# FedericoV/SysBio_Modeling

Hardware: AMD Instinct MI355X
Metric: ensemble ODE-steps/sec (20-state model + fwd sens) (higher is better)
Workload: dtype f64; 1 GPU; configs[2]: cascade20 (20 states, 40 params) + full forward sensitivities = 820 ODEs, 4096 vectors/GPU, DOPRI45, 16 output times; gather + integrate + residual/Jacobian assembly; vectors_per_gpu=4096, n_equations=820, integrator=dopri45, failed_vectors=0

## Files before the change

sysbio_modeling_amd/csrc/models/cascade20.hpp:

```cpp
#pragma once

__constant__ short SBM_RL_CLASS[20] = {0, 1, 1, 1, 1, 1, 1, 1, 1, 1, 1, 1, 1, 1, 1, 1, 1, 1, 1, 1};
__constant__ short SBM_RL_YS[40] = {19, 1, 2, 3, 4, 5, 6, 7, 8, 9, 10, 11, 12, 13, 14, 15, 16, 17, 18, 19, 0, 0, 1, 2, 3, 4, 5, 6, 7, 8, 9, 10, 11, 12, 13, 14, 15, 16, 17, 18};
__constant__ short SBM_RL_PS[40] = {0, 21, 22, 23, 24, 25, 26, 27, 28, 29, 30, 31, 32, 33, 34, 35, 36, 37, 38, 39, 20, 1, 2, 3, 4, 5, 6, 7, 8, 9, 10, 11, 12, 13, 14, 15, 16, 17, 18, 19};
__constant__ short SBM_RL_JYOUT[40] = {0, 2, 4, 6, 8, 10, 12, 14, 16, 18, 20, 22, 24, 26, 28, 30, 32, 34, 36, 38, 1, 3, 5, 7, 9, 11, 13, 15, 17, 19, 21, 23, 25, 27, 29, 31, 33, 35, 37, 39};
__constant__ short SBM_RL_APOS[40] = {0, 65, 130, 195, 260, 325, 390, 455, 520, 585, 650, 715, 780, 845, 910, 975, 1040, 1105, 1170, 1235, 20, 85, 150, 215, 280, 345, 410, 475, 540, 605, 670, 735, 800, 865, 930, 995, 1060, 1125, 1190, 1255};
__constant__ short SBM_RL_JPCOL[40] = {0, 1, 2, 3, 4, 5, 6, 7, 8, 9, 10, 11, 12, 13, 14, 15, 16, 17, 18, 19, 20, 21, 22, 23, 24, 25, 26, 27, 28, 29, 30, 31, 32, 33, 34, 35, 36, 37, 38, 39};
__constant__ short SBM_RL_JYCOL[40] = {0, 0, 1, 2, 3, 4, 5, 6, 7, 8, 9, 10, 11, 12, 13, 14, 15, 16, 17, 18, 19, 1, 2, 3, 4, 5, 6, 7, 8, 9, 10, 11, 12, 13, 14, 15, 16, 17, 18, 19};

__constant__ short SBM_RG0_JYPOS[40] = {0, 3, 5, 7, 9, 11, 13, 15, 17, 19, 21, 23, 25, 27, 29, 31, 33, 35, 37, 39, 1, 2, 4, 6, 8, 10, 12, 14, 16, 18, 20, 22, 24, 26, 28, 30, 32, 34, 36, 38};
__constant__ short SBM_RG0_HSRC[3] = {19, 6, 13};

__constant__ short SBM_RG1_JYPOS[40] = {0, 3, 5, 7, 9, 11, 13, 15, 17, 19, 21, 23, 25, 27, 29, 31, 33, 35, 37, 39, 1, 2, 4, 6, 8, 10, 12, 14, 16, 18, 20, 22, 24, 26, 28, 30, 32, 34, 36, 38};
__constant__ short SBM_RG1_HSRC[7] = {19, 2, 5, 8, 11, 14, 17};

__constant__ short SBM_RG2_JYPOS[40] = {0, 3, 5, 7, 9, 11, 13, 15, 17, 19, 21, 23, 25, 27, 29, 31, 33, 35, 37, 39, 1, 2, 4, 6, 8, 10, 12, 14, 16, 18, 20, 22, 24, 26, 28, 30, 32, 34, 36, 38};
__constant__ short SBM_RG2_HSRC[3] = {19, 6, 13};

__constant__ short SBM_IM_RSTART[1] = {0};
__constant__ short SBM_IM_DIAGSLOT[1] = {-1};
__constant__ short SBM_IM_MFPOS[1] = {0};
__constant__ short SBM_IM_R0[1] = {0};
__constant__ short SBM_IM_JPQ[1] = {0};

struct SbmModel {
  static constexpr int NV = 20;
  static constexpr int NP = 40;
  static constexpr int NK = 40;
  static constexpr int NNZ_JY = 40;
  static constexpr int NNZ_JP = 40;
  static constexpr int NJY = 40;
  static constexpr int NJP = 40;
  static constexpr const char* NAME = "cascade20";

  template <class PA>
  __device__ __forceinline__ static void eval_f(double t, const double (&y)[NV], const PA& p,
                                                double (&f)[NV]) {
    (void)t;
    f[0] = -p[20]*y[0] + p[0]*SBM_RCP(y[19] + 1.0);
    f[1] = -p[21]*y[1] + p[1]*y[0]*SBM_RCP(y[0] + 1.0);
    f[2] = -p[22]*y[2] + p[2]*y[1]*SBM_RCP(y[1] + 1.0);
    f[3] = -p[23]*y[3] + p[3]*y[2]*SBM_RCP(y[2] + 1.0);
    f[4] = -p[24]*y[4] + p[4]*y[3]*SBM_RCP(y[3] + 1.0);
    f[5] = -p[25]*y[5] + p[5]*y[4]*SBM_RCP(y[4] + 1.0);
    f[6] = -p[26]*y[6] + p[6]*y[5]*SBM_RCP(y[5] + 1.0);
    f[7] = -p[27]*y[7] + p[7]*y[6]*SBM_RCP(y[6] + 1.0);
    f[8] = -p[28]*y[8] + p[8]*y[7]*SBM_RCP(y[7] + 1.0);
    f[9] = -p[29]*y[9] + p[9]*y[8]*SBM_RCP(y[8] + 1.0);
    f[10] = -p[30]*y[10] + p[10]*y[9]*SBM_RCP(y[9] + 1.0);
    f[11] = -p[31]*y[11] + p[11]*y[10]*SBM_RCP(y[10] + 1.0);
    f[12] = -p[32]*y[12] + p[12]*y[11]*SBM_RCP(y[11] + 1.0);
    f[13] = -p[33]*y[13] + p[13]*y[12]*SBM_RCP(y[12] + 1.0);
    f[14] = -p[34]*y[14] + p[14]*y[13]*SBM_RCP(y[13] + 1.0);
    f[15] = -p[35]*y[15] + p[15]*y[14]*SBM_RCP(y[14] + 1.0);
    f[16] = -p[36]*y[16] + p[16]*y[15]*SBM_RCP(y[15] + 1.0);
    f[17] = -p[37]*y[17] + p[17]*y[16]*SBM_RCP(y[16] + 1.0);
    f[18] = -p[38]*y[18] + p[18]*y[17]*SBM_RCP(y[17] + 1.0);
    f[19] = -p[39]*y[19] + p[19]*y[18]*SBM_RCP(y[18] + 1.0);
  }

  template <class PA>
  __device__ __forceinline__ static void eval_jac(double t, const double (&y)[NV], const PA& p,
                                                  double (&f)[NV], double (&jy)[NJY], double (&jp)[NJP]) {
    (void)t;
    const double x_0 = SBM_RCP(y[19] + 1.0);
    const double x_1 = SBM_RCP(y[0] + 1.0);
    const double x_2 = SBM_RCP(y[1] + 1.0);
    const double x_3 = SBM_RCP(y[2] + 1.0);
    const double x_4 = SBM_RCP(y[3] + 1.0);
    const double x_5 = SBM_RCP(y[4] + 1.0);
    const double x_6 = SBM_RCP(y[5] + 1.0);
    const double x_7 = SBM_RCP(y[6] + 1.0);
    const double x_8 = SBM_RCP(y[7] + 1.0);
    const double x_9 = SBM_RCP(y[8] + 1.0);
    const double x_10 = SBM_RCP(y[9] + 1.0);
    const double x_11 = SBM_RCP(y[10] + 1.0);
    const double x_12 = SBM_RCP(y[11] + 1.0);
    const double x_13 = SBM_RCP(y[12] + 1.0);
    const double x_14 = SBM_RCP(y[13] + 1.0);
    const double x_15 = SBM_RCP(y[14] + 1.0);
    const double x_16 = SBM_RCP(y[15] + 1.0);
    const double x_17 = SBM_RCP(y[16] + 1.0);
    const double x_18 = SBM_RCP(y[17] + 1.0);
    const double x_19 = SBM_RCP(y[18] + 1.0);
    f[0] = -p[20]*y[0] + p[0]*x_0;
    f[1] = -p[21]*y[1] + p[1]*y[0]*x_1;
    f[2] = -p[22]*y[2] + p[2]*y[1]*x_2;
    f[3] = -p[23]*y[3] + p[3]*y[2]*x_3;
    f[4] = -p[24]*y[4] + p[4]*y[3]*x_4;
    f[5] = -p[25]*y[5] + p[5]*y[4]*x_5;
    f[6] = -p[26]*y[6] + p[6]*y[5]*x_6;
    f[7] = -p[27]*y[7] + p[7]*y[6]*x_7;
    f[8] = -p[28]*y[8] + p[8]*y[7]*x_8;
    f[9] = -p[29]*y[9] + p[9]*y[8]*x_9;
    f[10] = -p[30]*y[10] + p[10]*y[9]*x_10;
    f[11] = -p[31]*y[11] + p[11]*y[10]*x_11;
    f[12] = -p[32]*y[12] + p[12]*y[11]*x_12;
    f[13] = -p[33]*y[13] + p[13]*y[12]*x_13;
    f[14] = -p[34]*y[14] + p[14]*y[13]*x_14;
    f[15] = -p[35]*y[15] + p[15]*y[14]*x_15;
    f[16] = -p[36]*y[16] + p[16]*y[15]*x_16;
    f[17] = -p[37]*y[17] + p[17]*y[16]*x_17;
    f[18] = -p[38]*y[18] + p[18]*y[17]*x_18;
    f[19] = -p[39]*y[19] + p[19]*y[18]*x_19;
    jy[0] = -p[20];
    jy[1] = -p[0]*(x_0*x_0);
    jy[2] = p[1]*(x_1*x_1);
    jy[3] = -p[21];
    jy[4] = p[2]*(x_2*x_2);
    jy[5] = -p[22];
    jy[6] = p[3]*(x_3*x_3);
    jy[7] = -p[23];
    jy[8] = p[4]*(x_4*x_4);
    jy[9] = -p[24];
    jy[10] = p[5]*(x_5*x_5);
    jy[11] = -p[25];
    jy[12] = p[6]*(x_6*x_6);
    jy[13] = -p[26];
    jy[14] = p[7]*(x_7*x_7);
    jy[15] = -p[27];
    jy[16] = p[8]*(x_8*x_8);
    jy[17] = -p[28];
    jy[18] = p[9]*(x_9*x_9);
    jy[19] = -p[29];
    jy[20] = p[10]*(x_10*x_10);
    jy[21] = -p[30];
    jy[22] = p[11]*(x_11*x_11);
    jy[23] = -p[31];
    jy[24] = p[12]*(x_12*x_12);
    jy[25] = -p[32];
    jy[26] = p[13]*(x_13*x_13);
    jy[27] = -p[33];
    jy[28] = p[14]*(x_14*x_14);
    jy[29] = -p[34];
    jy[30] = p[15]*(x_15*x_15);
    jy[31] = -p[35];
    jy[32] = p[16]*(x_16*x_16);
    jy[33] = -p[36];
    jy[34] = p[17]*(x_17*x_17);
    jy[35] = -p[37];
    jy[36] = p[18]*(x_18*x_18);
    jy[37] = -p[38];
    jy[38] = p[19]*(x_19*x_19);
    jy[39] = -p[39];
    jp[0] = x_0;
    jp[1] = -y[0];
    jp[2] = y[0]*x_1;
    jp[3] = -y[1];
    jp[4] = y[1]*x_2;
    jp[5] = -y[2];
    jp[6] = y[2]*x_3;
    jp[7] = -y[3];
    jp[8] = y[3]*x_4;
    jp[9] = -y[4];
    jp[10] = y[4]*x_5;
    jp[11] = -y[5];
    jp[12] = y[5]*x_6;
    jp[13] = -y[6];
    jp[14] = y[6]*x_7;
    jp[15] = -y[7];
    jp[16] = y[7]*x_8;
    jp[17] = -y[8];
    jp[18] = y[8]*x_9;
    jp[19] = -y[9];
    jp[20] = y[9]*x_10;
    jp[21] = -y[10];
    jp[22] = y[10]*x_11;
    jp[23] = -y[11];
    jp[24] = y[11]*x_12;
    jp[25] = -y[12];
    jp[26] = y[12]*x_13;
    jp[27] = -y[13];
    jp[28] = y[13]*x_14;
    jp[29] = -y[14];
    jp[30] = y[14]*x_15;
    jp[31] = -y[15];
    jp[32] = y[15]*x_16;
    jp[33] = -y[16];
    jp[34] = y[16]*x_17;
    jp[35] = -y[17];
    jp[36] = y[17]*x_18;
    jp[37] = -y[18];
    jp[38] = y[18]*x_19;
    jp[39] = -y[19];
  }

  __device__ __forceinline__ static void apply_col(const double (&jy)[NJY], const double (&jp)[NJP],
                                                   int scol, const double (&z)[NV], double (&dz)[NV]) {
    dz[0] = fma(jy[1], z[19], fma(jy[0], z[0], SBM_PICK(scol, 0, jp[0], SBM_PICK(scol, 20, jp[1], 0.0))));
    dz[1] = fma(jy[3], z[1], fma(jy[2], z[0], SBM_PICK(scol, 1, jp[2], SBM_PICK(scol, 21, jp[3], 0.0))));
    dz[2] = fma(jy[5], z[2], fma(jy[4], z[1], SBM_PICK(scol, 2, jp[4], SBM_PICK(scol, 22, jp[5], 0.0))));
    dz[3] = fma(jy[7], z[3], fma(jy[6], z[2], SBM_PICK(scol, 3, jp[6], SBM_PICK(scol, 23, jp[7], 0.0))));
    dz[4] = fma(jy[9], z[4], fma(jy[8], z[3], SBM_PICK(scol, 4, jp[8], SBM_PICK(scol, 24, jp[9], 0.0))));
    dz[5] = fma(jy[11], z[5], fma(jy[10], z[4], SBM_PICK(scol, 5, jp[10], SBM_PICK(scol, 25, jp[11], 0.0))));
    dz[6] = fma(jy[13], z[6], fma(jy[12], z[5], SBM_PICK(scol, 6, jp[12], SBM_PICK(scol, 26, jp[13], 0.0))));
    dz[7] = fma(jy[15], z[7], fma(jy[14], z[6], SBM_PICK(scol, 7, jp[14], SBM_PICK(scol, 27, jp[15], 0.0))));
    dz[8] = fma(jy[17], z[8], fma(jy[16], z[7], SBM_PICK(scol, 8, jp[16], SBM_PICK(scol, 28, jp[17], 0.0))));
    dz[9] = fma(jy[19], z[9], fma(jy[18], z[8], SBM_PICK(scol, 9, jp[18], SBM_PICK(scol, 29, jp[19], 0.0))));
    dz[10] = fma(jy[21], z[10], fma(jy[20], z[9], SBM_PICK(scol, 10, jp[20], SBM_PICK(scol, 30, jp[21], 0.0))));
    dz[11] = fma(jy[23], z[11], fma(jy[22], z[10], SBM_PICK(scol, 11, jp[22], SBM_PICK(scol, 31, jp[23], 0.0))));
    dz[12] = fma(jy[25], z[12], fma(jy[24], z[11], SBM_PICK(scol, 12, jp[24], SBM_PICK(scol, 32, jp[25], 0.0))));
    dz[13] = fma(jy[27], z[13], fma(jy[26], z[12], SBM_PICK(scol, 13, jp[26], SBM_PICK(scol, 33, jp[27], 0.0))));
    dz[14] = fma(jy[29], z[14], fma(jy[28], z[13], SBM_PICK(scol, 14, jp[28], SBM_PICK(scol, 34, jp[29], 0.0))));
    dz[15] = fma(jy[31], z[15], fma(jy[30], z[14], SBM_PICK(scol, 15, jp[30], SBM_PICK(scol, 35, jp[31], 0.0))));
    dz[16] = fma(jy[33], z[16], fma(jy[32], z[15], SBM_PICK(scol, 16, jp[32], SBM_PICK(scol, 36, jp[33], 0.0))));
    dz[17] = fma(jy[35], z[17], fma(jy[34], z[16], SBM_PICK(scol, 17, jp[34], SBM_PICK(scol, 37, jp[35], 0.0))));
    dz[18] = fma(jy[37], z[18], fma(jy[36], z[17], SBM_PICK(scol, 18, jp[36], SBM_PICK(scol, 38, jp[37], 0.0))));
    dz[19] = fma(jy[39], z[19], fma(jy[38], z[18], SBM_PICK(scol, 19, jp[38], SBM_PICK(scol, 39, jp[39], 0.0))));
  }

  template <class PA>
  __device__ __forceinline__ static void eval_col(double t, const double (&y)[NV], const PA& p, int scol,
                                                  const double (&z)[NV], double (&dz)[NV]) {
    (void)t;
    const bool state_lane = scol < 0;
    const double x_0 = SBM_RCP(y[19] + 1.0);
    dz[0] = SBM_SEL(state_lane, -p[20]*y[0] + p[0]*x_0, fma(-p[0]*(x_0*x_0), z[19], fma(-p[20], z[0], SBM_PICK(scol, 0, x_0, SBM_PICK(scol, 20, -y[0], 0.0)))));
    const double x_1 = SBM_RCP(y[0] + 1.0);
    dz[1] = SBM_SEL(state_lane, -p[21]*y[1] + p[1]*y[0]*x_1, fma(-p[21], z[1], fma(p[1]*(x_1*x_1), z[0], SBM_PICK(scol, 1, y[0]*x_1, SBM_PICK(scol, 21, -y[1], 0.0)))));
    const double x_2 = SBM_RCP(y[1] + 1.0);
    dz[2] = SBM_SEL(state_lane, -p[22]*y[2] + p[2]*y[1]*x_2, fma(-p[22], z[2], fma(p[2]*(x_2*x_2), z[1], SBM_PICK(scol, 2, y[1]*x_2, SBM_PICK(scol, 22, -y[2], 0.0)))));
    const double x_3 = SBM_RCP(y[2] + 1.0);
    dz[3] = SBM_SEL(state_lane, -p[23]*y[3] + p[3]*y[2]*x_3, fma(-p[23], z[3], fma(p[3]*(x_3*x_3), z[2], SBM_PICK(scol, 3, y[2]*x_3, SBM_PICK(scol, 23, -y[3], 0.0)))));
    const double x_4 = SBM_RCP(y[3] + 1.0);
    dz[4] = SBM_SEL(state_lane, -p[24]*y[4] + p[4]*y[3]*x_4, fma(-p[24], z[4], fma(p[4]*(x_4*x_4), z[3], SBM_PICK(scol, 4, y[3]*x_4, SBM_PICK(scol, 24, -y[4], 0.0)))));
    const double x_5 = SBM_RCP(y[4] + 1.0);
    dz[5] = SBM_SEL(state_lane, -p[25]*y[5] + p[5]*y[4]*x_5, fma(-p[25], z[5], fma(p[5]*(x_5*x_5), z[4], SBM_PICK(scol, 5, y[4]*x_5, SBM_PICK(scol, 25, -y[5], 0.0)))));
    const double x_6 = SBM_RCP(y[5] + 1.0);
    dz[6] = SBM_SEL(state_lane, -p[26]*y[6] + p[6]*y[5]*x_6, fma(-p[26], z[6], fma(p[6]*(x_6*x_6), z[5], SBM_PICK(scol, 6, y[5]*x_6, SBM_PICK(scol, 26, -y[6], 0.0)))));
    const double x_7 = SBM_RCP(y[6] + 1.0);
    dz[7] = SBM_SEL(state_lane, -p[27]*y[7] + p[7]*y[6]*x_7, fma(-p[27], z[7], fma(p[7]*(x_7*x_7), z[6], SBM_PICK(scol, 7, y[6]*x_7, SBM_PICK(scol, 27, -y[7], 0.0)))));
    const double x_8 = SBM_RCP(y[7] + 1.0);
    dz[8] = SBM_SEL(state_lane, -p[28]*y[8] + p[8]*y[7]*x_8, fma(-p[28], z[8], fma(p[8]*(x_8*x_8), z[7], SBM_PICK(scol, 8, y[7]*x_8, SBM_PICK(scol, 28, -y[8], 0.0)))));
    const double x_9 = SBM_RCP(y[8] + 1.0);
    dz[9] = SBM_SEL(state_lane, -p[29]*y[9] + p[9]*y[8]*x_9, fma(-p[29], z[9], fma(p[9]*(x_9*x_9), z[8], SBM_PICK(scol, 9, y[8]*x_9, SBM_PICK(scol, 29, -y[9], 0.0)))));
    const double x_10 = SBM_RCP(y[9] + 1.0);
    dz[10] = SBM_SEL(state_lane, -p[30]*y[10] + p[10]*y[9]*x_10, fma(-p[30], z[10], fma(p[10]*(x_10*x_10), z[9], SBM_PICK(scol, 10, y[9]*x_10, SBM_PICK(scol, 30, -y[10], 0.0)))));
    const double x_11 = SBM_RCP(y[10] + 1.0);
    dz[11] = SBM_SEL(state_lane, -p[31]*y[11] + p[11]*y[10]*x_11, fma(-p[31], z[11], fma(p[11]*(x_11*x_11), z[10], SBM_PICK(scol, 11, y[10]*x_11, SBM_PICK(scol, 31, -y[11], 0.0)))));
    const double x_12 = SBM_RCP(y[11] + 1.0);
    dz[12] = SBM_SEL(state_lane, -p[32]*y[12] + p[12]*y[11]*x_12, fma(-p[32], z[12], fma(p[12]*(x_12*x_12), z[11], SBM_PICK(scol, 12, y[11]*x_12, SBM_PICK(scol, 32, -y[12], 0.0)))));
    const double x_13 = SBM_RCP(y[12] + 1.0);
    dz[13] = SBM_SEL(state_lane, -p[33]*y[13] + p[13]*y[12]*x_13, fma(-p[33], z[13], fma(p[13]*(x_13*x_13), z[12], SBM_PICK(scol, 13, y[12]*x_13, SBM_PICK(scol, 33, -y[13], 0.0)))));
    const double x_14 = SBM_RCP(y[13] + 1.0);
    dz[14] = SBM_SEL(state_lane, -p[34]*y[14] + p[14]*y[13]*x_14, fma(-p[34], z[14], fma(p[14]*(x_14*x_14), z[13], SBM_PICK(scol, 14, y[13]*x_14, SBM_PICK(scol, 34, -y[14], 0.0)))));
    const double x_15 = SBM_RCP(y[14] + 1.0);
    dz[15] = SBM_SEL(state_lane, -p[35]*y[15] + p[15]*y[14]*x_15, fma(-p[35], z[15], fma(p[15]*(x_15*x_15), z[14], SBM_PICK(scol, 15, y[14]*x_15, SBM_PICK(scol, 35, -y[15], 0.0)))));
    const double x_16 = SBM_RCP(y[15] + 1.0);
    dz[16] = SBM_SEL(state_lane, -p[36]*y[16] + p[16]*y[15]*x_16, fma(-p[36], z[16], fma(p[16]*(x_16*x_16), z[15], SBM_PICK(scol, 16, y[15]*x_16, SBM_PICK(scol, 36, -y[16], 0.0)))));
    const double x_17 = SBM_RCP(y[16] + 1.0);
    dz[17] = SBM_SEL(state_lane, -p[37]*y[17] + p[17]*y[16]*x_17, fma(-p[37], z[17], fma(p[17]*(x_17*x_17), z[16], SBM_PICK(scol, 17, y[16]*x_17, SBM_PICK(scol, 37, -y[17], 0.0)))));
    const double x_18 = SBM_RCP(y[17] + 1.0);
    dz[18] = SBM_SEL(state_lane, -p[38]*y[18] + p[18]*y[17]*x_18, fma(-p[38], z[18], fma(p[18]*(x_18*x_18), z[17], SBM_PICK(scol, 18, y[17]*x_18, SBM_PICK(scol, 38, -y[18], 0.0)))));
    const double x_19 = SBM_RCP(y[18] + 1.0);
    dz[19] = SBM_SEL(state_lane, -p[39]*y[19] + p[19]*y[18]*x_19, fma(-p[39], z[19], fma(p[19]*(x_19*x_19), z[18], SBM_PICK(scol, 19, y[18]*x_19, SBM_PICK(scol, 39, -y[19], 0.0)))));
  }

  static constexpr int RL_NCLASS = 2;
  static constexpr int RL_MAXYS = 2, RL_MAXPS = 2, RL_MAXJY = 2, RL_MAXJP = 2;
  static constexpr int RL_LARGEST_CLASS = 19;
  __device__ __forceinline__ static int rl_class(int row) { return SBM_RL_CLASS[row]; }
  __device__ __forceinline__ static int rl_ys(int slot, int row) { return SBM_RL_YS[slot * NV + row]; }
  __device__ __forceinline__ static int rl_ps(int slot, int row) { return SBM_RL_PS[slot * NV + row]; }
  __device__ __forceinline__ static int rl_jyout(int slot, int row) { return SBM_RL_JYOUT[slot * NV + row]; }
  __device__ __forceinline__ static int rl_apos(int slot, int row) { return SBM_RL_APOS[slot * NV + row]; }
  __device__ __forceinline__ static int rl_jpcol(int slot, int row) { return SBM_RL_JPCOL[slot * NV + row]; }
  __device__ __forceinline__ static int rl_jycol(int slot, int row) { return SBM_RL_JYCOL[slot * NV + row]; }
  __device__ __forceinline__ static void class_dispatch(int cls, double t, const double (&ys)[RL_MAXYS],
                                                        const double (&ps)[RL_MAXPS], double& f,
                                                        double (&jy)[RL_MAXJY], double (&jp)[RL_MAXJP]) {
    (void)t; (void)ys; (void)ps;
    const bool is0 = (cls == 0);
    const double h0 = SBM_RCP(SBM_SEL(is0, ys[0], ys[1]) + 1.0);
    const double c0_x0 = h0;
    const double c1_x0 = h0;
    f = SBM_SEL(is0, ps[0]*c0_x0 - ps[1]*ys[1], -ps[0]*ys[0] + ps[1]*ys[1]*c1_x0);
    jy[0] = SBM_SEL(is0, -ps[1], ps[1]*(c1_x0*c1_x0));
    jy[1] = SBM_SEL(is0, -ps[0]*(c0_x0*c0_x0), -ps[0]);
    jp[0] = SBM_SEL(is0, c0_x0, ys[1]*c1_x0);
    jp[1] = SBM_SEL(is0, -ys[1], -ys[0]);
  }

  static constexpr int RL_NSTATIC = 20;
  __device__ __forceinline__ static void rl_static(const double (&jy)[RL_MAXJY], double (&sj)[20]) {
    (void)jy;
    sj[0] = SBM_LANE_BCAST(jy[0], 0);
    sj[1] = SBM_LANE_BCAST(jy[1], 1);
    sj[2] = SBM_LANE_BCAST(jy[1], 2);
    sj[3] = SBM_LANE_BCAST(jy[1], 3);
    sj[4] = SBM_LANE_BCAST(jy[1], 4);
    sj[5] = SBM_LANE_BCAST(jy[1], 5);
    sj[6] = SBM_LANE_BCAST(jy[1], 6);
    sj[7] = SBM_LANE_BCAST(jy[1], 7);
    sj[8] = SBM_LANE_BCAST(jy[1], 8);
    sj[9] = SBM_LANE_BCAST(jy[1], 9);
    sj[10] = SBM_LANE_BCAST(jy[1], 10);
    sj[11] = SBM_LANE_BCAST(jy[1], 11);
    sj[12] = SBM_LANE_BCAST(jy[1], 12);
    sj[13] = SBM_LANE_BCAST(jy[1], 13);
    sj[14] = SBM_LANE_BCAST(jy[1], 14);
    sj[15] = SBM_LANE_BCAST(jy[1], 15);
    sj[16] = SBM_LANE_BCAST(jy[1], 16);
    sj[17] = SBM_LANE_BCAST(jy[1], 17);
    sj[18] = SBM_LANE_BCAST(jy[1], 18);
    sj[19] = SBM_LANE_BCAST(jy[1], 19);
  }

  template <int NZ>
  __device__ __forceinline__ static void apply_rowlane(const double (&jy)[RL_MAXJY], const double (&sj)[20],
                                                       const double (&acol)[NV], const double (&z)[NZ],
                                                       double (&dz)[NZ]) {
    (void)jy; (void)sj;
    dz[0] = fma(SBM_LANE_BCAST(jy[1], 0), z[19], fma(sj[0], z[0], acol[0]));
    dz[1] = fma(sj[1], z[1], fma(SBM_LANE_BCAST(jy[0], 1), z[0], acol[1]));
    dz[2] = fma(sj[2], z[2], fma(SBM_LANE_BCAST(jy[0], 2), z[1], acol[2]));
    dz[3] = fma(sj[3], z[3], fma(SBM_LANE_BCAST(jy[0], 3), z[2], acol[3]));
    dz[4] = fma(sj[4], z[4], fma(SBM_LANE_BCAST(jy[0], 4), z[3], acol[4]));
    dz[5] = fma(sj[5], z[5], fma(SBM_LANE_BCAST(jy[0], 5), z[4], acol[5]));
    dz[6] = fma(sj[6], z[6], fma(SBM_LANE_BCAST(jy[0], 6), z[5], acol[6]));
    dz[7] = fma(sj[7], z[7], fma(SBM_LANE_BCAST(jy[0], 7), z[6], acol[7]));
    dz[8] = fma(sj[8], z[8], fma(SBM_LANE_BCAST(jy[0], 8), z[7], acol[8]));
    dz[9] = fma(sj[9], z[9], fma(SBM_LANE_BCAST(jy[0], 9), z[8], acol[9]));
    dz[10] = fma(sj[10], z[10], fma(SBM_LANE_BCAST(jy[0], 10), z[9], acol[10]));
    dz[11] = fma(sj[11], z[11], fma(SBM_LANE_BCAST(jy[0], 11), z[10], acol[11]));
    dz[12] = fma(sj[12], z[12], fma(SBM_LANE_BCAST(jy[0], 12), z[11], acol[12]));
    dz[13] = fma(sj[13], z[13], fma(SBM_LANE_BCAST(jy[0], 13), z[12], acol[13]));
    dz[14] = fma(sj[14], z[14], fma(SBM_LANE_BCAST(jy[0], 14), z[13], acol[14]));
    dz[15] = fma(sj[15], z[15], fma(SBM_LANE_BCAST(jy[0], 15), z[14], acol[15]));
    dz[16] = fma(sj[16], z[16], fma(SBM_LANE_BCAST(jy[0], 16), z[15], acol[16]));
    dz[17] = fma(sj[17], z[17], fma(SBM_LANE_BCAST(jy[0], 17), z[16], acol[17]));
    dz[18] = fma(sj[18], z[18], fma(SBM_LANE_BCAST(jy[0], 18), z[17], acol[18]));
    dz[19] = fma(sj[19], z[19], fma(SBM_LANE_BCAST(jy[0], 19), z[18], acol[19]));
  }

  template <int NZ>
  __device__ __forceinline__ static void apply_lds(const double* jyl, const double (&acol)[NV],
                                                   const double (&z)[NZ], double (&dz)[NZ]) {
    (void)jyl;
    dz[0] = fma(jyl[1], z[19], fma(jyl[0], z[0], acol[0]));
    dz[1] = fma(jyl[3], z[1], fma(jyl[2], z[0], acol[1]));
    dz[2] = fma(jyl[5], z[2], fma(jyl[4], z[1], acol[2]));
    dz[3] = fma(jyl[7], z[3], fma(jyl[6], z[2], acol[3]));
    dz[4] = fma(jyl[9], z[4], fma(jyl[8], z[3], acol[4]));
    dz[5] = fma(jyl[11], z[5], fma(jyl[10], z[4], acol[5]));
    dz[6] = fma(jyl[13], z[6], fma(jyl[12], z[5], acol[6]));
    dz[7] = fma(jyl[15], z[7], fma(jyl[14], z[6], acol[7]));
    dz[8] = fma(jyl[17], z[8], fma(jyl[16], z[7], acol[8]));
    dz[9] = fma(jyl[19], z[9], fma(jyl[18], z[8], acol[9]));
    dz[10] = fma(jyl[21], z[10], fma(jyl[20], z[9], acol[10]));
    dz[11] = fma(jyl[23], z[11], fma(jyl[22], z[10], acol[11]));
    dz[12] = fma(jyl[25], z[12], fma(jyl[24], z[11], acol[12]));
    dz[13] = fma(jyl[27], z[13], fma(jyl[26], z[12], acol[13]));
    dz[14] = fma(jyl[29], z[14], fma(jyl[28], z[13], acol[14]));
    dz[15] = fma(jyl[31], z[15], fma(jyl[30], z[14], acol[15]));
    dz[16] = fma(jyl[33], z[16], fma(jyl[32], z[15], acol[16]));
    dz[17] = fma(jyl[35], z[17], fma(jyl[34], z[16], acol[17]));
    dz[18] = fma(jyl[37], z[18], fma(jyl[36], z[17], acol[18]));
    dz[19] = fma(jyl[39], z[19], fma(jyl[38], z[18], acol[19]));
  }

  struct RG0 {
  static constexpr bool RG_OK = true;
  static constexpr int RG_G = 3, RG_C = 20, RG_CPL = 2, RG_RPG = 7, RG_JYS = 2, RG_NHALO = 1;
  static constexpr int RG_NCH = 1;
  static constexpr int RG_LS = 128;
  __device__ __forceinline__ static int rg_pos(int row, int col) {
    return (row % RG_RPG) * RG_LS + RG_CPL * ((row / RG_RPG) * RG_C + col % RG_C) + col / RG_C;
  }
  __device__ __forceinline__ static int rg_jypos(int slot, int row) { return SBM_RG0_JYPOS[slot * NV + row]; }
  __device__ __forceinline__ static int rg_hsrc(int term, int group) { return SBM_RG0_HSRC[term * RG_G + group]; }
  template <int NZ>
  __device__ __forceinline__ static void publish_rowgroup(double* h_lane, const double (&z)[NZ]) {
    (void)h_lane; (void)z;
    h_lane[640] = z[5];
    h_lane[641] = z[12];
    h_lane[768] = z[6];
    h_lane[769] = z[13];
  }
  __device__ __forceinline__ static void load_rowgroup(const double* a_lane, const double* jy_lane,
                                                       double (&acol)[14], double (&coef)[14]) {
    coef[0] = jy_lane[0];
    coef[1] = jy_lane[1];
    coef[2] = jy_lane[2];
    coef[3] = jy_lane[3];
    coef[4] = jy_lane[4];
    coef[5] = jy_lane[5];
    coef[6] = jy_lane[6];
    coef[7] = jy_lane[7];
    coef[8] = jy_lane[8];
    coef[9] = jy_lane[9];
    coef[10] = jy_lane[10];
    coef[11] = jy_lane[11];
    coef[12] = jy_lane[12];
    coef[13] = jy_lane[13];
    acol[0] = a_lane[0];
    acol[7] = a_lane[1];
    acol[1] = a_lane[128];
    acol[8] = a_lane[129];
    acol[2] = a_lane[256];
    acol[9] = a_lane[257];
    acol[3] = a_lane[384];
    acol[10] = a_lane[385];
    acol[4] = a_lane[512];
    acol[11] = a_lane[513];
    acol[5] = a_lane[640];
    acol[12] = a_lane[641];
    acol[6] = a_lane[768];
    acol[13] = a_lane[769];
  }
  template <int NZ>
  __device__ __forceinline__ static void apply_rowgroup(const double (&acol)[14], const double (&coef)[14],
                                                        const double* h_all, const int (&hoff)[1],
                                                        const double (&z)[NZ], double (&dz)[NZ]) {
    (void)h_all; (void)hoff;
    const double h0_1_0 = h_all[hoff[0] + 0];
    const double h0_1_1 = h_all[hoff[0] + 1];
    dz[1] = fma(coef[3], z[0], fma(coef[2], z[1], acol[1]));
    dz[2] = fma(coef[5], z[1], fma(coef[4], z[2], acol[2]));
    dz[3] = fma(coef[7], z[2], fma(coef[6], z[3], acol[3]));
    dz[4] = fma(coef[9], z[3], fma(coef[8], z[4], acol[4]));
    dz[5] = fma(coef[11], z[4], fma(coef[10], z[5], acol[5]));
    dz[6] = fma(coef[13], z[5], fma(coef[12], z[6], acol[6]));
    dz[0] = fma(coef[1], h0_1_0, fma(coef[0], z[0], acol[0]));
    dz[8] = fma(coef[3], z[7], fma(coef[2], z[8], acol[8]));
    dz[9] = fma(coef[5], z[8], fma(coef[4], z[9], acol[9]));
    dz[10] = fma(coef[7], z[9], fma(coef[6], z[10], acol[10]));
    dz[11] = fma(coef[9], z[10], fma(coef[8], z[11], acol[11]));
    dz[12] = fma(coef[11], z[11], fma(coef[10], z[12], acol[12]));
    dz[13] = fma(coef[13], z[12], fma(coef[12], z[13], acol[13]));
    dz[7] = fma(coef[1], h0_1_1, fma(coef[0], z[7], acol[7]));
  }
  };
  struct RG1 {
  static constexpr bool RG_OK = true;
  static constexpr int RG_G = 7, RG_C = 8, RG_CPL = 1, RG_RPG = 3, RG_JYS = 2, RG_NHALO = 1;
  static constexpr int RG_NCH = 5;
  static constexpr int RG_LS = 64;
  __device__ __forceinline__ static int rg_pos(int row, int col) {
    return (row % RG_RPG) * RG_LS + RG_CPL * ((row / RG_RPG) * RG_C + col % RG_C) + col / RG_C;
  }
  __device__ __forceinline__ static int rg_jypos(int slot, int row) { return SBM_RG1_JYPOS[slot * NV + row]; }
  __device__ __forceinline__ static int rg_hsrc(int term, int group) { return SBM_RG1_HSRC[term * RG_G + group]; }
  template <int NZ>
  __device__ __forceinline__ static void publish_rowgroup(double* h_lane, const double (&z)[NZ]) {
    (void)h_lane; (void)z;
    h_lane[64] = z[1];
    h_lane[128] = z[2];
  }
  __device__ __forceinline__ static void load_rowgroup(const double* a_lane, const double* jy_lane,
                                                       double (&acol)[3], double (&coef)[6]) {
    coef[0] = jy_lane[0];
    coef[1] = jy_lane[1];
    coef[2] = jy_lane[2];
    coef[3] = jy_lane[3];
    coef[4] = jy_lane[4];
    coef[5] = jy_lane[5];
    acol[0] = a_lane[0];
    acol[1] = a_lane[64];
    acol[2] = a_lane[128];
  }
  template <int NZ>
  __device__ __forceinline__ static void apply_rowgroup(const double (&acol)[3], const double (&coef)[6],
                                                        const double* h_all, const int (&hoff)[1],
                                                        const double (&z)[NZ], double (&dz)[NZ]) {
    (void)h_all; (void)hoff;
    const double h0_1_0 = h_all[hoff[0] + 0];
    dz[1] = fma(coef[3], z[0], fma(coef[2], z[1], acol[1]));
    dz[2] = fma(coef[5], z[1], fma(coef[4], z[2], acol[2]));
    dz[0] = fma(coef[1], h0_1_0, fma(coef[0], z[0], acol[0]));
  }
  };
  struct RG2 {
  static constexpr bool RG_OK = true;
  static constexpr int RG_G = 3, RG_C = 20, RG_CPL = 1, RG_RPG = 7, RG_JYS = 2, RG_NHALO = 1;
  static constexpr int RG_NCH = 2;
  static constexpr int RG_LS = 64;
  __device__ __forceinline__ static int rg_pos(int row, int col) {
    return (row % RG_RPG) * RG_LS + RG_CPL * ((row / RG_RPG) * RG_C + col % RG_C) + col / RG_C;
  }
  __device__ __forceinline__ static int rg_jypos(int slot, int row) { return SBM_RG2_JYPOS[slot * NV + row]; }
  __device__ __forceinline__ static int rg_hsrc(int term, int group) { return SBM_RG2_HSRC[term * RG_G + group]; }
  template <int NZ>
  __device__ __forceinline__ static void publish_rowgroup(double* h_lane, const double (&z)[NZ]) {
    (void)h_lane; (void)z;
    h_lane[320] = z[5];
    h_lane[384] = z[6];
  }
  __device__ __forceinline__ static void load_rowgroup(const double* a_lane, const double* jy_lane,
                                                       double (&acol)[7], double (&coef)[14]) {
    coef[0] = jy_lane[0];
    coef[1] = jy_lane[1];
    coef[2] = jy_lane[2];
    coef[3] = jy_lane[3];
    coef[4] = jy_lane[4];
    coef[5] = jy_lane[5];
    coef[6] = jy_lane[6];
    coef[7] = jy_lane[7];
    coef[8] = jy_lane[8];
    coef[9] = jy_lane[9];
    coef[10] = jy_lane[10];
    coef[11] = jy_lane[11];
    coef[12] = jy_lane[12];
    coef[13] = jy_lane[13];
    acol[0] = a_lane[0];
    acol[1] = a_lane[64];
    acol[2] = a_lane[128];
    acol[3] = a_lane[192];
    acol[4] = a_lane[256];
    acol[5] = a_lane[320];
    acol[6] = a_lane[384];
  }
// ... 218 lines not shown
```

sysbio_modeling_amd/csrc/models/michaelis_menten.hpp:

```cpp
#pragma once

__constant__ short SBM_RL_CLASS[2] = {0, 1};
__constant__ short SBM_RL_YS[4] = {0, 1, 0, 0};
__constant__ short SBM_RL_PS[8] = {2, 4, 3, 0, 0, 1, 1, 0};
__constant__ short SBM_RL_JYOUT[4] = {0, 1, 3, 2};
__constant__ short SBM_RL_APOS[8] = {0, 64, 1, 65, 2, 68, 3, 128};
__constant__ short SBM_RL_JPCOL[8] = {0, 0, 1, 1, 2, 4, 3, -1};
__constant__ short SBM_RL_JYCOL[4] = {0, 0, -1, 1};

__constant__ short SBM_RG0_JYPOS[4] = {0, 3, 4, 2};
__constant__ short SBM_RG0_HSRC[2] = {2, 0};

__constant__ short SBM_IM_RSTART[2] = {0, 2};
__constant__ short SBM_IM_DIAGSLOT[2] = {0, 1};
__constant__ short SBM_IM_MFPOS[4] = {4, 3, 4, 4};
__constant__ short SBM_IM_R0[1] = {0};
__constant__ short SBM_IM_JPQ[1] = {0};

struct SbmModel {
  static constexpr int NV = 2;
  static constexpr int NP = 5;
  static constexpr int NK = 5;
  static constexpr int NNZ_JY = 3;
  static constexpr int NNZ_JP = 7;
  static constexpr int NJY = 3;
  static constexpr int NJP = 7;
  static constexpr const char* NAME = "michaelis_menten";

  template <class PA>
  __device__ __forceinline__ static void eval_f(double t, const double (&y)[NV], const PA& p,
                                                double (&f)[NV]) {
    (void)t;
    const double x_0 = y[0]*p[0]*SBM_RCP(y[0] + p[1]);
    f[0] = -y[0]*p[3] + p[2] - x_0;
    f[1] = -y[1]*p[4] + x_0;
  }

  template <class PA>
  __device__ __forceinline__ static void eval_jac(double t, const double (&y)[NV], const PA& p,
                                                  double (&f)[NV], double (&jy)[NJY], double (&jp)[NJP]) {
    (void)t;
    const double x_0 = SBM_RCP(y[0] + p[1]);
    const double x_1 = y[0]*x_0;
    const double x_2 = p[0]*x_1;
    const double x_3 = p[0]*(x_0*x_0);
    const double x_4 = p[1]*x_3;
    const double x_5 = y[0]*x_3;
    f[0] = -y[0]*p[3] + p[2] - x_2;
    f[1] = -y[1]*p[4] + x_2;
    jy[0] = -p[3] - x_4;
    jy[1] = x_4;
    jy[2] = -p[4];
    jp[0] = -x_1;
    jp[1] = x_5;
    jp[2] = 1.0;
    jp[3] = -y[0];
    jp[4] = x_1;
    jp[5] = -x_5;
    jp[6] = -y[1];
  }

  __device__ __forceinline__ static void apply_col(const double (&jy)[NJY], const double (&jp)[NJP],
                                                   int scol, const double (&z)[NV], double (&dz)[NV]) {
    dz[0] = fma(jy[0], z[0], SBM_PICK(scol, 0, jp[0], SBM_PICK(scol, 1, jp[1], SBM_PICK(scol, 2, jp[2], SBM_PICK(scol, 3, jp[3], 0.0)))));
    dz[1] = fma(jy[2], z[1], fma(jy[1], z[0], SBM_PICK(scol, 0, jp[4], SBM_PICK(scol, 1, jp[5], SBM_PICK(scol, 4, jp[6], 0.0)))));
  }

  template <class PA>
  __device__ __forceinline__ static void eval_col(double t, const double (&y)[NV], const PA& p, int scol,
                                                  const double (&z)[NV], double (&dz)[NV]) {
    (void)t;
    const bool state_lane = scol < 0;
    const double x_0 = SBM_RCP(y[0] + p[1]);
    const double x_1 = y[0]*x_0;
    const double x_2 = p[0]*x_1;
    const double x_3 = p[0]*(x_0*x_0);
    const double x_4 = p[1]*x_3;
    const double x_5 = y[0]*x_3;
    dz[0] = SBM_SEL(state_lane, -y[0]*p[3] + p[2] - x_2, fma(-p[3] - x_4, z[0], SBM_PICK(scol, 0, -x_1, SBM_PICK(scol, 1, x_5, SBM_PICK(scol, 2, 1.0, SBM_PICK(scol, 3, -y[0], 0.0))))));
    dz[1] = SBM_SEL(state_lane, -y[1]*p[4] + x_2, fma(-p[4], z[1], fma(x_4, z[0], SBM_PICK(scol, 0, x_1, SBM_PICK(scol, 1, -x_5, SBM_PICK(scol, 4, -y[1], 0.0))))));
  }

  static constexpr int RL_NCLASS = 2;
  static constexpr int RL_MAXYS = 2, RL_MAXPS = 4, RL_MAXJY = 2, RL_MAXJP = 4;
  static constexpr int RL_LARGEST_CLASS = 1;
  __device__ __forceinline__ static int rl_class(int row) { return SBM_RL_CLASS[row]; }
  __device__ __forceinline__ static int rl_ys(int slot, int row) { return SBM_RL_YS[slot * NV + row]; }
  __device__ __forceinline__ static int rl_ps(int slot, int row) { return SBM_RL_PS[slot * NV + row]; }
  __device__ __forceinline__ static int rl_jyout(int slot, int row) { return SBM_RL_JYOUT[slot * NV + row]; }
  __device__ __forceinline__ static int rl_apos(int slot, int row) { return SBM_RL_APOS[slot * NV + row]; }
  __device__ __forceinline__ static int rl_jpcol(int slot, int row) { return SBM_RL_JPCOL[slot * NV + row]; }
  __device__ __forceinline__ static int rl_jycol(int slot, int row) { return SBM_RL_JYCOL[slot * NV + row]; }
  __device__ __forceinline__ static void class_dispatch(int cls, double t, const double (&ys)[RL_MAXYS],
                                                        const double (&ps)[RL_MAXPS], double& f,
                                                        double (&jy)[RL_MAXJY], double (&jp)[RL_MAXJP]) {
    (void)t; (void)ys; (void)ps;
    const bool is0 = (cls == 0);
    const double h0 = SBM_RCP(SBM_SEL(is0, ps[3], ps[2]) + SBM_SEL(is0, ys[0], ys[1]));
    const double c0_x0 = h0;
    const double c0_x1 = ys[0]*c0_x0;
    const double c0_x2 = ps[2]*(c0_x0*c0_x0);
    const double c1_x0 = h0;
    const double c1_x1 = ps[1]*(c1_x0*c1_x0);
    f = SBM_SEL(is0, ps[0] - ps[1]*ys[0] - ps[2]*c0_x1, -ps[0]*ys[0] + ps[1]*ys[1]*c1_x0);
    jy[0] = SBM_SEL(is0, -ps[1] - ps[3]*c0_x2, ps[2]*c1_x1);
    jy[1] = SBM_SEL(is0, 0.0, -ps[0]);
    jp[0] = SBM_SEL(is0, -c0_x1, ys[1]*c1_x0);
    jp[1] = SBM_SEL(is0, ys[0]*c0_x2, -ys[1]*c1_x1);
    jp[2] = SBM_SEL(is0, 1.0, -ys[0]);
    jp[3] = SBM_SEL(is0, -ys[0], 0.0);
  }

  static constexpr int RL_NSTATIC = 1;
  __device__ __forceinline__ static void rl_static(const double (&jy)[RL_MAXJY], double (&sj)[1]) {
    (void)jy;
    sj[0] = SBM_LANE_BCAST(jy[1], 1);
  }

  template <int NZ>
  __device__ __forceinline__ static void apply_rowlane(const double (&jy)[RL_MAXJY], const double (&sj)[1],
                                                       const double (&acol)[NV], const double (&z)[NZ],
                                                       double (&dz)[NZ]) {
    (void)jy; (void)sj;
    dz[0] = fma(SBM_LANE_BCAST(jy[0], 0), z[0], acol[0]);
    dz[1] = fma(sj[0], z[1], fma(SBM_LANE_BCAST(jy[0], 1), z[0], acol[1]));
  }

  template <int NZ>
  __device__ __forceinline__ static void apply_lds(const double* jyl, const double (&acol)[NV],
                                                   const double (&z)[NZ], double (&dz)[NZ]) {
    (void)jyl;
    dz[0] = fma(jyl[0], z[0], acol[0]);
    dz[1] = fma(jyl[3], z[1], fma(jyl[2], z[0], acol[1]));
  }

  struct RG0 {
  static constexpr bool RG_OK = true;
  static constexpr int RG_G = 2, RG_C = 5, RG_CPL = 1, RG_RPG = 1, RG_JYS = 2, RG_NHALO = 1;
  static constexpr int RG_NCH = 1;
  static constexpr int RG_LS = 64;
  __device__ __forceinline__ static int rg_pos(int row, int col) {
    return (row % RG_RPG) * RG_LS + RG_CPL * ((row / RG_RPG) * RG_C + col % RG_C) + col / RG_C;
  }
  __device__ __forceinline__ static int rg_jypos(int slot, int row) { return SBM_RG0_JYPOS[slot * NV + row]; }
  __device__ __forceinline__ static int rg_hsrc(int term, int group) { return SBM_RG0_HSRC[term * RG_G + group]; }
  template <int NZ>
  __device__ __forceinline__ static void publish_rowgroup(double* h_lane, const double (&z)[NZ]) {
    (void)h_lane; (void)z;
    h_lane[0] = z[0];
  }
  __device__ __forceinline__ static void load_rowgroup(const double* a_lane, const double* jy_lane,
                                                       double (&acol)[1], double (&coef)[2]) {
    coef[0] = jy_lane[0];
    coef[1] = jy_lane[1];
    acol[0] = a_lane[0];
  }
  template <int NZ>
  __device__ __forceinline__ static void apply_rowgroup(const double (&acol)[1], const double (&coef)[2],
                                                        const double* h_all, const int (&hoff)[1],
                                                        const double (&z)[NZ], double (&dz)[NZ]) {
    (void)h_all; (void)hoff;
    const double h0_1_0 = h_all[hoff[0] + 0];
    dz[0] = fma(coef[1], h0_1_0, fma(coef[0], z[0], acol[0]));
  }
  };
  using RG1 = RG0;
  using RG2 = RG0;

  static constexpr int IM_NM = 3;
  __device__ __forceinline__ static void im_build(double gamma, const double* jy, double (&m)[IM_NM]) {
    (void)gamma; (void)jy;
    m[0] = fma(-gamma, jy[0], 1.0);
    m[1] = -gamma * jy[1];
    m[2] = fma(-gamma, jy[2], 1.0);
  }
  __device__ __forceinline__ static void im_factor(double (&m)[IM_NM]) {
    m[0] = SBM_RCP(m[0]);
    m[1] *= m[0];
    m[2] = SBM_RCP(m[2]);
  }
  __device__ __forceinline__ static void im_solve(const double (&m)[IM_NM], double (&b)[NV]) {
    b[1] = fma(-m[1], b[0], b[1]);
    b[1] *= m[2];
    b[0] *= m[0];
  }
  static constexpr bool IM_TRI = true;
  __device__ __forceinline__ static void im_solve_tri(const double* mf, double (&b)[NV]) {
    b[0] = mf[0] * b[0];
    b[1] = fma(mf[3], b[0], mf[2] * b[1]);
  }
  template <int RPL>
  __device__ __forceinline__ static void im_solve_tri_pick(const double* mf, const double* g, int lane, double (&d)[RPL]) {
    const double x_0 = mf[0] * g[0];
    d[0] = SBM_SEL(lane == 0, x_0, d[0]);
    const double x_1 = fma(mf[3], x_0, mf[2] * g[1]);
    d[0] = SBM_SEL(lane == 1, x_1, d[0]);
  }
  static constexpr bool IM_SENS_TRI = true;
  static constexpr int IM_JP = RL_MAXJP > 0 ? RL_MAXJP : 1;
  __device__ __forceinline__ static void im_sens_tri(const double* mf, const double* ja, double hh, int col, double (&z)[NV]) {
    (void)col;
    double t0[4], a0[2 * IM_JP];
    _Pragma("unroll") for (int e = 0; e < 4; ++e) t0[e] = mf[0 + e];
    _Pragma("unroll") for (int e = 0; e < 2 * RL_MAXJP; ++e) a0[e] = ja[0 * RL_MAXJP + e];
    SBM_LDS_FENCE();
    z[0] = fma(hh, SBM_PICK_COL(col, 0, a0[0 * RL_MAXJP + 0], SBM_PICK_COL(col, 1, a0[0 * RL_MAXJP + 1], SBM_PICK_COL(col, 2, a0[0 * RL_MAXJP + 2], SBM_PICK_COL(col, 3, a0[0 * RL_MAXJP + 3], 0.0)))), z[0]);
    z[0] = t0[0] * z[0];
    z[1] = fma(hh, SBM_PICK_COL(col, 0, a0[1 * RL_MAXJP + 0], SBM_PICK_COL(col, 1, a0[1 * RL_MAXJP + 1], SBM_PICK_COL(col, 4, a0[1 * RL_MAXJP + 2], 0.0))), z[1]);
    z[1] = fma(t0[3], z[0], t0[2] * z[1]);
  }
  static constexpr int IM_MF = 4;
  static constexpr bool IM_CHAIN = true;
  static constexpr bool IM_ROT = false;
  static_assert(!IM_ROT || sizeof(SBM_IM_R0) / sizeof(short) >= NK, "one rotated-column entry per column");
  static_assert(!IM_ROT || sizeof(SBM_IM_JPQ) / sizeof(short) >= NK, "one rotated-column entry per column");
  __device__ __forceinline__ static int im_r0(int col) { return SBM_IM_R0[IM_ROT ? col : 0]; }
  __device__ __forceinline__ static int im_jpq(int col) { return SBM_IM_JPQ[IM_ROT ? col : 0]; }
  static constexpr bool IM_DIST = false;
  static constexpr int IM_LD = 2;
  __device__ __forceinline__ static void im_factor_rows(double (&)[NV], int, double*) {}
  __device__ __forceinline__ static void im_solve_lds(const double*, const double*, double (&)[NV]) {}
  __device__ __forceinline__ static int im_rstart(int row) { return SBM_IM_RSTART[IM_TRI ? row : 0]; }
  __device__ __forceinline__ static int im_diagslot(int row) { return SBM_IM_DIAGSLOT[IM_TRI ? row : 0]; }
  __device__ __forceinline__ static int im_mfpos(int slot, int row) { return SBM_IM_MFPOS[IM_TRI ? slot * NV + row : 0]; }
};
```

sysbio_modeling_amd/csrc/models/stiff50.hpp:

```cpp
#pragma once

__constant__ short SBM_RL_CLASS[50] = {0, 1, 1, 1, 1, 1, 1, 1, 1, 1, 1, 1, 1, 1, 1, 1, 1, 1, 1, 1, 1, 1, 1, 1, 1, 1, 1, 1, 1, 1, 1, 1, 1, 1, 1, 1, 1, 1, 1, 1, 1, 1, 1, 1, 1, 1, 1, 1, 1, 1};
__constant__ short SBM_RL_YS[100] = {0, 0, 1, 2, 3, 4, 5, 6, 7, 8, 9, 10, 11, 12, 13, 14, 15, 16, 17, 18, 19, 20, 21, 22, 23, 24, 25, 26, 27, 28, 29, 30, 31, 32, 33, 34, 35, 36, 37, 38, 39, 40, 41, 42, 43, 44, 45, 46, 47, 48, 0, 1, 2, 3, 4, 5, 6, 7, 8, 9, 10, 11, 12, 13, 14, 15, 16, 17, 18, 19, 20, 21, 22, 23, 24, 25, 26, 27, 28, 29, 30, 31, 32, 33, 34, 35, 36, 37, 38, 39, 40, 41, 42, 43, 44, 45, 46, 47, 48, 49};
__constant__ short SBM_RL_PS[100] = {0, 1, 2, 3, 4, 5, 6, 7, 8, 9, 10, 11, 12, 13, 14, 15, 16, 17, 18, 19, 20, 21, 22, 23, 24, 25, 26, 27, 28, 29, 30, 31, 32, 33, 34, 35, 36, 37, 38, 39, 40, 41, 42, 43, 44, 45, 46, 47, 48, 49, 50, 51, 52, 53, 54, 55, 56, 57, 58, 59, 60, 61, 62, 63, 64, 65, 66, 67, 68, 69, 70, 71, 72, 73, 74, 75, 76, 77, 78, 79, 80, 81, 82, 83, 84, 85, 86, 87, 88, 89, 90, 91, 92, 93, 94, 95, 96, 97, 98, 99};
__constant__ short SBM_RL_JYOUT[100] = {0, 1, 3, 5, 7, 9, 11, 13, 15, 17, 19, 21, 23, 25, 27, 29, 31, 33, 35, 37, 39, 41, 43, 45, 47, 49, 51, 53, 55, 57, 59, 61, 63, 65, 67, 69, 71, 73, 75, 77, 79, 81, 83, 85, 87, 89, 91, 93, 95, 97, 99, 2, 4, 6, 8, 10, 12, 14, 16, 18, 20, 22, 24, 26, 28, 30, 32, 34, 36, 38, 40, 42, 44, 46, 48, 50, 52, 54, 56, 58, 60, 62, 64, 66, 68, 70, 72, 74, 76, 78, 80, 82, 84, 86, 88, 90, 92, 94, 96, 98};
__constant__ short SBM_RL_APOS[50] = {0, 65, 130, 195, 260, 325, 390, 455, 520, 585, 650, 715, 780, 845, 910, 975, 1040, 1105, 1170, 1235, 1300, 1365, 1430, 1495, 1560, 1625, 1690, 1755, 1820, 1885, 1950, 2015, 2080, 2145, 2210, 2275, 2340, 2405, 2470, 2535, 2600, 2665, 2730, 2795, 2860, 2925, 2990, 3055, 3120, 3185};
__constant__ short SBM_RL_JPCOL[50] = {0, 1, 2, 3, 4, 5, 6, 7, 8, 9, 10, 11, 12, 13, 14, 15, 16, 17, 18, 19, 20, 21, 22, 23, 24, 25, 26, 27, 28, 29, 30, 31, 32, 33, 34, 35, 36, 37, 38, 39, 40, 41, 42, 43, 44, 45, 46, 47, 48, 49};
__constant__ short SBM_RL_JYCOL[100] = {0, 0, 1, 2, 3, 4, 5, 6, 7, 8, 9, 10, 11, 12, 13, 14, 15, 16, 17, 18, 19, 20, 21, 22, 23, 24, 25, 26, 27, 28, 29, 30, 31, 32, 33, 34, 35, 36, 37, 38, 39, 40, 41, 42, 43, 44, 45, 46, 47, 48, -1, 1, 2, 3, 4, 5, 6, 7, 8, 9, 10, 11, 12, 13, 14, 15, 16, 17, 18, 19, 20, 21, 22, 23, 24, 25, 26, 27, 28, 29, 30, 31, 32, 33, 34, 35, 36, 37, 38, 39, 40, 41, 42, 43, 44, 45, 46, 47, 48, 49};

__constant__ short SBM_RG0_JYPOS[100] = {0, 3, 5, 7, 9, 11, 13, 15, 17, 19, 21, 23, 25, 27, 29, 31, 33, 35, 37, 39, 41, 43, 45, 47, 49, 51, 53, 55, 57, 59, 61, 63, 65, 67, 69, 71, 73, 75, 77, 79, 81, 83, 85, 87, 89, 91, 93, 95, 97, 99, 108, 2, 4, 6, 8, 10, 12, 14, 16, 18, 20, 22, 24, 26, 28, 30, 32, 34, 36, 38, 40, 42, 44, 46, 48, 50, 52, 54, 56, 58, 60, 62, 64, 66, 68, 70, 72, 74, 76, 78, 80, 82, 84, 86, 88, 90, 92, 94, 96, 98};
__constant__ short SBM_RG0_HSRC[6] = {54, 8, 17, 26, 35, 44};

__constant__ short SBM_RG1_JYPOS[100] = {0, 3, 5, 7, 9, 11, 13, 15, 17, 19, 21, 23, 25, 27, 29, 31, 33, 35, 37, 39, 41, 43, 45, 47, 49, 51, 53, 55, 57, 59, 61, 63, 65, 67, 69, 71, 73, 75, 77, 79, 81, 83, 85, 87, 89, 91, 93, 95, 97, 99, 112, 2, 4, 6, 8, 10, 12, 14, 16, 18, 20, 22, 24, 26, 28, 30, 32, 34, 36, 38, 40, 42, 44, 46, 48, 50, 52, 54, 56, 58, 60, 62, 64, 66, 68, 70, 72, 74, 76, 78, 80, 82, 84, 86, 88, 90, 92, 94, 96, 98};
__constant__ short SBM_RG1_HSRC[8] = {56, 6, 13, 20, 27, 34, 41, 48};

__constant__ short SBM_RG2_JYPOS[100] = {0, 3, 5, 7, 9, 11, 13, 15, 17, 19, 21, 23, 25, 27, 29, 31, 33, 35, 37, 39, 41, 43, 45, 47, 49, 51, 53, 55, 57, 59, 61, 63, 65, 67, 69, 71, 73, 75, 77, 79, 81, 83, 85, 87, 89, 91, 93, 95, 97, 99, 112, 2, 4, 6, 8, 10, 12, 14, 16, 18, 20, 22, 24, 26, 28, 30, 32, 34, 36, 38, 40, 42, 44, 46, 48, 50, 52, 54, 56, 58, 60, 62, 64, 66, 68, 70, 72, 74, 76, 78, 80, 82, 84, 86, 88, 90, 92, 94, 96, 98};
__constant__ short SBM_RG2_HSRC[8] = {56, 6, 13, 20, 27, 34, 41, 48};

__constant__ short SBM_IM_RSTART[50] = {0, 2, 4, 6, 8, 10, 12, 14, 16, 18, 20, 22, 24, 26, 28, 30, 32, 34, 36, 38, 40, 42, 44, 46, 48, 50, 52, 54, 56, 58, 60, 62, 64, 66, 68, 70, 72, 74, 76, 78, 80, 82, 84, 86, 88, 90, 92, 94, 96, 98};
__constant__ short SBM_IM_DIAGSLOT[50] = {0, 1, 1, 1, 1, 1, 1, 1, 1, 1, 1, 1, 1, 1, 1, 1, 1, 1, 1, 1, 1, 1, 1, 1, 1, 1, 1, 1, 1, 1, 1, 1, 1, 1, 1, 1, 1, 1, 1, 1, 1, 1, 1, 1, 1, 1, 1, 1, 1, 1};
__constant__ short SBM_IM_MFPOS[100] = {100, 3, 5, 7, 9, 11, 13, 15, 17, 19, 21, 23, 25, 27, 29, 31, 33, 35, 37, 39, 41, 43, 45, 47, 49, 51, 53, 55, 57, 59, 61, 63, 65, 67, 69, 71, 73, 75, 77, 79, 81, 83, 85, 87, 89, 91, 93, 95, 97, 99, 100, 100, 100, 100, 100, 100, 100, 100, 100, 100, 100, 100, 100, 100, 100, 100, 100, 100, 100, 100, 100, 100, 100, 100, 100, 100, 100, 100, 100, 100, 100, 100, 100, 100, 100, 100, 100, 100, 100, 100, 100, 100, 100, 100, 100, 100, 100, 100, 100, 100};
__constant__ short SBM_IM_R0[50] = {0, 1, 2, 3, 4, 5, 6, 7, 8, 9, 10, 11, 12, 13, 14, 15, 16, 17, 18, 19, 20, 21, 22, 23, 24, 25, 26, 27, 28, 29, 30, 31, 32, 33, 34, 35, 36, 37, 38, 39, 40, 41, 42, 43, 44, 45, 46, 47, 48, 49};
__constant__ short SBM_IM_JPQ[50] = {0, 0, 0, 0, 0, 0, 0, 0, 0, 0, 0, 0, 0, 0, 0, 0, 0, 0, 0, 0, 0, 0, 0, 0, 0, 0, 0, 0, 0, 0, 0, 0, 0, 0, 0, 0, 0, 0, 0, 0, 0, 0, 0, 0, 0, 0, 0, 0, 0, 0};

// ... 790 lines not shown
    const double x_109 = SBM_RCP(x_108 + 1.0);
    const double x_110 = p[77]*x_108*x_109 + y[26]*x_107;
    const double x_225 = 4.0*y[26];
    dz[27] = SBM_SEL(state_lane, -p[27]*x_110, fma(-p[27]*(x_109*x_109)*(2.0*p[77] + y[26] + (y[27]*y[27])*x_225 + y[27]*x_225), z[27], fma(-p[27]*x_107, z[26], SBM_PICK(scol, 27, -x_110, 0.0))));
    const double x_111 = y[28] + (-1.0);
    const double x_112 = 2.0*y[28];
    const double x_113 = SBM_RCP(x_112 + 1.0);
    const double x_114 = p[78]*x_112*x_113 + y[27]*x_111;
    const double x_226 = 4.0*y[27];
    dz[28] = SBM_SEL(state_lane, -p[28]*x_114, fma(-p[28]*(x_113*x_113)*(2.0*p[78] + y[27] + (y[28]*y[28])*x_226 + y[28]*x_226), z[28], fma(-p[28]*x_111, z[27], SBM_PICK(scol, 28, -x_114, 0.0))));
    const double x_115 = y[29] + (-1.0);
    const double x_116 = 2.0*y[29];
    const double x_117 = SBM_RCP(x_116 + 1.0);
    const double x_118 = p[79]*x_116*x_117 + y[28]*x_115;
    const double x_227 = 4.0*y[28];
    dz[29] = SBM_SEL(state_lane, -p[29]*x_118, fma(-p[29]*(x_117*x_117)*(2.0*p[79] + y[28] + (y[29]*y[29])*x_227 + y[29]*x_227), z[29], fma(-p[29]*x_115, z[28], SBM_PICK(scol, 29, -x_118, 0.0))));
    const double x_119 = y[30] + (-1.0);
    const double x_120 = 2.0*y[30];
    const double x_121 = SBM_RCP(x_120 + 1.0);
    const double x_122 = p[80]*x_120*x_121 + y[29]*x_119;
    const double x_228 = 4.0*y[29];
    dz[30] = SBM_SEL(state_lane, -p[30]*x_122, fma(-p[30]*(x_121*x_121)*(2.0*p[80] + y[29] + (y[30]*y[30])*x_228 + y[30]*x_228), z[30], fma(-p[30]*x_119, z[29], SBM_PICK(scol, 30, -x_122, 0.0))));
    const double x_123 = y[31] + (-1.0);
    const double x_124 = 2.0*y[31];
    const double x_125 = SBM_RCP(x_124 + 1.0);
    const double x_126 = p[81]*x_124*x_125 + y[30]*x_123;
    const double x_229 = 4.0*y[30];
    dz[31] = SBM_SEL(state_lane, -p[31]*x_126, fma(-p[31]*(x_125*x_125)*(2.0*p[81] + y[30] + (y[31]*y[31])*x_229 + y[31]*x_229), z[31], fma(-p[31]*x_123, z[30], SBM_PICK(scol, 31, -x_126, 0.0))));
    const double x_127 = y[32] + (-1.0);
    const double x_128 = 2.0*y[32];
    const double x_129 = SBM_RCP(x_128 + 1.0);
    const double x_130 = p[82]*x_128*x_129 + y[31]*x_127;
    const double x_230 = 4.0*y[31];
    dz[32] = SBM_SEL(state_lane, -p[32]*x_130, fma(-p[32]*(x_129*x_129)*(2.0*p[82] + y[31] + (y[32]*y[32])*x_230 + y[32]*x_230), z[32], fma(-p[32]*x_127, z[31], SBM_PICK(scol, 32, -x_130, 0.0))));
    const double x_131 = y[33] + (-1.0);
    const double x_132 = 2.0*y[33];
    const double x_133 = SBM_RCP(x_132 + 1.0);
    const double x_134 = p[83]*x_132*x_133 + y[32]*x_131;
    const double x_231 = 4.0*y[32];
    dz[33] = SBM_SEL(state_lane, -p[33]*x_134, fma(-p[33]*(x_133*x_133)*(2.0*p[83] + y[32] + (y[33]*y[33])*x_231 + y[33]*x_231), z[33], fma(-p[33]*x_131, z[32], SBM_PICK(scol, 33, -x_134, 0.0))));
    const double x_135 = y[34] + (-1.0);
    const double x_136 = 2.0*y[34];
    const double x_137 = SBM_RCP(x_136 + 1.0);
    const double x_138 = p[84]*x_136*x_137 + y[33]*x_135;
    const double x_232 = 4.0*y[33];
    dz[34] = SBM_SEL(state_lane, -p[34]*x_138, fma(-p[34]*(x_137*x_137)*(2.0*p[84] + y[33] + (y[34]*y[34])*x_232 + y[34]*x_232), z[34], fma(-p[34]*x_135, z[33], SBM_PICK(scol, 34, -x_138, 0.0))));
    const double x_139 = y[35] + (-1.0);
    const double x_140 = 2.0*y[35];
    const double x_141 = SBM_RCP(x_140 + 1.0);
    const double x_142 = p[85]*x_140*x_141 + y[34]*x_139;
    const double x_233 = 4.0*y[34];
    dz[35] = SBM_SEL(state_lane, -p[35]*x_142, fma(-p[35]*(x_141*x_141)*(2.0*p[85] + y[34] + (y[35]*y[35])*x_233 + y[35]*x_233), z[35], fma(-p[35]*x_139, z[34], SBM_PICK(scol, 35, -x_142, 0.0))));
    const double x_143 = y[36] + (-1.0);
    const double x_144 = 2.0*y[36];
    const double x_145 = SBM_RCP(x_144 + 1.0);
    const double x_146 = p[86]*x_144*x_145 + y[35]*x_143;
    const double x_234 = 4.0*y[35];
    dz[36] = SBM_SEL(state_lane, -p[36]*x_146, fma(-p[36]*(x_145*x_145)*(2.0*p[86] + y[35] + (y[36]*y[36])*x_234 + y[36]*x_234), z[36], fma(-p[36]*x_143, z[35], SBM_PICK(scol, 36, -x_146, 0.0))));
    const double x_147 = y[37] + (-1.0);
    const double x_148 = 2.0*y[37];
    const double x_149 = SBM_RCP(x_148 + 1.0);
    const double x_150 = p[87]*x_148*x_149 + y[36]*x_147;
    const double x_235 = 4.0*y[36];
    dz[37] = SBM_SEL(state_lane, -p[37]*x_150, fma(-p[37]*(x_149*x_149)*(2.0*p[87] + y[36] + (y[37]*y[37])*x_235 + y[37]*x_235), z[37], fma(-p[37]*x_147, z[36], SBM_PICK(scol, 37, -x_150, 0.0))));
    const double x_151 = y[38] + (-1.0);
    const double x_152 = 2.0*y[38];
    const double x_153 = SBM_RCP(x_152 + 1.0);
    const double x_154 = p[88]*x_152*x_153 + y[37]*x_151;
    const double x_236 = 4.0*y[37];
    dz[38] = SBM_SEL(state_lane, -p[38]*x_154, fma(-p[38]*(x_153*x_153)*(2.0*p[88] + y[37] + (y[38]*y[38])*x_236 + y[38]*x_236), z[38], fma(-p[38]*x_151, z[37], SBM_PICK(scol, 38, -x_154, 0.0))));
    const double x_155 = y[39] + (-1.0);
    const double x_156 = 2.0*y[39];
    const double x_157 = SBM_RCP(x_156 + 1.0);
    const double x_158 = p[89]*x_156*x_157 + y[38]*x_155;
    const double x_237 = 4.0*y[38];
    dz[39] = SBM_SEL(state_lane, -p[39]*x_158, fma(-p[39]*(x_157*x_157)*(2.0*p[89] + y[38] + (y[39]*y[39])*x_237 + y[39]*x_237), z[39], fma(-p[39]*x_155, z[38], SBM_PICK(scol, 39, -x_158, 0.0))));
    const double x_159 = y[40] + (-1.0);
    const double x_160 = 2.0*y[40];
    const double x_161 = SBM_RCP(x_160 + 1.0);
    const double x_162 = p[90]*x_160*x_161 + y[39]*x_159;
    const double x_238 = 4.0*y[39];
    dz[40] = SBM_SEL(state_lane, -p[40]*x_162, fma(-p[40]*(x_161*x_161)*(2.0*p[90] + y[39] + (y[40]*y[40])*x_238 + y[40]*x_238), z[40], fma(-p[40]*x_159, z[39], SBM_PICK(scol, 40, -x_162, 0.0))));
    const double x_163 = y[41] + (-1.0);
    const double x_164 = 2.0*y[41];
    const double x_165 = SBM_RCP(x_164 + 1.0);
    const double x_166 = p[91]*x_164*x_165 + y[40]*x_163;
    const double x_239 = 4.0*y[40];
    dz[41] = SBM_SEL(state_lane, -p[41]*x_166, fma(-p[41]*(x_165*x_165)*(2.0*p[91] + y[40] + (y[41]*y[41])*x_239 + y[41]*x_239), z[41], fma(-p[41]*x_163, z[40], SBM_PICK(scol, 41, -x_166, 0.0))));
    const double x_167 = y[42] + (-1.0);
    const double x_168 = 2.0*y[42];
    const double x_169 = SBM_RCP(x_168 + 1.0);
    const double x_170 = p[92]*x_168*x_169 + y[41]*x_167;
    const double x_240 = 4.0*y[41];
    dz[42] = SBM_SEL(state_lane, -p[42]*x_170, fma(-p[42]*(x_169*x_169)*(2.0*p[92] + y[41] + (y[42]*y[42])*x_240 + y[42]*x_240), z[42], fma(-p[42]*x_167, z[41], SBM_PICK(scol, 42, -x_170, 0.0))));
    const double x_171 = y[43] + (-1.0);
    const double x_172 = 2.0*y[43];
    const double x_173 = SBM_RCP(x_172 + 1.0);
    const double x_174 = p[93]*x_172*x_173 + y[42]*x_171;
    const double x_241 = 4.0*y[42];
    dz[43] = SBM_SEL(state_lane, -p[43]*x_174, fma(-p[43]*(x_173*x_173)*(2.0*p[93] + y[42] + (y[43]*y[43])*x_241 + y[43]*x_241), z[43], fma(-p[43]*x_171, z[42], SBM_PICK(scol, 43, -x_174, 0.0))));
    const double x_175 = y[44] + (-1.0);
    const double x_176 = 2.0*y[44];
    const double x_177 = SBM_RCP(x_176 + 1.0);
    const double x_178 = p[94]*x_176*x_177 + y[43]*x_175;
    const double x_242 = 4.0*y[43];
    dz[44] = SBM_SEL(state_lane, -p[44]*x_178, fma(-p[44]*(x_177*x_177)*(2.0*p[94] + y[43] + (y[44]*y[44])*x_242 + y[44]*x_242), z[44], fma(-p[44]*x_175, z[43], SBM_PICK(scol, 44, -x_178, 0.0))));
    const double x_179 = y[45] + (-1.0);
    const double x_180 = 2.0*y[45];
    const double x_181 = SBM_RCP(x_180 + 1.0);
    const double x_182 = p[95]*x_180*x_181 + y[44]*x_179;
    const double x_243 = 4.0*y[44];
    dz[45] = SBM_SEL(state_lane, -p[45]*x_182, fma(-p[45]*(x_181*x_181)*(2.0*p[95] + y[44] + (y[45]*y[45])*x_243 + y[45]*x_243), z[45], fma(-p[45]*x_179, z[44], SBM_PICK(scol, 45, -x_182, 0.0))));
    const double x_183 = y[46] + (-1.0);
    const double x_184 = 2.0*y[46];
    const double x_185 = SBM_RCP(x_184 + 1.0);
    const double x_186 = p[96]*x_184*x_185 + y[45]*x_183;
    const double x_244 = 4.0*y[45];
    dz[46] = SBM_SEL(state_lane, -p[46]*x_186, fma(-p[46]*(x_185*x_185)*(2.0*p[96] + y[45] + (y[46]*y[46])*x_244 + y[46]*x_244), z[46], fma(-p[46]*x_183, z[45], SBM_PICK(scol, 46, -x_186, 0.0))));
    const double x_187 = y[47] + (-1.0);
    const double x_188 = 2.0*y[47];
    const double x_189 = SBM_RCP(x_188 + 1.0);
    const double x_190 = p[97]*x_188*x_189 + y[46]*x_187;
    const double x_245 = 4.0*y[46];
    dz[47] = SBM_SEL(state_lane, -p[47]*x_190, fma(-p[47]*(x_189*x_189)*(2.0*p[97] + y[46] + (y[47]*y[47])*x_245 + y[47]*x_245), z[47], fma(-p[47]*x_187, z[46], SBM_PICK(scol, 47, -x_190, 0.0))));
    const double x_191 = y[48] + (-1.0);
    const double x_192 = 2.0*y[48];
    const double x_193 = SBM_RCP(x_192 + 1.0);
    const double x_194 = p[98]*x_192*x_193 + y[47]*x_191;
    const double x_246 = 4.0*y[47];
    dz[48] = SBM_SEL(state_lane, -p[48]*x_194, fma(-p[48]*(x_193*x_193)*(2.0*p[98] + y[47] + (y[48]*y[48])*x_246 + y[48]*x_246), z[48], fma(-p[48]*x_191, z[47], SBM_PICK(scol, 48, -x_194, 0.0))));
    const double x_195 = y[49] + (-1.0);
    const double x_196 = 2.0*y[49];
    const double x_197 = SBM_RCP(x_196 + 1.0);
    const double x_198 = p[99]*x_196*x_197 + y[48]*x_195;
    const double x_247 = 4.0*y[48];
    dz[49] = SBM_SEL(state_lane, -p[49]*x_198, fma(-p[49]*(x_197*x_197)*(2.0*p[99] + y[48] + (y[49]*y[49])*x_247 + y[49]*x_247), z[49], fma(-p[49]*x_195, z[48], SBM_PICK(scol, 49, -x_198, 0.0))));
  }

  static constexpr int RL_NCLASS = 2;
  static constexpr int RL_MAXYS = 2, RL_MAXPS = 2, RL_MAXJY = 2, RL_MAXJP = 1;
  static constexpr int RL_LARGEST_CLASS = 49;
  __device__ __forceinline__ static int rl_class(int row) { return SBM_RL_CLASS[row]; }
  __device__ __forceinline__ static int rl_ys(int slot, int row) { return SBM_RL_YS[slot * NV + row]; }
  __device__ __forceinline__ static int rl_ps(int slot, int row) { return SBM_RL_PS[slot * NV + row]; }
  __device__ __forceinline__ static int rl_jyout(int slot, int row) { return SBM_RL_JYOUT[slot * NV + row]; }
  __device__ __forceinline__ static int rl_apos(int slot, int row) { return SBM_RL_APOS[slot * NV + row]; }
  __device__ __forceinline__ static int rl_jpcol(int slot, int row) { return SBM_RL_JPCOL[slot * NV + row]; }
  __device__ __forceinline__ static int rl_jycol(int slot, int row) { return SBM_RL_JYCOL[slot * NV + row]; }
  __device__ __forceinline__ static void class_dispatch(int cls, double t, const double (&ys)[RL_MAXYS],
                                                        const double (&ps)[RL_MAXPS], double& f,
                                                        double (&jy)[RL_MAXJY], double (&jp)[RL_MAXJP]) {
    (void)t; (void)ys; (void)ps;
    const bool is0 = (cls == 0);
    const double c0_x0 = 2.0*ys[0];
    const double h0 = SBM_RCP((2.0*SBM_SEL(is0, ys[0], ys[1])) + 1.0);
    const double c0_x1 = h0;
    const double c0_x2 = ps[1]*c0_x0*c0_x1 + ys[0] + (-1.0);
    const double c1_x0 = ys[1] + (-1.0);
    const double c1_x1 = 2.0*ys[1];
    const double c1_x2 = h0;
    const double c1_x3 = ps[1]*c1_x1*c1_x2 + ys[0]*c1_x0;
    const double c1_x4 = 4.0*ys[0];
    f = SBM_SEL(is0, -ps[0]*c0_x2, -ps[0]*c1_x3);
    jy[0] = SBM_SEL(is0, -ps[0]*(c0_x1*c0_x1)*(2.0*ps[1] + 4.0*(ys[0]*ys[0]) + 4.0*ys[0] + 1.0), -ps[0]*c1_x0);
    jy[1] = SBM_SEL(is0, 0.0, -ps[0]*(c1_x2*c1_x2)*(2.0*ps[1] + ys[0] + (ys[1]*ys[1])*c1_x4 + ys[1]*c1_x4));
    jp[0] = SBM_SEL(is0, -c0_x2, -c1_x3);
  }

  static constexpr int RL_NSTATIC = 0;
  __device__ __forceinline__ static void rl_static(const double (&jy)[RL_MAXJY], double (&sj)[1]) {
    (void)jy;
    sj[0] = 0.0;
  }

  template <int NZ>
  __device__ __forceinline__ static void apply_rowlane(const double (&jy)[RL_MAXJY], const double (&sj)[1],
                                                       const double (&acol)[NV], const double (&z)[NZ],
                                                       double (&dz)[NZ]) {
    (void)jy; (void)sj;
    dz[0] = fma(SBM_LANE_BCAST(jy[0], 0), z[0], acol[0]);
    dz[1] = fma(SBM_LANE_BCAST(jy[1], 1), z[1], fma(SBM_LANE_BCAST(jy[0], 1), z[0], acol[1]));
    dz[2] = fma(SBM_LANE_BCAST(jy[1], 2), z[2], fma(SBM_LANE_BCAST(jy[0], 2), z[1], acol[2]));
    dz[3] = fma(SBM_LANE_BCAST(jy[1], 3), z[3], fma(SBM_LANE_BCAST(jy[0], 3), z[2], acol[3]));
    dz[4] = fma(SBM_LANE_BCAST(jy[1], 4), z[4], fma(SBM_LANE_BCAST(jy[0], 4), z[3], acol[4]));
    dz[5] = fma(SBM_LANE_BCAST(jy[1], 5), z[5], fma(SBM_LANE_BCAST(jy[0], 5), z[4], acol[5]));
    dz[6] = fma(SBM_LANE_BCAST(jy[1], 6), z[6], fma(SBM_LANE_BCAST(jy[0], 6), z[5], acol[6]));
    dz[7] = fma(SBM_LANE_BCAST(jy[1], 7), z[7], fma(SBM_LANE_BCAST(jy[0], 7), z[6], acol[7]));
    dz[8] = fma(SBM_LANE_BCAST(jy[1], 8), z[8], fma(SBM_LANE_BCAST(jy[0], 8), z[7], acol[8]));
    dz[9] = fma(SBM_LANE_BCAST(jy[1], 9), z[9], fma(SBM_LANE_BCAST(jy[0], 9), z[8], acol[9]));
    dz[10] = fma(SBM_LANE_BCAST(jy[1], 10), z[10], fma(SBM_LANE_BCAST(jy[0], 10), z[9], acol[10]));
    dz[11] = fma(SBM_LANE_BCAST(jy[1], 11), z[11], fma(SBM_LANE_BCAST(jy[0], 11), z[10], acol[11]));
    dz[12] = fma(SBM_LANE_BCAST(jy[1], 12), z[12], fma(SBM_LANE_BCAST(jy[0], 12), z[11], acol[12]));
    dz[13] = fma(SBM_LANE_BCAST(jy[1], 13), z[13], fma(SBM_LANE_BCAST(jy[0], 13), z[12], acol[13]));
    dz[14] = fma(SBM_LANE_BCAST(jy[1], 14), z[14], fma(SBM_LANE_BCAST(jy[0], 14), z[13], acol[14]));
    dz[15] = fma(SBM_LANE_BCAST(jy[1], 15), z[15], fma(SBM_LANE_BCAST(jy[0], 15), z[14], acol[15]));
    dz[16] = fma(SBM_LANE_BCAST(jy[1], 16), z[16], fma(SBM_LANE_BCAST(jy[0], 16), z[15], acol[16]));
    dz[17] = fma(SBM_LANE_BCAST(jy[1], 17), z[17], fma(SBM_LANE_BCAST(jy[0], 17), z[16], acol[17]));
    dz[18] = fma(SBM_LANE_BCAST(jy[1], 18), z[18], fma(SBM_LANE_BCAST(jy[0], 18), z[17], acol[18]));
    dz[19] = fma(SBM_LANE_BCAST(jy[1], 19), z[19], fma(SBM_LANE_BCAST(jy[0], 19), z[18], acol[19]));
    dz[20] = fma(SBM_LANE_BCAST(jy[1], 20), z[20], fma(SBM_LANE_BCAST(jy[0], 20), z[19], acol[20]));
    dz[21] = fma(SBM_LANE_BCAST(jy[1], 21), z[21], fma(SBM_LANE_BCAST(jy[0], 21), z[20], acol[21]));
    dz[22] = fma(SBM_LANE_BCAST(jy[1], 22), z[22], fma(SBM_LANE_BCAST(jy[0], 22), z[21], acol[22]));
    dz[23] = fma(SBM_LANE_BCAST(jy[1], 23), z[23], fma(SBM_LANE_BCAST(jy[0], 23), z[22], acol[23]));
    dz[24] = fma(SBM_LANE_BCAST(jy[1], 24), z[24], fma(SBM_LANE_BCAST(jy[0], 24), z[23], acol[24]));
    dz[25] = fma(SBM_LANE_BCAST(jy[1], 25), z[25], fma(SBM_LANE_BCAST(jy[0], 25), z[24], acol[25]));
    dz[26] = fma(SBM_LANE_BCAST(jy[1], 26), z[26], fma(SBM_LANE_BCAST(jy[0], 26), z[25], acol[26]));
    dz[27] = fma(SBM_LANE_BCAST(jy[1], 27), z[27], fma(SBM_LANE_BCAST(jy[0], 27), z[26], acol[27]));
    dz[28] = fma(SBM_LANE_BCAST(jy[1], 28), z[28], fma(SBM_LANE_BCAST(jy[0], 28), z[27], acol[28]));
    dz[29] = fma(SBM_LANE_BCAST(jy[1], 29), z[29], fma(SBM_LANE_BCAST(jy[0], 29), z[28], acol[29]));
    dz[30] = fma(SBM_LANE_BCAST(jy[1], 30), z[30], fma(SBM_LANE_BCAST(jy[0], 30), z[29], acol[30]));
    dz[31] = fma(SBM_LANE_BCAST(jy[1], 31), z[31], fma(SBM_LANE_BCAST(jy[0], 31), z[30], acol[31]));
    dz[32] = fma(SBM_LANE_BCAST(jy[1], 32), z[32], fma(SBM_LANE_BCAST(jy[0], 32), z[31], acol[32]));
    dz[33] = fma(SBM_LANE_BCAST(jy[1], 33), z[33], fma(SBM_LANE_BCAST(jy[0], 33), z[32], acol[33]));
    dz[34] = fma(SBM_LANE_BCAST(jy[1], 34), z[34], fma(SBM_LANE_BCAST(jy[0], 34), z[33], acol[34]));
    dz[35] = fma(SBM_LANE_BCAST(jy[1], 35), z[35], fma(SBM_LANE_BCAST(jy[0], 35), z[34], acol[35]));
    dz[36] = fma(SBM_LANE_BCAST(jy[1], 36), z[36], fma(SBM_LANE_BCAST(jy[0], 36), z[35], acol[36]));
    dz[37] = fma(SBM_LANE_BCAST(jy[1], 37), z[37], fma(SBM_LANE_BCAST(jy[0], 37), z[36], acol[37]));
    dz[38] = fma(SBM_LANE_BCAST(jy[1], 38), z[38], fma(SBM_LANE_BCAST(jy[0], 38), z[37], acol[38]));
    dz[39] = fma(SBM_LANE_BCAST(jy[1], 39), z[39], fma(SBM_LANE_BCAST(jy[0], 39), z[38], acol[39]));
    dz[40] = fma(SBM_LANE_BCAST(jy[1], 40), z[40], fma(SBM_LANE_BCAST(jy[0], 40), z[39], acol[40]));
    dz[41] = fma(SBM_LANE_BCAST(jy[1], 41), z[41], fma(SBM_LANE_BCAST(jy[0], 41), z[40], acol[41]));
    dz[42] = fma(SBM_LANE_BCAST(jy[1], 42), z[42], fma(SBM_LANE_BCAST(jy[0], 42), z[41], acol[42]));
    dz[43] = fma(SBM_LANE_BCAST(jy[1], 43), z[43], fma(SBM_LANE_BCAST(jy[0], 43), z[42], acol[43]));
    dz[44] = fma(SBM_LANE_BCAST(jy[1], 44), z[44], fma(SBM_LANE_BCAST(jy[0], 44), z[43], acol[44]));
    dz[45] = fma(SBM_LANE_BCAST(jy[1], 45), z[45], fma(SBM_LANE_BCAST(jy[0], 45), z[44], acol[45]));
    dz[46] = fma(SBM_LANE_BCAST(jy[1], 46), z[46], fma(SBM_LANE_BCAST(jy[0], 46), z[45], acol[46]));
    dz[47] = fma(SBM_LANE_BCAST(jy[1], 47), z[47], fma(SBM_LANE_BCAST(jy[0], 47), z[46], acol[47]));
    dz[48] = fma(SBM_LANE_BCAST(jy[1], 48), z[48], fma(SBM_LANE_BCAST(jy[0], 48), z[47], acol[48]));
    dz[49] = fma(SBM_LANE_BCAST(jy[1], 49), z[49], fma(SBM_LANE_BCAST(jy[0], 49), z[48], acol[49]));
  }

  template <int NZ>
  __device__ __forceinline__ static void apply_lds(const double* jyl, const double (&acol)[NV],
                                                   const double (&z)[NZ], double (&dz)[NZ]) {
    (void)jyl;
    dz[0] = fma(jyl[0], z[0], acol[0]);
    dz[1] = fma(jyl[3], z[1], fma(jyl[2], z[0], acol[1]));
    dz[2] = fma(jyl[5], z[2], fma(jyl[4], z[1], acol[2]));
    dz[3] = fma(jyl[7], z[3], fma(jyl[6], z[2], acol[3]));
    dz[4] = fma(jyl[9], z[4], fma(jyl[8], z[3], acol[4]));
    dz[5] = fma(jyl[11], z[5], fma(jyl[10], z[4], acol[5]));
    dz[6] = fma(jyl[13], z[6], fma(jyl[12], z[5], acol[6]));
    dz[7] = fma(jyl[15], z[7], fma(jyl[14], z[6], acol[7]));
    dz[8] = fma(jyl[17], z[8], fma(jyl[16], z[7], acol[8]));
    dz[9] = fma(jyl[19], z[9], fma(jyl[18], z[8], acol[9]));
    dz[10] = fma(jyl[21], z[10], fma(jyl[20], z[9], acol[10]));
    dz[11] = fma(jyl[23], z[11], fma(jyl[22], z[10], acol[11]));
    dz[12] = fma(jyl[25], z[12], fma(jyl[24], z[11], acol[12]));
    dz[13] = fma(jyl[27], z[13], fma(jyl[26], z[12], acol[13]));
    dz[14] = fma(jyl[29], z[14], fma(jyl[28], z[13], acol[14]));
    dz[15] = fma(jyl[31], z[15], fma(jyl[30], z[14], acol[15]));
    dz[16] = fma(jyl[33], z[16], fma(jyl[32], z[15], acol[16]));
    dz[17] = fma(jyl[35], z[17], fma(jyl[34], z[16], acol[17]));
    dz[18] = fma(jyl[37], z[18], fma(jyl[36], z[17], acol[18]));
    dz[19] = fma(jyl[39], z[19], fma(jyl[38], z[18], acol[19]));
    dz[20] = fma(jyl[41], z[20], fma(jyl[40], z[19], acol[20]));
    dz[21] = fma(jyl[43], z[21], fma(jyl[42], z[20], acol[21]));
    dz[22] = fma(jyl[45], z[22], fma(jyl[44], z[21], acol[22]));
    dz[23] = fma(jyl[47], z[23], fma(jyl[46], z[22], acol[23]));
    dz[24] = fma(jyl[49], z[24], fma(jyl[48], z[23], acol[24]));
    dz[25] = fma(jyl[51], z[25], fma(jyl[50], z[24], acol[25]));
    dz[26] = fma(jyl[53], z[26], fma(jyl[52], z[25], acol[26]));
    dz[27] = fma(jyl[55], z[27], fma(jyl[54], z[26], acol[27]));
    dz[28] = fma(jyl[57], z[28], fma(jyl[56], z[27], acol[28]));
    dz[29] = fma(jyl[59], z[29], fma(jyl[58], z[28], acol[29]));
    dz[30] = fma(jyl[61], z[30], fma(jyl[60], z[29], acol[30]));
    dz[31] = fma(jyl[63], z[31], fma(jyl[62], z[30], acol[31]));
    dz[32] = fma(jyl[65], z[32], fma(jyl[64], z[31], acol[32]));
    dz[33] = fma(jyl[67], z[33], fma(jyl[66], z[32], acol[33]));
    dz[34] = fma(jyl[69], z[34], fma(jyl[68], z[33], acol[34]));
    dz[35] = fma(jyl[71], z[35], fma(jyl[70], z[34], acol[35]));
    dz[36] = fma(jyl[73], z[36], fma(jyl[72], z[35], acol[36]));
    dz[37] = fma(jyl[75], z[37], fma(jyl[74], z[36], acol[37]));
    dz[38] = fma(jyl[77], z[38], fma(jyl[76], z[37], acol[38]));
    dz[39] = fma(jyl[79], z[39], fma(jyl[78], z[38], acol[39]));
    dz[40] = fma(jyl[81], z[40], fma(jyl[80], z[39], acol[40]));
    dz[41] = fma(jyl[83], z[41], fma(jyl[82], z[40], acol[41]));
    dz[42] = fma(jyl[85], z[42], fma(jyl[84], z[41], acol[42]));
    dz[43] = fma(jyl[87], z[43], fma(jyl[86], z[42], acol[43]));
    dz[44] = fma(jyl[89], z[44], fma(jyl[88], z[43], acol[44]));
    dz[45] = fma(jyl[91], z[45], fma(jyl[90], z[44], acol[45]));
    dz[46] = fma(jyl[93], z[46], fma(jyl[92], z[45], acol[46]));
    dz[47] = fma(jyl[95], z[47], fma(jyl[94], z[46], acol[47]));
    dz[48] = fma(jyl[97], z[48], fma(jyl[96], z[47], acol[48]));
    dz[49] = fma(jyl[99], z[49], fma(jyl[98], z[48], acol[49]));
  }

  struct RG0 {
  static constexpr bool RG_OK = true;
  static constexpr int RG_G = 6, RG_C = 10, RG_CPL = 1, RG_RPG = 9, RG_JYS = 2, RG_NHALO = 1;
  static constexpr int RG_NCH = 5;
  static constexpr int RG_LS = 64;
  __device__ __forceinline__ static int rg_pos(int row, int col) {
    return (row % RG_RPG) * RG_LS + RG_CPL * ((row / RG_RPG) * RG_C + col % RG_C) + col / RG_C;
  }
  __device__ __forceinline__ static int rg_jypos(int slot, int row) { return SBM_RG0_JYPOS[slot * NV + row]; }
  __device__ __forceinline__ static int rg_hsrc(int term, int group) { return SBM_RG0_HSRC[term * RG_G + group]; }
  template <int NZ>
  __device__ __forceinline__ static void publish_rowgroup(double* h_lane, const double (&z)[NZ]) {
    (void)h_lane; (void)z;
    h_lane[512] = z[8];
  }
  __device__ __forceinline__ static void load_rowgroup(const double* a_lane, const double* jy_lane,
                                                       double (&acol)[9], double (&coef)[18]) {
    coef[0] = jy_lane[0];
    coef[1] = jy_lane[1];
    coef[2] = jy_lane[2];
    coef[3] = jy_lane[3];
    coef[4] = jy_lane[4];
    coef[5] = jy_lane[5];
    coef[6] = jy_lane[6];
    coef[7] = jy_lane[7];
    coef[8] = jy_lane[8];
    coef[9] = jy_lane[9];
    coef[10] = jy_lane[10];
    coef[11] = jy_lane[11];
    coef[12] = jy_lane[12];
    coef[13] = jy_lane[13];
// ... 786 lines not shown
```

sysbio_modeling_amd/csrc/sbm_integrators.hpp:

```cpp
#pragma once
#include <type_traits>

#include <hip/hip_runtime.h>
#include <stdint.h>
#include "sbm_plugin.h"

#ifndef SBM_RCP_NR
#define SBM_RCP_NR 2
#endif
__device__ __forceinline__ double sbm_rcp(double x) {
  double r = __builtin_amdgcn_rcp(x);
#pragma unroll
  for (int it = 0; it < SBM_RCP_NR; ++it) {
    const double e = fma(-x, r, 1.0);
    r = fma(e, r, r);
  }
  return r;
}
#define SBM_RCP(x) sbm_rcp(x)
#define SBM_LDS_FENCE() __atomic_signal_fence(__ATOMIC_SEQ_CST)

__device__ __forceinline__ double sbm_pick(int scol, int c, double v, double otherwise) {
  return scol == c ? v : otherwise;
}
#define SBM_PICK(scol, c, v, otherwise) sbm_pick(scol, c, v, otherwise)
__device__ __forceinline__ double sbm_sel(bool c, double a, double b) { return c ? a : b; }
#define SBM_SEL(c, a, b) sbm_sel(c, a, b)
__device__ __forceinline__ double sbm_pick_col(int col, int c, double v, double otherwise) {
  const int chunk = __builtin_amdgcn_readfirstlane(col) >> 6;
  const unsigned long long mask = (c >> 6) == chunk ? (1ull << (c & 63)) : 0ull;
  return __builtin_amdgcn_inverse_ballot_w64(mask) ? v : otherwise;
}
#define SBM_PICK_COL(col, c, v, otherwise) sbm_pick_col(col, c, v, otherwise)
__device__ __forceinline__ double sbm_lane_bcast(double v, int src) {
  const int lo = __builtin_amdgcn_readlane(__double2loint(v), src);
  const int hi = __builtin_amdgcn_readlane(__double2hiint(v), src);
  return __hiloint2double(hi, lo);
}
#define SBM_LANE_BCAST(v, src) sbm_lane_bcast(v, src)

__device__ __forceinline__ double sbm_bcast0(double v) {
  int lo = __builtin_amdgcn_readfirstlane(__double2loint(v));
  int hi = __builtin_amdgcn_readfirstlane(__double2hiint(v));
  return __hiloint2double(hi, lo);
}
__device__ __forceinline__ float sbm_bcast0f(float v) {
  return __int_as_float(__builtin_amdgcn_readfirstlane(__float_as_int(v)));
}
template <int CTRL, int ROW_MASK>
__device__ __forceinline__ float sbm_dpp(float v) {
  return __int_as_float(__builtin_amdgcn_update_dpp(0, __float_as_int(v), CTRL, ROW_MASK, 0xf, false));
}
__device__ __forceinline__ float sbm_lane63f(float v) {
  return __int_as_float(__builtin_amdgcn_readlane(__float_as_int(v), 63));
}
template <int CTRL, int ROW_MASK>
__device__ __forceinline__ int sbm_dpp_smax(int x) {
  const int o = __builtin_amdgcn_update_dpp((int)0x80000000, x, CTRL, ROW_MASK, 0xf, false);
  return x > o ? x : o;
}
__device__ __forceinline__ float sbm_wave_max(float v) {
  int x = __float_as_int(v);
  x = sbm_dpp_smax<0xb1, 0xf>(x);
  x = sbm_dpp_smax<0x4e, 0xf>(x);
  x = sbm_dpp_smax<0x124, 0xf>(x);
  x = sbm_dpp_smax<0x128, 0xf>(x);
  x = sbm_dpp_smax<0x142, 0xa>(x);
  x = sbm_dpp_smax<0x143, 0xc>(x);
  return __int_as_float(__builtin_amdgcn_readlane(x, 63));
}
__device__ __forceinline__ float sbm_wave_sumf(float v) {
  v += sbm_dpp<0xb1, 0xf>(v);
  v += sbm_dpp<0x4e, 0xf>(v);
  v += sbm_dpp<0x124, 0xf>(v);
  v += sbm_dpp<0x128, 0xf>(v);
  v += sbm_dpp<0x142, 0xa>(v);
  v += sbm_dpp<0x143, 0xc>(v);
  return sbm_lane63f(v);
}
__device__ __forceinline__ float sbm_nan_to_inf(float v) { return (v != v) ? __builtin_inff() : v; }
__device__ __forceinline__ double sbm_wave_sum(double v) {
#pragma unroll
  for (int off = 32; off > 0; off >>= 1) v += __shfl_xor(v, off, 64);
  return sbm_bcast0(v);
}

namespace dp {
constexpr double C2 = 1.0 / 5.0, C3 = 3.0 / 10.0, C4 = 4.0 / 5.0, C5 = 8.0 / 9.0;
constexpr double A21 = 1.0 / 5.0;
constexpr double A31 = 3.0 / 40.0, A32 = 9.0 / 40.0;
constexpr double A41 = 44.0 / 45.0, A42 = -56.0 / 15.0, A43 = 32.0 / 9.0;
constexpr double A51 = 19372.0 / 6561.0, A52 = -25360.0 / 2187.0, A53 = 64448.0 / 6561.0, A54 = -212.0 / 729.0;
constexpr double A61 = 9017.0 / 3168.0, A62 = -355.0 / 33.0, A63 = 46732.0 / 5247.0, A64 = 49.0 / 176.0,
                 A65 = -5103.0 / 18656.0;
constexpr double A71 = 35.0 / 384.0, A73 = 500.0 / 1113.0, A74 = 125.0 / 192.0, A75 = -2187.0 / 6784.0,
                 A76 = 11.0 / 84.0;
constexpr double E1 = 71.0 / 57600.0, E3 = -71.0 / 16695.0, E4 = 71.0 / 1920.0, E5 = -17253.0 / 339200.0,
                 E6 = 22.0 / 525.0, E7 = -1.0 / 40.0;
}

namespace dp8 {
constexpr double C2 = 0.05260015195876773, C3 = 0.0789002279381516, C4 = 0.1183503419072274, C5 = 0.2816496580927726, C6 = 0.3333333333333333, C7 = 0.25, C8 = 0.3076923076923077, C9 = 0.6512820512820513, C10 = 0.6, C11 = 0.8571428571428571, C12 = 1.0;
constexpr double A2_1 = 0.05260015195876773;
constexpr double A3_1 = 0.0197250569845379, A3_2 = 0.0591751709536137;
constexpr double A4_1 = 0.02958758547680685, A4_3 = 0.08876275643042054;
constexpr double A5_1 = 0.2413651341592667, A5_3 = -0.8845494793282861, A5_4 = 0.924834003261792;
constexpr double A6_1 = 0.037037037037037035, A6_4 = 0.17082860872947386, A6_5 = 0.12546768756682242;
constexpr double A7_1 = 0.037109375, A7_4 = 0.17025221101954405, A7_5 = 0.06021653898045596, A7_6 = -0.017578125;
constexpr double A8_1 = 0.03709200011850479, A8_4 = 0.17038392571223998, A8_5 = 0.10726203044637328, A8_6 = -0.015319437748624402, A8_7 = 0.008273789163814023;
constexpr double A9_1 = 0.6241109587160757, A9_4 = -3.3608926294469414, A9_5 = -0.868219346841726, A9_6 = 27.59209969944671, A9_7 = 20.154067550477894, A9_8 = -43.48988418106996;
constexpr double A10_1 = 0.47766253643826434, A10_4 = -2.4881146199716677, A10_5 = -0.590290826836843, A10_6 = 21.230051448181193, A10_7 = 15.279233632882423, A10_8 = -33.28821096898486, A10_9 = -0.020331201708508627;
constexpr double A11_1 = -0.9371424300859873, A11_4 = 5.186372428844064, A11_5 = 1.0914373489967295, A11_6 = -8.149787010746927, A11_7 = -18.52006565999696, A11_8 = 22.739487099350505, A11_9 = 2.4936055526796523, A11_10 = -3.0467644718982196;
constexpr double A12_1 = 2.273310147516538, A12_4 = -10.53449546673725, A12_5 = -2.0008720582248625, A12_6 = -17.9589318631188, A12_7 = 27.94888452941996, A12_8 = -2.8589982771350235, A12_9 = -8.87285693353063, A12_10 = 12.360567175794303, A12_11 = 0.6433927460157636;
constexpr double B1 = 0.054293734116568765, B6 = 4.450312892752409, B7 = 1.8915178993145003, B8 = -5.801203960010585, B9 = 0.3111643669578199, B10 = -0.1521609496625161, B11 = 0.20136540080403034, B12 = 0.04471061572777259;
constexpr double E5_1 = 0.01312004499419488, E5_6 = -1.2251564463762044, E5_7 = -0.4957589496572502, E5_8 = 1.6643771824549864, E5_9 = -0.35032884874997366, E5_10 = 0.3341791187130175, E5_11 = 0.08192320648511571, E5_12 = -0.022355307863886294;
constexpr double E3_1 = -0.18980075407240762, E3_6 = 4.450312892752409, E3_7 = 1.8915178993145003, E3_8 = -5.801203960010585, E3_9 = -0.4226823213237919, E3_10 = -0.1521609496625161, E3_11 = 0.20136540080403034, E3_12 = 0.02265179219836082;
}

#define SBM_ALL(c, i)                       \
  _Pragma("unroll") for (int c = 0; c < CPL; ++c) \
  _Pragma("unroll") for (int i = 0; i < NVX; ++i)
#define SBM_MAIN(c, i)                      \
  _Pragma("unroll") for (int c = 0; c < CPL; ++c) \
  _Pragma("unroll") for (int i = 0; i < NV; ++i)
#define SBM_EXTRA(c, i)                     \
  _Pragma("unroll") for (int c = 0; c < CPL; ++c) \
  _Pragma("unroll") for (int i = NV; i < NVX; ++i)
#define SBM_ISSUE(tt, stmt)                 \
  {                                         \
    SBM_EXTRA(c, i) { stmt }                \
    pend_ = sys.issue((tt), zt);            \
  }
#define SBM_STAGE_THEN(tt, stmt, kout, next) \
  {                                         \
    auto tok_ = sys.eval(pend_, (tt));      \
    sys.extra_out(tok_, kout);              \
    next                                    \
    SBM_MAIN(c, i) { stmt }                 \
    sys.finish(tok_, (tt), zt, kout);       \
  }
#define SBM_STAGE(tt, stmt, kout) SBM_ISSUE(tt, stmt) SBM_STAGE_THEN(tt, stmt, kout, )

struct SbmLdsParams {
  const double* base;
  __device__ __forceinline__ double operator[](int c) const { return base[c * 64]; }
};

template <class D>
struct SbmNoRowPhase {
  struct Pending {};
  template <class Z>
  __device__ __forceinline__ Pending issue(double, const Z&) const { return Pending{}; }
  __device__ __forceinline__ int eval(const Pending&, double) const { return 0; }
  template <class Z>
  __device__ __forceinline__ void extra_out(int, Z&) const {}
  template <class Z>
  __device__ __forceinline__ void finish(int, double t, const Z& z, Z& dz) const { static_cast<const D*>(this)->rhs(t, z, dz); }
};

template <class M>
struct SensSystem : SbmNoRowPhase<SensSystem<M>> {
  static constexpr int NV = M::NV;
  static constexpr int NVX = M::NV;
  static constexpr int NCOL = 1 + M::NK;
  static constexpr int CPL = (NCOL + 63) / 64;
  static constexpr int NCS = CPL;
  __device__ __forceinline__ static constexpr int col_of(int c, int) { return c; }
  static constexpr bool kUniform = true;
  const double* __restrict__ p;
  int lane;

  __device__ __forceinline__ void rhs(double t, const double (&z)[CPL][NV], double (&dz)[CPL][NV]) const {
    double y[NV];
#pragma unroll
    for (int i = 0; i < NV; ++i) y[i] = sbm_bcast0(z[0][i]);
    if constexpr (CPL == 1) {
      M::eval_col(t, y, p, lane - 1, z[0], dz[0]);
    } else {
      double f[NV], jy[M::NJY], jp[M::NJP];
      M::eval_jac(t, y, p, f, jy, jp);
// ... 56 lines not shown
    if (a.n_reject) atomicMax(a.n_reject + traj, n_rej);
  } else {
    if (a.status) a.status[traj] = status;
    if (a.n_steps) a.n_steps[traj] = n_acc;
    if (a.n_reject) a.n_reject[traj] = n_rej;
  }
}

template <class Sys>
inline constexpr bool sbm_fold_step_size = true;
template <class M>
inline constexpr bool sbm_fold_step_size<SensSystem<M>> = (SensSystem<M>::CPL * M::NV <= 36);

template <class Sys, class Store>
__device__ __forceinline__ SbmTrajOut sbm_dopri45(const Sys& sys, double (&z)[Sys::CPL][Sys::NVX],
                                                   const double* __restrict__ t_out, int n_t,
                                                   const sbm_integrator_opts& o, Store&& store) {
  constexpr int NV = Sys::NV;
  constexpr int NVX = Sys::NVX;
  constexpr int CPL = Sys::CPL;
  using namespace dp;
  const double rtol = o.rtol, atol = o.atol;
  const bool early_exit = o.max_steps < 0;
  const int max_steps = o.max_steps > 0 ? o.max_steps : (o.max_steps < 0 ? -o.max_steps : 1000000);

  double k1[CPL][NVX], k2[CPL][NVX], k3[CPL][NVX], k4[CPL][NVX], k5[CPL][NVX], k6[CPL][NVX], zt[CPL][NVX];
  SBM_ALL(c, i) { k1[c][i] = 0.0; k2[c][i] = 0.0; k3[c][i] = 0.0; k4[c][i] = 0.0; k5[c][i] = 0.0; k6[c][i] = 0.0; zt[c][i] = 0.0; }
  double t = o.t0;
  SbmTrajOut out{SBM_OK, 0, 0};
  if (n_t <= 0) return out;
  const double t_span = t_out[n_t - 1] - o.t0;

  sys.rhs(t, z, k1);

  double h = o.h0;
  if (!(h > 0.0)) {
    double dnf = 0.0, dny = 0.0;
    SBM_ALL(c, i) {
      const double sk = atol + rtol * fabs(z[c][i]);
      const double a = k1[c][i] / sk, b = z[c][i] / sk;
      dnf = fma(a, a, dnf);
      dny = fma(b, b, dny);
    }
    dnf = sys.sum(dnf);
    dny = sys.sum(dny);
    h = (dnf <= 1e-10 || dny <= 1e-10) ? 1e-6 : sqrt(dny / dnf) * 0.01;
    h = fmin(h, t_span > 0.0 ? t_span : 1.0);
    SBM_ALL(c, i) zt[c][i] = fma(h, k1[c][i], z[c][i]);
    sys.rhs(t + h, zt, k2);
    double der2 = 0.0;
    SBM_ALL(c, i) {
      const double sk = atol + rtol * fabs(z[c][i]);
      const double a = (k2[c][i] - k1[c][i]) / sk;
      der2 = fma(a, a, der2);
    }
    der2 = sqrt(sys.sum(der2)) / h;
    const double der12 = fmax(fabs(der2), sqrt(dnf));
    const double h1 = (der12 <= 1e-15) ? fmax(1e-6, fabs(h) * 1e-3) : pow(0.01 / der12, 0.2);
    h = fmin(fmin(100.0 * h, h1), t_span > 0.0 ? t_span : 1.0);
    if (!(h > 0.0)) h = 1e-6;
  }

  int n_try = 0;
  bool failed = false;
  float h_mark = 0.f;
  int rej_mark = 0;
  typename Sys::Pending pend_;
  for (int io = 0; io < n_t; ++io) {
    const double target = t_out[io];
    while (!failed && t < target) {
      if (n_try >= max_steps) { out.status = SBM_MAX_STEPS; failed = true; break; }
      if (early_exit && n_try >= 512 && (n_try & 255) == 0) {
        const bool growing = (float)h > 1.5f * h_mark;
        const bool smooth = out.n_rej - rej_mark < 3;
        h_mark = (float)h;
        rej_mark = out.n_rej;
        if (!growing && !smooth && (t_out[n_t - 1] - t) > 1.5 * (double)(max_steps - n_try) * h) { out.status = SBM_MAX_STEPS; failed = true; break; }
      }
      ++n_try;
      double hs = h;
      bool last = false;
      if (t + 1.01 * hs >= target) { hs = target - t; last = true; }

      constexpr bool kFold = sbm_fold_step_size<Sys>;
      const double ha21 = hs * A21;
      double ha31, ha32, ha41, ha42, ha43, ha51, ha52, ha53, ha54, ha61, ha62, ha63, ha64, ha71, ha73, ha74, ha65, ha75,
          ha76;
#define SBM_S2 zt[c][i] = fma(ha21, k1[c][i], z[c][i]);
#define SBM_S3                                                                                    \
  if constexpr (kFold) zt[c][i] = fma(ha32, k2[c][i], fma(ha31, k1[c][i], z[c][i]));              \
  else zt[c][i] = fma(hs, fma(A32, k2[c][i], A31 * k1[c][i]), z[c][i]);
#define SBM_S4                                                                                               \
  if constexpr (kFold) zt[c][i] = fma(ha43, k3[c][i], fma(ha42, k2[c][i], fma(ha41, k1[c][i], z[c][i])));    \
  else zt[c][i] = fma(hs, fma(A43, k3[c][i], fma(A42, k2[c][i], A41 * k1[c][i])), z[c][i]);
#define SBM_S5                                                                                    \
  const double a1_ = k1[c][i], a2_ = k2[c][i], a3_ = k3[c][i], a4_ = k4[c][i], z_ = z[c][i];      \
  if constexpr (kFold) {                                                                          \
    zt[c][i] = fma(ha54, a4_, fma(ha53, a3_, fma(ha52, a2_, fma(ha51, a1_, z_))));                \
    k2[c][i] = fma(ha64, a4_, fma(ha63, a3_, fma(ha62, a2_, fma(ha61, a1_, z_))));        \
    k3[c][i] = fma(ha74, a4_, fma(ha73, a3_, fma(ha71, a1_, z_)));                        \
  } else {                                                                                        \
    zt[c][i] = fma(hs, fma(A54, a4_, fma(A53, a3_, fma(A52, a2_, A51 * a1_))), z_);               \
    k2[c][i] = fma(A64, a4_, fma(A63, a3_, fma(A62, a2_, A61 * a1_)));                            \
    k3[c][i] = fma(A74, a4_, fma(A73, a3_, A71 * a1_));                                           \
  }                                                                                               \
  k4[c][i] = fma(E4, a4_, fma(E3, a3_, E1 * a1_));
#define SBM_S6                                                        \
  const double a5_ = k5[c][i];                                        \
  if constexpr (kFold) zt[c][i] = fma(ha65, a5_, k2[c][i]);           \
  else zt[c][i] = fma(hs, fma(A65, a5_, k2[c][i]), z[c][i]);          \
  if constexpr (kFold) k3[c][i] = fma(ha75, a5_, k3[c][i]);           \
  else k3[c][i] = fma(A75, a5_, k3[c][i]);                            \
  k4[c][i] = fma(E5, a5_, k4[c][i]);
#define SBM_S7                                                        \
  const double a6_ = k6[c][i];                                        \
  if constexpr (kFold) zt[c][i] = fma(ha76, a6_, k3[c][i]);           \
  else zt[c][i] = fma(hs, fma(A76, a6_, k3[c][i]), z[c][i]);          \
  k4[c][i] = fma(E6, a6_, k4[c][i]);
#define SBM_P3 if constexpr (kFold) { ha31 = hs * A31; ha32 = hs * A32; }
#define SBM_P4 if constexpr (kFold) { ha41 = hs * A41; ha42 = hs * A42; ha43 = hs * A43; }
#define SBM_P5                                                               \
  if constexpr (kFold) {                                                     \
    ha51 = hs * A51; ha52 = hs * A52; ha53 = hs * A53; ha54 = hs * A54;      \
    ha61 = hs * A61; ha62 = hs * A62; ha63 = hs * A63; ha64 = hs * A64;      \
    ha71 = hs * A71; ha73 = hs * A73; ha74 = hs * A74;                       \
  }
#define SBM_P6 if constexpr (kFold) { ha65 = hs * A65; ha75 = hs * A75; }
#define SBM_P7 if constexpr (kFold) { ha76 = hs * A76; }
      SBM_ISSUE(t + C2 * hs, SBM_S2)
      SBM_STAGE_THEN(t + C2 * hs, SBM_S2, k2, SBM_P3 SBM_ISSUE(t + C3 * hs, SBM_S3))
      SBM_STAGE_THEN(t + C3 * hs, SBM_S3, k3, SBM_P4 SBM_ISSUE(t + C4 * hs, SBM_S4))
      SBM_STAGE_THEN(t + C4 * hs, SBM_S4, k4, SBM_P5 SBM_ISSUE(t + C5 * hs, SBM_S5))
      SBM_STAGE_THEN(t + C5 * hs, SBM_S5, k5, SBM_P6 SBM_ISSUE(t + hs, SBM_S6))
      SBM_STAGE_THEN(t + hs, SBM_S6, k6, SBM_P7 SBM_ISSUE(t + hs, SBM_S7))
      SBM_STAGE_THEN(t + hs, SBM_S7, k1, )
#undef SBM_S2
#undef SBM_S3
#undef SBM_S4
#undef SBM_S5
#undef SBM_S6
#undef SBM_S7
#undef SBM_P3
#undef SBM_P4
#undef SBM_P5
#undef SBM_P6
#undef SBM_P7

      float colsum[Sys::NCS];
#pragma unroll
      for (int c = 0; c < Sys::NCS; ++c) colsum[c] = 0.f;
      float xsum = 0.f;
      auto err_ratio = [&](int c, int i) {
        const double e = fma(E7, k1[c][i], k4[c][i]);
        const double sc = fma(rtol, fmax(fabs(z[c][i]), fabs(zt[c][i])), atol);
        return (float)e * __builtin_amdgcn_rcpf((float)sc);
      };
#pragma unroll
      for (int c = 0; c < CPL; ++c) {
#pragma unroll
        for (int i = 0; i < NV; ++i) {
          const float r = err_ratio(c, i);
          colsum[Sys::col_of(c, i)] = fmaf(r, r, colsum[Sys::col_of(c, i)]);
        }
#pragma unroll
        for (int i = NV; i < NVX; ++i) {
          const float r = err_ratio(c, i);
          xsum = fmaf(r, r, xsum);
        }
      }
      const float err = fabsf((float)hs) * sys.norm(colsum, xsum);

      const bool finite = (err == err) && (err < 3.0e38f);
      const bool accept = finite && (err <= 1.0f);
      float fac;
      if (!finite) {
        fac = 0.2f;
      } else {
        fac = 0.9f * __builtin_amdgcn_exp2f(-0.2f * __builtin_amdgcn_logf(fmaxf(err, 1e-30f)));
        fac = fminf(10.f, fmaxf(0.2f, fac));
      }
      if (accept) {
        ++out.n_acc;
        t = last ? target : t + hs;
        SBM_ALL(c, i) z[c][i] = zt[c][i];
        const double hn = hs * (double)fac;
        h = last ? fmax(hn, h) : hn;
      } else {
        ++out.n_rej;
        h = hs * (double)fminf(fac, 1.0f);
        if (!(h > 1e-14 * fmax(fabs(t), 1e-3))) {
          out.status = finite ? SBM_STEP_UNDERFLOW : SBM_NON_FINITE;
          failed = true;
        } else {
          sys.rhs(t, z, k1);
        }
      }
    }
    if (failed) {
      SBM_ALL(c, i) z[c][i] = __builtin_nan("");
    }
    store(io, z);
  }
  return out;
}

template <class Sys, class Store>
__device__ __forceinline__ SbmTrajOut sbm_dop853(const Sys& sys, double (&z)[Sys::CPL][Sys::NVX],
                                                  const double* __restrict__ t_out, int n_t,
                                                  const sbm_integrator_opts& o, Store&& store) {
  constexpr int NV = Sys::NV;
  constexpr int NVX = Sys::NVX;
  constexpr int CPL = Sys::CPL;
  using namespace dp8;
  const double rtol = o.rtol, atol = o.atol;
  const bool early_exit = o.max_steps < 0;
  const int max_steps = o.max_steps > 0 ? o.max_steps : (o.max_steps < 0 ? -o.max_steps : 1000000);

  double k1[CPL][NVX], kx[CPL][NVX], ky[CPL][NVX], k5[CPL][NVX], k7[CPL][NVX], k8[CPL][NVX], k9[CPL][NVX],
      k10[CPL][NVX], k11[CPL][NVX], k12[CPL][NVX], zt[CPL][NVX];
  SBM_ALL(c, i) {
    k1[c][i] = 0.0; kx[c][i] = 0.0; ky[c][i] = 0.0; k5[c][i] = 0.0; k7[c][i] = 0.0; k8[c][i] = 0.0; k9[c][i] = 0.0;
    k10[c][i] = 0.0; k11[c][i] = 0.0; k12[c][i] = 0.0; zt[c][i] = 0.0;
  }
  double t = o.t0;
  SbmTrajOut out{SBM_OK, 0, 0};
  if (n_t <= 0) return out;
  const double t_span = t_out[n_t - 1] - o.t0;

  sys.rhs(t, z, k1);

  double h = o.h0;
  if (!(h > 0.0)) {
    double dnf = 0.0, dny = 0.0;
    SBM_ALL(c, i) {
      const double sk = atol + rtol * fabs(z[c][i]);
      const double a = k1[c][i] / sk, b = z[c][i] / sk;
      dnf = fma(a, a, dnf);
      dny = fma(b, b, dny);
    }
    dnf = sys.sum(dnf);
    dny = sys.sum(dny);
    h = (dnf <= 1e-10 || dny <= 1e-10) ? 1e-6 : sqrt(dny / dnf) * 0.01;
    h = fmin(h, t_span > 0.0 ? t_span : 1.0);
    SBM_ALL(c, i) zt[c][i] = fma(h, k1[c][i], z[c][i]);
    sys.rhs(t + h, zt, kx);
    double der2 = 0.0;
    SBM_ALL(c, i) {
      const double sk = atol + rtol * fabs(z[c][i]);
      const double a = (kx[c][i] - k1[c][i]) / sk;
      der2 = fma(a, a, der2);
    }
    der2 = sqrt(sys.sum(der2)) / h;
    const double der12 = fmax(fabs(der2), sqrt(dnf));
    const double h1 = (der12 <= 1e-15) ? fmax(1e-6, fabs(h) * 1e-3) : pow(0.01 / der12, 0.125);
    h = fmin(fmin(100.0 * h, h1), t_span > 0.0 ? t_span : 1.0);
    if (!(h > 0.0)) h = 1e-6;
  }

  int n_try = 0;
  bool failed = false;
  float h_mark = 0.f;
  int rej_mark = 0;
  typename Sys::Pending pend_;
  for (int io = 0; io < n_t; ++io) {
    const double target = t_out[io];
    while (!failed && t < target) {
      if (n_try >= max_steps) { out.status = SBM_MAX_STEPS; failed = true; break; }
      if (early_exit && n_try >= 512 && (n_try & 255) == 0) {
        const bool growing = (float)h > 1.5f * h_mark;
        const bool smooth = out.n_rej - rej_mark < 3;
        h_mark = (float)h;
        rej_mark = out.n_rej;
        if (!growing && !smooth && (t_out[n_t - 1] - t) > 1.5 * (double)(max_steps - n_try) * h) { out.status = SBM_MAX_STEPS; failed = true; break; }
      }
      ++n_try;
      double hs = h;
      bool last = false;
      if (t + 1.01 * hs >= target) { hs = target - t; last = true; }

      const double ha21 = hs * A2_1;
#define SBM_D2 zt[c][i] = fma(ha21, k1[c][i], z[c][i]);
#define SBM_D3 zt[c][i] = fma(hs, fma(A3_2, kx[c][i], A3_1 * k1[c][i]), z[c][i]);
#define SBM_D4 zt[c][i] = fma(hs, fma(A4_3, ky[c][i], A4_1 * k1[c][i]), z[c][i]);
#define SBM_D5 zt[c][i] = fma(hs, fma(A5_4, kx[c][i], fma(A5_3, ky[c][i], A5_1 * k1[c][i])), z[c][i]);
#define SBM_D6 zt[c][i] = fma(hs, fma(A6_5, k5[c][i], fma(A6_4, kx[c][i], A6_1 * k1[c][i])), z[c][i]);
#define SBM_D7 zt[c][i] = fma(hs, fma(A7_6, ky[c][i], fma(A7_5, k5[c][i], fma(A7_4, kx[c][i], A7_1 * k1[c][i]))), z[c][i]);
#define SBM_D8                                                                                                      \
  zt[c][i] = fma(hs, fma(A8_7, k7[c][i], fma(A8_6, ky[c][i], fma(A8_5, k5[c][i], fma(A8_4, kx[c][i], A8_1 * k1[c][i])))), \
                 z[c][i]);
#define SBM_D9                                                                                                      \
  zt[c][i] = fma(hs, fma(A9_8, k8[c][i], fma(A9_7, k7[c][i], fma(A9_6, ky[c][i], fma(A9_5, k5[c][i],                 \
                 fma(A9_4, kx[c][i], A9_1 * k1[c][i]))))), z[c][i]);
#define SBM_D10                                                                                                     \
  zt[c][i] = fma(hs, fma(A10_9, k9[c][i], fma(A10_8, k8[c][i], fma(A10_7, k7[c][i], fma(A10_6, ky[c][i],             \
                 fma(A10_5, k5[c][i], fma(A10_4, kx[c][i], A10_1 * k1[c][i])))))), z[c][i]);
#define SBM_D11                                                                                                     \
  zt[c][i] = fma(hs, fma(A11_10, k10[c][i], fma(A11_9, k9[c][i], fma(A11_8, k8[c][i], fma(A11_7, k7[c][i],           \
                 fma(A11_6, ky[c][i], fma(A11_5, k5[c][i], fma(A11_4, kx[c][i], A11_1 * k1[c][i]))))))), z[c][i]);
#define SBM_D12                                                                                                     \
  zt[c][i] = fma(hs, fma(A12_11, k11[c][i], fma(A12_10, k10[c][i], fma(A12_9, k9[c][i], fma(A12_8, k8[c][i],         \
                 fma(A12_7, k7[c][i], fma(A12_6, ky[c][i], fma(A12_5, k5[c][i], fma(A12_4, kx[c][i],                 \
                 A12_1 * k1[c][i])))))))), z[c][i]);
      SBM_ISSUE(t + C2 * hs, SBM_D2)
      SBM_STAGE_THEN(t + C2 * hs, SBM_D2, kx, SBM_ISSUE(t + C3 * hs, SBM_D3))
      SBM_STAGE_THEN(t + C3 * hs, SBM_D3, ky, SBM_ISSUE(t + C4 * hs, SBM_D4))
      SBM_STAGE_THEN(t + C4 * hs, SBM_D4, kx, SBM_ISSUE(t + C5 * hs, SBM_D5))
      SBM_STAGE_THEN(t + C5 * hs, SBM_D5, k5, SBM_ISSUE(t + C6 * hs, SBM_D6))
// ... 1142 lines not shown
```

sysbio_modeling_amd/symbolic/emit.py:

```python
from __future__ import annotations

from collections import OrderedDict
from dataclasses import dataclass, field

import sympy
from sympy import Symbol, cse
from sympy.printing.c import C99CodePrinter

from . import sympy_tools
from . import emit_rowlane
from . import emit_rowgroup
from . import emit_implicit


_RCP = sympy.Function('SBM_RCP')


_cheapest_memo = {}


def _cheapest(expr):
    def cost(e):
        return sympy.count_ops(e, visual=False) + 8 * len([a for a in sympy.preorder_traversal(e)
                                                           if a.is_Pow and a.exp.is_number and a.exp.is_negative])
    order = []
    for node in sympy.preorder_traversal(expr):
        if isinstance(node, Symbol) and node not in order:
            order.append(node)
    fwd = {sym: Symbol('_q%d' % i) for i, sym in enumerate(order)}
    canon = expr.xreplace(fwd)
    key = sympy.srepr(canon)
    if key not in _cheapest_memo:
        best = canon
        for f in (sympy.factor, sympy.simplify):
            try:
                cand = f(canon)
            except Exception:
                continue
            if cost(cand) < cost(best):
                best = cand
        _cheapest_memo[key] = best
    return _cheapest_memo[key].xreplace({v: k for k, v in fwd.items()})


def _canon_rcp(expr):
    def is_neg_pow(e):
        return e.is_Pow and e.exp.is_number and e.exp.is_negative

    def repl(e):
        if e.exp.is_Integer:
            content, prim = e.base.as_content_primitive()
            if content != 1 and content.is_Rational and content > 0:
                return sympy.Pow(content, e.exp) * sympy.Pow(_RCP(prim), -e.exp)
            return sympy.Pow(_RCP(e.base), -e.exp)
        return _RCP(sympy.Pow(e.base, -e.exp))
    return expr.replace(is_neg_pow, repl)


@dataclass
class ModelSpec:
    name: str
    variables: list
    params: list
    equations: OrderedDict
    fixed: list = field(default_factory=list)

    @property
    def n_vars(self):
        return len(self.variables)

    @property
    def n_params(self):
        return len(self.params)

    @property
    def sens_params(self):
        return [p for p in self.params if p not in self.fixed]

    @property
    def n_sens(self):
        return len(self.sens_params)

    @classmethod
    def from_model_dict(cls, model_dict, name='Model'):
        if 'Expanded Equations' not in model_dict:
            sympy_tools.process_model_dict(model_dict)
        params = model_dict['Parameters']
        fixed = [p for p in params if params[p] == 'fixed']
        return cls(name=name, variables=list(model_dict['Variables'].keys()),
                   params=list(params.keys()),
                   equations=OrderedDict(model_dict['Expanded Equations']), fixed=fixed)

    @classmethod
    def from_text(cls, model, name='Model', fixed_params=None):
        md = sympy_tools.parse_model_file(model)
        sympy_tools.process_model_dict(md, fixed_params=fixed_params,
                                       calculate_model_sensitivities=False)
        return cls.from_model_dict(md, name=name)


class Derived:

    def __init__(self, spec: ModelSpec):
        self.spec = spec
        params = OrderedDict((p, 'fixed' if p in spec.fixed else Symbol(p)) for p in spec.params)
        jy, jp = sympy_tools.derive_sparse_jacobians(spec.equations, params)
        self.jy = jy
        self.jp = jp
        f_exprs = [_canon_rcp(sympy.sympify(spec.equations[v])) for v in spec.variables]
        all_exprs = f_exprs + [_canon_rcp(_cheapest(e)) for _, _, e in jy] + \
            [_canon_rcp(_cheapest(e)) for _, _, e in jp]
        self.repl_all, red_all = cse(all_exprs, symbols=sympy.numbered_symbols('x_'),
                                     optimizations='basic')
        n = len(f_exprs)
        self.f_c = all_exprs[:n]
        self.jy_c = all_exprs[n:n + len(jy)]
        self.jp_c = all_exprs[n + len(jy):]
        self.f_red = red_all[:n]
        self.jy_red = red_all[n:n + len(jy)]
        self.jp_red = red_all[n + len(jy):]
        self.repl_f, self.f_only = cse(f_exprs, symbols=sympy.numbered_symbols('x_'),
                                       optimizations='basic')
        self.jy_rows = [[] for _ in range(spec.n_vars)]
        for e, (r, c, _) in enumerate(jy):
            self.jy_rows[r].append((e, c))
        self.jp_rows = [[] for _ in range(spec.n_vars)]
        for e, (r, c, _) in enumerate(jp):
            self.jp_rows[r].append((e, c))
        self._order_slots_by_structure()

    def _order_slots_by_structure(self):
        from . import emit_rowlane
        n = self.spec.n_vars
        if n < 3:
            return
        names = set(self.spec.variables) | set(self.spec.params)
        blank = {Symbol(nm): Symbol('_') for nm in names}
        before = len(emit_rowlane.find_classes(self.spec, self)[0])
        if before <= 1:
            return
        old = [list(r) for r in self.jy_rows]
        self.jy_rows = [sorted(r, key=lambda ec, i=i: (sympy.srepr(self.jy_c[ec[0]].xreplace(blank)), (ec[1] - i) % n))
                        for i, r in enumerate(old)]
        if len(emit_rowlane.find_classes(self.spec, self)[0]) >= before:
            self.jy_rows = old


class _ExprPrinter(C99CodePrinter):

    def __init__(self, symbol_map, rcp="(1.0/(%s))", lang='c'):
        super().__init__({'strict': False} if 'strict' in C99CodePrinter._default_settings else {})
        self._smap = symbol_map
        self._rcp = rcp
        self._lang = lang
        self.shared = {}

    @staticmethod
    def normalised(expr):
        return sympy.sympify(expr).replace(
            lambda e: e.is_Pow and e.exp.is_number and e.exp.is_negative,
            lambda e: _RCP(sympy.Pow(e.base, -e.exp)))

    def doprint(self, expr, assign_to=None):
        return super().doprint(self.normalised(expr), assign_to)

    def _print(self, expr, **kwargs):
        if self.shared and isinstance(expr, sympy.Basic):
            name = self.shared.get(expr)
            if name is not None:
                return name
        return super()._print(expr, **kwargs)

    def _print_Function(self, expr):
        if expr.func == _RCP:
            return self._rcp % self._print(expr.args[0])
        return super()._print_Function(expr)

    def _print_Symbol(self, expr):
        return self._smap.get(expr.name, expr.name)

    def _print_Rational(self, expr):
        return "(%d.0/%d.0)" % (expr.p, expr.q)

    def _print_Integer(self, expr):
        return "%d.0" % int(expr.p) if int(expr.p) >= 0 else "(%d.0)" % int(expr.p)

    def _mulpow(self, base, n):
        b = self._print(base)
        if not (base.is_Symbol or base.is_Number):
            b = "(%s)" % b
        return "(" + "*".join([b] * n) + ")"

    def _print_Pow(self, expr):
        base, exp = expr.as_base_exp()
        if exp.is_Integer:
            n = int(exp)
            if 1 <= n <= 4:
                return self._mulpow(base, n)
            if -4 <= n <= -1:
                inner = self._print(base) if n == -1 else self._mulpow(base, -n)
                return self._rcp % inner
        if exp == sympy.Rational(1, 2):
            return "sqrt(%s)" % self._print(base)
        if exp == sympy.Rational(-1, 2):
            return self._rcp % ("sqrt(%s)" % self._print(base))
        return "pow(%s, %s)" % (self._print(base), self._print(exp))


def _symbol_map(spec, y_fmt="y[%d]", p_fmt="p[%d]"):
    m = {}
    for i, v in enumerate(spec.variables):
        m[v] = y_fmt % i
    for i, p in enumerate(spec.params):
        m[p] = p_fmt % i
    m['t'] = 't'
    return m


def _fmt_header(spec, comment):
    c = comment
    lines = [
        "%s generated by sysbio_modeling_amd.symbolic.emit -- do not edit" % c,
        "%s model '%s': %d states, %d parameters (%d with sensitivities)"
        % (c, spec.name, spec.n_vars, spec.n_params, spec.n_sens),
        "%s states: %s" % (c, ", ".join(spec.variables)),
        "%s params: %s" % (c, ", ".join(spec.params)),
    ]
    if spec.fixed:
        lines.append("%s fixed : %s" % (c, ", ".join(spec.fixed)))
    return lines


def emit_python(spec: ModelSpec, derived: Derived = None) -> str:
    d = derived or Derived(spec)
    n, k = spec.n_vars, spec.n_sens
    pr = _ExprPrinter(_symbol_map(spec), rcp="(1.0/(%s))", lang='py')
    pad = "    "
    L = _fmt_header(spec, "#")
    L += ["from math import exp, log, sqrt, pow, sin, cos, tanh", "",
          "ordered_params = [%s]" % ", ".join("'%s'" % p for p in spec.params),
          "sens_params = [%s]" % ", ".join("'%s'" % p for p in spec.sens_params),
          "n_vars = %d" % n, "n_sens = %d" % k, "", ""]
    L += ["def model(y, t, yout, p):"]
    for s, e in d.repl_f:
        L.append(pad + "%s = %s" % (s, pr.doprint(e)))
    for i, e in enumerate(d.f_only):
        L.append(pad + "yout[%d] = (%s)" % (i, pr.doprint(e)))
    L += ["", "", "def sens_model(y, t, yout, p):"]
    for s, e in d.repl_all:
        L.append(pad + "%s = %s" % (s, pr.doprint(e)))
    for i, e in enumerate(d.f_red):
        L.append(pad + "yout[%d] = (%s)" % (i, pr.doprint(e)))
    for e_idx, e in enumerate(d.jy_red):
        L.append(pad + "jy_%d = %s" % (e_idx, pr.doprint(e)))
    for e_idx, e in enumerate(d.jp_red):
        L.append(pad + "jp_%d = %s" % (e_idx, pr.doprint(e)))
    for i in range(n):
        for j in range(k):
            terms = ["jy_%d*y[%d]" % (e_idx, n + c * k + j) for e_idx, c in d.jy_rows[i]]
            terms += ["jp_%d" % e_idx for e_idx, c in d.jp_rows[i] if c == j]
            L.append(pad + "yout[%d] = (%s)" % (n + i * k + j, " + ".join(terms) if terms else "0.0"))
    L.append("")
    return "\n".join(L)


def emit_python_jacobians(spec: ModelSpec, derived: Derived = None) -> str:
    d = derived or Derived(spec)
    n, k = spec.n_vars, spec.n_sens
    pr = _ExprPrinter(_symbol_map(spec), rcp="(1.0/(%s))", lang='py')
    pad = "    "
    ysyms = [Symbol(v) for v in spec.variables]
    hy, hp = [], []
    for e_idx, (i, l, expr) in enumerate(d.jy):
        for m, ym in enumerate(ysyms):
            if ym in expr.free_symbols:
                dd = sympy.diff(expr, ym)
                if dd != 0:
                    hy.append((i, l, m, _canon_rcp(_cheapest(dd))))
    for e_idx, (i, j, expr) in enumerate(d.jp):
        for m, ym in enumerate(ysyms):
            if ym in expr.free_symbols:
                dd = sympy.diff(expr, ym)
                if dd != 0:
                    hp.append((i, j, m, _canon_rcp(_cheapest(dd))))
    exprs = list(d.jy_c) + [h[3] for h in hy] + [h[3] for h in hp]
    repl, red = cse(exprs, symbols=sympy.numbered_symbols('x_'), optimizations='basic')
    jy_red = red[:len(d.jy)]
    hy_red = red[len(d.jy):len(d.jy) + len(hy)]
    hp_red = red[len(d.jy) + len(hy):]
    L = ["from math import exp, log, sqrt, pow, sin, cos, tanh", "", "",
         "def model_jac(y, t, jacout, p):"]
    repl_y, red_y = cse(list(d.jy_c), symbols=sympy.numbered_symbols('x_'), optimizations='basic')
    for s_, e in repl_y:
        L.append(pad + "%s = %s" % (s_, pr.doprint(e)))
    for (i, m, _), e in zip(d.jy, red_y):
        L.append(pad + "jacout[%d, %d] = (%s)" % (m, i, pr.doprint(e)))
    if not d.jy:
        L.append(pad + "pass")
    L += ["", "", "def sens_model_jac(y, t, jacout, p):"]
    for s_, e in repl:
        L.append(pad + "%s = %s" % (s_, pr.doprint(e)))
    for e_idx, ((i, l, _), e) in enumerate(zip(d.jy, jy_red)):
        L.append(pad + "jy_%d = %s" % (e_idx, pr.doprint(e)))
        L.append(pad + "jacout[%d, %d] = jy_%d" % (l, i, e_idx))
        if k:
            L.append(pad + "for j in range(%d):" % k)
            L.append(pad * 2 + "jacout[%d + j, %d + j] = jy_%d" % (n + l * k, n + i * k, e_idx))
    by_im = OrderedDict()
    for (i, l, m, _), e in zip(hy, hy_red):
        by_im.setdefault((i, m), dict(hy=[], hp=[]))['hy'].append((l, e))
    for (i, j, m, _), e in zip(hp, hp_red):
        by_im.setdefault((i, m), dict(hy=[], hp=[]))['hp'].append((j, e))
    for q, ((i, m), terms) in enumerate(by_im.items()):
        names = []
        for t_idx, (l, e) in enumerate(terms['hy']):
            L.append(pad + "h_%d_%d = %s" % (q, t_idx, pr.doprint(e)))
            names.append(("h_%d_%d" % (q, t_idx), l))
        if names and k:
            L.append(pad + "for j in range(%d):" % k)
            L.append(pad * 2 + "jacout[%d, %d + j] = %s" % (
                m, n + i * k, " + ".join("%s*y[%d + j]" % (nm, n + l * k) for nm, l in names)))
        elif k and terms['hp']:
            L.append(pad + "for j in range(%d):" % k)
            L.append(pad * 2 + "jacout[%d, %d + j] = 0.0" % (m, n + i * k))
        for j, e in terms['hp']:
            L.append(pad + "jacout[%d, %d] += (%s)" % (m, n + i * k + j, pr.doprint(e)))
    if not d.jy and not by_im:
        L.append(pad + "pass")
    L.append("")
    return "\n".join(L)


def emit_c(spec: ModelSpec, derived: Derived = None) -> str:
    d = derived or Derived(spec)
    n, k = spec.n_vars, spec.n_sens
    pr = _ExprPrinter(_symbol_map(spec), rcp="(1.0/(%s))", lang='c')
    L = _fmt_header(spec, "//")
    L += ["#include <math.h>", "",
          "int sbm_n_vars(void) { return %d; }" % n,
          "int sbm_n_params(void) { return %d; }" % spec.n_params,
          "int sbm_n_sens(void) { return %d; }" % k, ""]
    L += ["void sbm_rhs(const double* y, double t, double* yout, const double* p) {", "  (void)t;"]
    for s, e in d.repl_f:
        L.append("  const double %s = %s;" % (s, pr.doprint(e)))
    for i, e in enumerate(d.f_only):
        L.append("  yout[%d] = %s;" % (i, pr.doprint(e)))
    L += ["}", ""]
    nnz_y, nnz_p = max(len(d.jy), 1), max(len(d.jp), 1)
    L += ["static const int JY_ROW[%d] = {%s};" % (nnz_y, ", ".join(str(r) for r, _, _ in d.jy) or "0"),
          "static const int JY_COL[%d] = {%s};" % (nnz_y, ", ".join(str(c) for _, c, _ in d.jy) or "0"),
          "static const int JP_ROW[%d] = {%s};" % (nnz_p, ", ".join(str(r) for r, _, _ in d.jp) or "0"),
          "static const int JP_COL[%d] = {%s};" % (nnz_p, ", ".join(str(c) for _, c, _ in d.jp) or "0"), ""]
    L += ["// augmented system: yout[n + i*k + j] = J_p[i][j] + sum_m J_y[i][m] * y[n + m*k + j]",
          "void sbm_sens_rhs(const double* y, double t, double* yout, const double* p) {", "  (void)t;",
          "  enum { N = %d, K = %d, NNZ_Y = %d, NNZ_P = %d };" % (n, k, len(d.jy), len(d.jp)),
          "  double jy[%d], jp[%d];" % (nnz_y, nnz_p)]
    for s, e in d.repl_all:
        L.append("  const double %s = %s;" % (s, pr.doprint(e)))
    for i, e in enumerate(d.f_red):
        L.append("  yout[%d] = %s;" % (i, pr.doprint(e)))
    for e_idx, e in enumerate(d.jy_red):
        L.append("  jy[%d] = %s;" % (e_idx, pr.doprint(e)))
    for e_idx, e in enumerate(d.jp_red):
        L.append("  jp[%d] = %s;" % (e_idx, pr.doprint(e)))
    L += ["  for (int i = N; i < N + N * K; ++i) yout[i] = 0.0;",
          "  for (int e = 0; e < NNZ_Y; ++e) {",
          "    const double a = jy[e]; const double* src = y + N + JY_COL[e] * K; double* dst = yout + N + JY_ROW[e] * K;",
          "    for (int j = 0; j < K; ++j) dst[j] += a * src[j];",
          "  }",
          "  for (int e = 0; e < NNZ_P; ++e) yout[N + JP_ROW[e] * K + JP_COL[e]] += jp[e];",
          "}", ""]
    return "\n".join(L)


def emit_hip(spec: ModelSpec, derived: Derived = None, class_hoist: bool = True) -> str:
    d = derived or Derived(spec)
    n, k = spec.n_vars, spec.n_sens
    pr = _ExprPrinter(_symbol_map(spec), rcp="SBM_RCP(%s)", lang='hip')
    nnz_y, nnz_p = max(len(d.jy), 1), max(len(d.jp), 1)
    L = _fmt_header(spec, "//")
    rl_tables, rl_meta = emit_rowlane.emit_rowlane_tables(spec, d, None)
    rg_tables, rg_layout = emit_rowgroup.emit_tables(spec, d, tag='RG0')
    rg_tables1, rg_layout1 = emit_rowgroup.emit_tables(spec, d, tag='RG1', latency=True)
    rg_tables2, rg_layout2 = emit_rowgroup.emit_tables(spec, d, tag='RG2', dop853=True)
    rg_tables = rg_tables + rg_tables1 + rg_tables2
    im_members, im_meta = emit_implicit.emit_members(spec, d)
    im_tables = emit_implicit.emit_tables(spec, d, im_meta)
    L += ["#pragma once", ""] + rl_tables + rg_tables + im_tables + [
          "struct SbmModel {",
          "  static constexpr int NV = %d;      // state variables" % n,
          "  static constexpr int NP = %d;      // model parameters (length of p)" % spec.n_params,
          "  static constexpr int NK = %d;      // non-fixed parameters = sensitivity columns" % k,
          "  static constexpr int NNZ_JY = %d;  // non-zeros of df/dy" % len(d.jy),
          "  static constexpr int NNZ_JP = %d;  // non-zeros of df/dp" % len(d.jp),
          "  static constexpr int NJY = %d;" % nnz_y,
          "  static constexpr int NJP = %d;" % nnz_p,
          "  static constexpr const char* NAME = \"%s\";" % spec.name, ""]
    L += ["  template <class PA>",
          "  __device__ __forceinline__ static void eval_f(double t, const double (&y)[NV], const PA& p,",
          "                                                double (&f)[NV]) {", "    (void)t;"]
    for s, e in d.repl_f:
        L.append("    const double %s = %s;" % (s, pr.doprint(e)))
    for i, e in enumerate(d.f_only):
        L.append("    f[%d] = %s;" % (i, pr.doprint(e)))
    L += ["  }", ""]
    L += ["  template <class PA>",
          "  __device__ __forceinline__ static void eval_jac(double t, const double (&y)[NV], const PA& p,",
          "                                                  double (&f)[NV], double (&jy)[NJY], double (&jp)[NJP]) {",
          "    (void)t;"]
    for s, e in d.repl_all:
        L.append("    const double %s = %s;" % (s, pr.doprint(e)))
    for i, e in enumerate(d.f_red):
        L.append("    f[%d] = %s;" % (i, pr.doprint(e)))
    for e_idx, e in enumerate(d.jy_red):
        L.append("    jy[%d] = %s;" % (e_idx, pr.doprint(e)))
    for e_idx, e in enumerate(d.jp_red):
        L.append("    jp[%d] = %s;" % (e_idx, pr.doprint(e)))
    if not d.jy:
        L.append("    jy[0] = 0.0;")
    if not d.jp:
        L.append("    jp[0] = 0.0;")
    L += ["  }", ""]
    L += ["  // one sensitivity column: dz = J_y z + J_p[:, scol]   (scol < 0: no J_p term)",
          "  __device__ __forceinline__ static void apply_col(const double (&jy)[NJY], const double (&jp)[NJP],",
          "                                                   int scol, const double (&z)[NV], double (&dz)[NV]) {"]
    for i in range(n):
        sel = "0.0"
        for e_idx, c in reversed(d.jp_rows[i]):
            sel = "SBM_PICK(scol, %d, jp[%d], %s)" % (c, e_idx, sel)
        expr = sel
        for e_idx, c in d.jy_rows[i]:
            expr = "fma(jy[%d], z[%d], %s)" % (e_idx, c, expr)
        L.append("    dz[%d] = %s;" % (i, expr))
    L += ["  }", ""]
    L += ["  // fused eval_jac + apply_col for ONE column per lane: scol < 0 -> dz = f (state lane),",
          "  // scol in [0, NK) -> dz = J_y z + J_p[:, scol]",
          "  template <class PA>",
          "  __device__ __forceinline__ static void eval_col(double t, const double (&y)[NV], const PA& p, int scol,",
          "                                                  const double (&z)[NV], double (&dz)[NV]) {",
          "    (void)t;", "    const bool state_lane = scol < 0;"]
    temp_expr = OrderedDict((s, e) for s, e in d.repl_all)
    emitted = set()

    def need(expr, out):
        for s in sorted(expr.free_symbols, key=lambda x: x.name):
            if s in temp_expr and s not in emitted and s not in out:
                need(temp_expr[s], out)
                out.append(s)

    for i in range(n):
        exprs = [d.f_red[i]] + [d.jy_red[e] for e, _ in d.jy_rows[i]] + [d.jp_red[e] for e, _ in d.jp_rows[i]]
        todo = []
        for e in exprs:
            need(e, todo)
        for s in todo:
            L.append("    const double %s = %s;" % (s, pr.doprint(temp_expr[s])))
            emitted.add(s)
        sel = "0.0"
        for e_idx, c in reversed(d.jp_rows[i]):
            sel = "SBM_PICK(scol, %d, %s, %s)" % (c, pr.doprint(d.jp_red[e_idx]), sel)
        expr = sel
        for e_idx, c in d.jy_rows[i]:
            expr = "fma(%s, z[%d], %s)" % (pr.doprint(d.jy_red[e_idx]), c, expr)
        L.append("    dz[%d] = SBM_SEL(state_lane, %s, %s);" % (i, pr.doprint(d.f_red[i]), expr))
    L += ["  }", ""]

    L += emit_rowlane.emit_rowlane_members(spec, d, rl_meta,
                                           lambda smap: _ExprPrinter(smap, rcp="SBM_RCP(%s)", lang='hip'),
                                           hoist=class_hoist)
    L += [""] + emit_rowgroup.emit_members(spec, d, rg_layout, tag='RG0')
    L += emit_rowgroup.emit_members(spec, d, rg_layout1, tag='RG1', alias_of='RG0')
    L += emit_rowgroup.emit_members(spec, d, rg_layout2, tag='RG2', alias_of='RG0')
    L += [""] + im_members + [
        "  __device__ __forceinline__ static int im_rstart(int row) { return SBM_IM_RSTART[IM_TRI ? row : 0]; }",
        "  __device__ __forceinline__ static int im_diagslot(int row) { return SBM_IM_DIAGSLOT[IM_TRI ? row : 0]; }",
        "  __device__ __forceinline__ static int im_mfpos(int slot, int row) { return SBM_IM_MFPOS[IM_TRI ? slot * NV + row : 0]; }"]
    L += ["};", ""]
    return "\n".join(L)
```

sysbio_modeling_amd/symbolic/emit_rowlane.py:

```python
from __future__ import annotations

import re
from collections import OrderedDict

import sympy
from sympy import Symbol, cse


def _canonical(bundle, var_index, par_index):
    ys, ps = [], []
    mapping = {}
    for expr in bundle:
        for node in sympy.preorder_traversal(expr):
            if isinstance(node, Symbol) and node not in mapping:
                if node.name in var_index:
                    mapping[node] = Symbol('YS_%d' % len(ys))
                    ys.append(var_index[node.name])
                elif node.name in par_index:
                    mapping[node] = Symbol('PS_%d' % len(ps))
                    ps.append(par_index[node.name])
    canon = tuple(e.xreplace(mapping) for e in bundle)
    return canon, ys, ps


def find_classes(spec, d):
    var_index = {v: i for i, v in enumerate(spec.variables)}
    par_index = {p: i for i, p in enumerate(spec.params)}
    classes = OrderedDict()
    row_info = []
    for i in range(spec.n_vars):
        bundle = [d.f_c[i]] + [d.jy_c[e] for e, _ in d.jy_rows[i]] + [d.jp_c[e] for e, _ in d.jp_rows[i]]
        canon, ys, ps = _canonical(bundle, var_index, par_index)
        key = (sympy.srepr(canon), len(d.jy_rows[i]), len(d.jp_rows[i]))
        if key not in classes:
            classes[key] = dict(canon=canon, rows=[], n_jy=len(d.jy_rows[i]), n_jp=len(d.jp_rows[i]),
                                n_ys=len(ys), n_ps=len(ps))
        classes[key]['rows'].append(i)
        row_info.append(dict(cls=list(classes.keys()).index(key), ys=ys, ps=ps))
    return list(classes.values()), row_info


def emit_rowlane_tables(spec, d, printer_factory):
    classes, row_info = find_classes(spec, d)
    n = spec.n_vars
    max_ys = max([c['n_ys'] for c in classes] + [1])
    max_ps = max([c['n_ps'] for c in classes] + [1])
    max_jy = max([c['n_jy'] for c in classes] + [1])
    max_jp = max([c['n_jp'] for c in classes] + [1])
    tag = "SBM_RL"

    def table(name, rows_of_slots):
        flat = ", ".join(str(v) for slot in rows_of_slots for v in slot)
        return "__constant__ short %s_%s[%d] = {%s};" % (tag, name, len(rows_of_slots) * n, flat)

    ys_t = [[(row_info[i]['ys'][s] if s < len(row_info[i]['ys']) else 0) for i in range(n)] for s in range(max_ys)]
    ps_t = [[(row_info[i]['ps'][s] if s < len(row_info[i]['ps']) else 0) for i in range(n)] for s in range(max_ps)]
    nj = max(len(d.jy), 1)
    jy_t = [[(d.jy_rows[i][s][0] if s < len(d.jy_rows[i]) else nj) for i in range(n)] for s in range(max_jy)]
    jp_t = [[(i * 64 + d.jp_rows[i][s][1] if s < len(d.jp_rows[i]) else n * 64) for i in range(n)]
            for s in range(max_jp)]
    jpc_t = [[(d.jp_rows[i][s][1] if s < len(d.jp_rows[i]) else -1) for i in range(n)] for s in range(max_jp)]
    jyc_t = [[(d.jy_rows[i][s][1] if s < len(d.jy_rows[i]) else -1) for i in range(n)] for s in range(max_jy)]
    L = ["// row-lane tables: [slot][row]",
         "__constant__ short %s_CLASS[%d] = {%s};" % (tag, n, ", ".join(str(r['cls']) for r in row_info)),
         table("YS", ys_t), table("PS", ps_t), table("JYOUT", jy_t), table("APOS", jp_t), table("JPCOL", jpc_t),
         table("JYCOL", jyc_t), ""]
    meta = dict(classes=classes, max_ys=max_ys, max_ps=max_ps, max_jy=max_jy, max_jp=max_jp)
    return L, meta


_OP_COST = {'rcp': 8, 'sqrt': 16, 'exp': 40, 'log': 40, 'pow': 80, 'call': 40, 'add': 1, 'mul': 1}
_SEL_COST = 2
_LEAF = re.compile(r'(?<![A-Za-z0-9_])(?:ys\[\d+\]|ps\[\d+\]|c\d+_x\d+|h\d+|t)(?![A-Za-z0-9_])')
_NAME = re.compile(r'(?<![A-Za-z0-9_])(?:c\d+_x\d+|h\d+)(?![A-Za-z0-9_])')


def _op_kind(node):
    if node.is_Function:
        return {'SBM_RCP': 'rcp', 'exp': 'exp', 'log': 'log'}.get(node.func.__name__, 'call')
    if node.is_Pow:
        if node.exp.is_Integer and 1 <= int(node.exp) <= 4:
            return 'mul'
        return 'sqrt' if node.exp == sympy.Rational(1, 2) else 'pow'
    if node.is_Add:
        return 'add'
    if node.is_Mul:
        return 'mul'
    return None


def _tree_cost(node):
    kind = _op_kind(node)
    if kind is None:
        return 0
    n = int(node.exp) - 1 if node.is_Pow and kind == 'mul' else max(len(node.args) - 1, 1)
    return _OP_COST[kind] * n + sum(_tree_cost(a) for a in node.args)


def _plan_hoist(per_class, pr):
    n_cls = len(per_class)
    shared = [{} for _ in range(n_cls)]
    hoisted = []
    rejected = set()
    exprs = [[pr.normalised(e) for _, e in repl] + [pr.normalised(e) for e in red] for repl, red in per_class]
    temps = [[str(s) for s, _ in repl] for repl, _ in per_class]

    def depends(name, on, seen):
        if name in seen:
            return False
        seen.add(name)
        for ci in range(n_cls):
            if name in temps[ci]:
                pr.shared = shared[ci]
                uses = _NAME.findall(pr.doprint(exprs[ci][temps[ci].index(name)]))
                break
        else:
            h = next(h for h in hoisted if h['name'] == name)
            uses = [x for lv in h['leaves'].values() for x in lv if _NAME.fullmatch(x)]
        return any(u == on or depends(u, on, seen) for u in uses)

    def printed(ci, node):
        pr.shared = {k: v for k, v in shared[ci].items() if k != node}
        for (sym, _), e in zip(per_class[ci][0], exprs[ci]):
            if _op_kind(e) == 'mul':
                pr.shared[sym] = "(%s)" % pr._print(e)
        text = pr._print(node)
        return _LEAF.sub('@', text), _LEAF.findall(text)

    def n_selects(leaves):
        return sum(len(pos) - max(pos.count(x) for x in pos) for pos in zip(*leaves))

    def cyclic(h):
        feeds = [x for lv in h['leaves'].values() for x in lv if _NAME.fullmatch(x)]
        return any(depends(x, h['name'], set()) for x in feeds)

    while True:
        groups = OrderedDict()
        for ci in range(n_cls):
            seen, count = set(), {}
            for e in exprs[ci]:
                walk = sympy.preorder_traversal(e)
                for node in walk:
                    if node in shared[ci]:
                        walk.skip()
                        continue
                    if node in seen or _op_kind(node) in (None, 'add', 'mul'):
                        continue
                    seen.add(node)
                    shape, leaves = printed(ci, node)
                    occ = count.get(shape, 0)
                    count[shape] = occ + 1
                    groups.setdefault((shape, occ), OrderedDict())[ci] = (node, leaves)
        best = None
        for key, members in groups.items():
            if len(members) < 2 or key in rejected:
                continue
            cost = _tree_cost(next(iter(members.values()))[0])
            gain = cost * (len(members) - 1) - _SEL_COST * n_selects([lv for _, lv in members.values()])
            if gain > 0 and (best is None or cost > best[0]):
                best = (cost, key, members)
        if best is None:
            break
        _, key, members = best
        name = 'h%d' % len(hoisted)
        h = dict(name=name, shape=key[0], classes=list(members), nodes={ci: nd for ci, (nd, _) in members.items()},
                 leaves={ci: lv for ci, (_, lv) in members.items()})
        hoisted.append(h)
        for ci, (node, _) in members.items():
            shared[ci][node] = name
        if cyclic(h):
            hoisted.pop()
            for ci, (node, _) in members.items():
                del shared[ci][node]
            rejected.add(key)
    for h in hoisted:
        again = {ci: printed(ci, h['nodes'][ci]) for ci in h['classes']}
        if len({shape for shape, _ in again.values()}) == 1:
            old = (h['shape'], h['leaves'])
            h['shape'], h['leaves'] = next(iter(again.values()))[0], {ci: lv for ci, (_, lv) in again.items()}
            if cyclic(h):
                h['shape'], h['leaves'] = old
    pr.shared = {}
    return shared, hoisted


def _sel_template(h):
    cls = h['classes']
    parts = h['shape'].split('@')
    out = [parts[0]]
    for pos in range(len(parts) - 1):
        col = [h['leaves'][ci][pos] for ci in cls]
        expr = max(col, key=lambda x: (col.count(x), len(col) - col[::-1].index(x)))
        default = expr
        for ci in reversed(cls):
            if h['leaves'][ci][pos] != default:
                expr = "SBM_SEL(is%d, %s, %s)" % (ci, h['leaves'][ci][pos], expr)
        out += [expr, parts[pos + 1]]
    return "".join(out)


def emit_rowlane_members(spec, d, meta, make_printer, hoist=True):
    n = spec.n_vars
    classes = meta['classes']
    L = ["  // ---- row-lane form (sbm_sens_rowlane_kernel) ----",
         "  static constexpr int RL_NCLASS = %d;" % len(classes),
         "  static constexpr int RL_MAXYS = %d, RL_MAXPS = %d, RL_MAXJY = %d, RL_MAXJP = %d;"
         % (meta['max_ys'], meta['max_ps'], meta['max_jy'], meta['max_jp']),
         "  static constexpr int RL_LARGEST_CLASS = %d;  // rows evaluated side by side" %
         max(len(c['rows']) for c in classes),
         "  // table accessors (the tables are namespace-scope __constant__ arrays above)",
         "  __device__ __forceinline__ static int rl_class(int row) { return SBM_RL_CLASS[row]; }",
         "  __device__ __forceinline__ static int rl_ys(int slot, int row) { return SBM_RL_YS[slot * NV + row]; }",
         "  __device__ __forceinline__ static int rl_ps(int slot, int row) { return SBM_RL_PS[slot * NV + row]; }",
         "  __device__ __forceinline__ static int rl_jyout(int slot, int row) { return SBM_RL_JYOUT[slot * NV + row]; }",
         "  __device__ __forceinline__ static int rl_apos(int slot, int row) { return SBM_RL_APOS[slot * NV + row]; }",
         "  __device__ __forceinline__ static int rl_jpcol(int slot, int row) { return SBM_RL_JPCOL[slot * NV + row]; }",
         "  __device__ __forceinline__ static int rl_jycol(int slot, int row) { return SBM_RL_JYCOL[slot * NV + row]; }",
         "  // one class body per distinct kinetic form; lane = row, operands per lane",
         "  __device__ __forceinline__ static void class_dispatch(int cls, double t, const double (&ys)[RL_MAXYS],",
         "                                                        const double (&ps)[RL_MAXPS], double& f,",
         "                                                        double (&jy)[RL_MAXJY], double (&jp)[RL_MAXJP]) {",
         "    (void)t; (void)ys; (void)ps;"]
    smap = {'t': 't'}
    for s in range(meta['max_ys']):
        smap['YS_%d' % s] = 'ys[%d]' % s
    for s in range(meta['max_ps']):
        smap['PS_%d' % s] = 'ps[%d]' % s
    pr = make_printer(smap)
    last = len(classes) - 1
    for ci in range(last):
        L.append("    const bool is%d = (cls == %d);" % (ci, ci))
    is_last_at = len(L)
    per_class = [cse(list(c['canon']), symbols=sympy.numbered_symbols('c%d_x' % ci), optimizations='basic')
                 for ci, c in enumerate(classes)]
    shared, hoisted = _plan_hoist(per_class, pr) if hoist and len(classes) > 1 else ([{} for _ in classes], [])
    stmts = OrderedDict()
    for ci, (repl, _) in enumerate(per_class):
        pr.shared = shared[ci]
        for sym, e in repl:
            stmts[str(sym)] = "    const double %s = %s;" % (sym, pr.doprint(e))
    for h in hoisted:
        stmts[h['name']] = "    const double %s = %s;   // classes %s" % (
            h['name'], _sel_template(h), ", ".join(str(ci) for ci in h['classes']))
    emitted = set()

    def emit_stmt(name):
        if name in emitted:
            return
        emitted.add(name)
        for dep in _NAME.findall(stmts[name].split('=', 1)[1]):
            if dep in stmts:
                emit_stmt(dep)
        L.append(stmts[name])

    bodies = []
    for ci, c in enumerate(classes):
        L.append("    // class %d: rows %s" % (ci, ", ".join(str(r) for r in c['rows'])))
        pr.shared = shared[ci]
        for sym, _ in per_class[ci][0]:
            emit_stmt(str(sym))
        bodies.append([pr.doprint(e) for e in per_class[ci][1]])
    pr.shared = {}
    for h in hoisted:
        emit_stmt(h['name'])
    if any("(is%d," % last in ln for ln in L[is_last_at:]):
        L.insert(is_last_at, "    const bool is%d = (cls == %d);" % (last, last))

    def chain(kind, k):
        def of(ci):
            c = classes[ci]
            if kind == 'f':
                return bodies[ci][0]
            if kind == 'jy':
                return bodies[ci][1 + k] if k < c['n_jy'] else "0.0"
            return bodies[ci][1 + c['n_jy'] + k] if k < c['n_jp'] else "0.0"
        expr = of(last)
        for ci in range(last - 1, -1, -1):
            expr = "SBM_SEL(is%d, %s, %s)" % (ci, of(ci), expr)
        return expr

    L.append("    f = %s;" % chain('f', 0))
    for k in range(meta['max_jy']):
        L.append("    jy[%d] = %s;" % (k, chain('jy', k)))
    for k in range(meta['max_jp']):
        L.append("    jp[%d] = %s;" % (k, chain('jp', k)))
    where = {}
    for i in range(n):
        for k, (e_idx, c) in enumerate(d.jy_rows[i]):
            where[e_idx] = (i, k)
    var_names = set(spec.variables)
    static_idx = {}
    for e_idx in sorted(where):
        syms = {str(x) for x in d.jy_c[e_idx].free_symbols}
        if not (syms & var_names) and 't' not in syms:
            static_idx[e_idx] = len(static_idx)
    nst = max(len(static_idx), 1)
    L += ["  }", "",
          "  static constexpr int RL_NSTATIC = %d;   // J_y entries that depend on parameters only" % len(static_idx),
          "  // run once per kernel, after one class_dispatch: broadcast the static entries",
          "  __device__ __forceinline__ static void rl_static(const double (&jy)[RL_MAXJY], double (&sj)[%d]) {" % nst,
          "    (void)jy;"]
    if not static_idx:
        L.append("    sj[0] = 0.0;")
    for e_idx, si in static_idx.items():
        r, k = where[e_idx]
        L.append("    sj[%d] = SBM_LANE_BCAST(jy[%d], %d);" % (si, k, r))
    L += ["  }", "",
          "  // dz = J_y z + acol, one sensitivity column per lane.  A state-dependent J_y[i,m] sits in",
          "  // register jy[slot] of row lane i: SBM_LANE_BCAST (v_readlane, literal lane) turns it into a",
          "  // scalar operand; static entries come from sj; acol[i] = A[i][lane] was fetched from LDS.",
          "  template <int NZ>",
          "  __device__ __forceinline__ static void apply_rowlane(const double (&jy)[RL_MAXJY], const double (&sj)[%d]," % nst,
          "                                                       const double (&acol)[NV], const double (&z)[NZ],",
          "                                                       double (&dz)[NZ]) {",
          "    (void)jy; (void)sj;"]
    for i in range(n):
        expr = "acol[%d]" % i
        for e_idx, c in d.jy_rows[i]:
            if e_idx in static_idx:
                expr = "fma(sj[%d], z[%d], %s)" % (static_idx[e_idx], c, expr)
            else:
                r, k = where[e_idx]
                expr = "fma(SBM_LANE_BCAST(jy[%d], %d), z[%d], %s)" % (k, r, c, expr)
        L.append("    dz[%d] = %s;" % (i, expr))
    L += ["  }", "",
          "  // the same product with the J_y entries read from a table jyl[row * RL_MAXJY + slot] (LDS): the form of the",
          "  // packed kernel, where several trajectories share a wavefront and a lane cannot name its row lane literally",
          "  template <int NZ>",
          "  __device__ __forceinline__ static void apply_lds(const double* jyl, const double (&acol)[NV],",
          "                                                   const double (&z)[NZ], double (&dz)[NZ]) {",
          "    (void)jyl;"]
    for i in range(n):
        expr = "acol[%d]" % i
        for k, (e_idx, c) in enumerate(d.jy_rows[i]):
            expr = "fma(jyl[%d], z[%d], %s)" % (i * meta['max_jy'] + k, c, expr)
        L.append("    dz[%d] = %s;" % (i, expr))
    L += ["  }"]
    return L
```

Before: 430.7 million ODE-steps/s.

## Search slot assignments to unify class dispatch and fuse max-abs in error norm

The code generator now searches over per-class placements of ys/ps/jy/jp slots so the rowlane classes share algebraic forms. This removes SBM_SEL selects from class_dispatch, for example in cascade20 where the reciprocal and several Jacobian entries become select-free, and the constant tables are regenerated to match. The error-ratio computation also replaces fmax(fabs,fabs) with a single v_max_f64 using absolute-value modifiers via inline asm. The risks are the extra generator complexity and the correctness of the regenerated index tables.

```diff
diff --git a/sysbio_modeling_amd/csrc/models/cascade20.hpp b/sysbio_modeling_amd/csrc/models/cascade20.hpp
--- a/sysbio_modeling_amd/csrc/models/cascade20.hpp
+++ b/sysbio_modeling_amd/csrc/models/cascade20.hpp
@@ -1,20 +1,20 @@
 #pragma once
 
 __constant__ short SBM_RL_CLASS[20] = {0, 1, 1, 1, 1, 1, 1, 1, 1, 1, 1, 1, 1, 1, 1, 1, 1, 1, 1, 1};
-__constant__ short SBM_RL_YS[40] = {19, 1, 2, 3, 4, 5, 6, 7, 8, 9, 10, 11, 12, 13, 14, 15, 16, 17, 18, 19, 0, 0, 1, 2, 3, 4, 5, 6, 7, 8, 9, 10, 11, 12, 13, 14, 15, 16, 17, 18};
-__constant__ short SBM_RL_PS[40] = {0, 21, 22, 23, 24, 25, 26, 27, 28, 29, 30, 31, 32, 33, 34, 35, 36, 37, 38, 39, 20, 1, 2, 3, 4, 5, 6, 7, 8, 9, 10, 11, 12, 13, 14, 15, 16, 17, 18, 19};
-__constant__ short SBM_RL_JYOUT[40] = {0, 2, 4, 6, 8, 10, 12, 14, 16, 18, 20, 22, 24, 26, 28, 30, 32, 34, 36, 38, 1, 3, 5, 7, 9, 11, 13, 15, 17, 19, 21, 23, 25, 27, 29, 31, 33, 35, 37, 39};
+__constant__ short SBM_RL_YS[40] = {19, 0, 1, 2, 3, 4, 5, 6, 7, 8, 9, 10, 11, 12, 13, 14, 15, 16, 17, 18, 0, 1, 2, 3, 4, 5, 6, 7, 8, 9, 10, 11, 12, 13, 14, 15, 16, 17, 18, 19};
+__constant__ short SBM_RL_PS[40] = {0, 1, 2, 3, 4, 5, 6, 7, 8, 9, 10, 11, 12, 13, 14, 15, 16, 17, 18, 19, 20, 21, 22, 23, 24, 25, 26, 27, 28, 29, 30, 31, 32, 33, 34, 35, 36, 37, 38, 39};
+__constant__ short SBM_RL_JYOUT[40] = {0, 3, 5, 7, 9, 11, 13, 15, 17, 19, 21, 23, 25, 27, 29, 31, 33, 35, 37, 39, 1, 2, 4, 6, 8, 10, 12, 14, 16, 18, 20, 22, 24, 26, 28, 30, 32, 34, 36, 38};
 __constant__ short SBM_RL_APOS[40] = {0, 65, 130, 195, 260, 325, 390, 455, 520, 585, 650, 715, 780, 845, 910, 975, 1040, 1105, 1170, 1235, 20, 85, 150, 215, 280, 345, 410, 475, 540, 605, 670, 735, 800, 865, 930, 995, 1060, 1125, 1190, 1255};
 __constant__ short SBM_RL_JPCOL[40] = {0, 1, 2, 3, 4, 5, 6, 7, 8, 9, 10, 11, 12, 13, 14, 15, 16, 17, 18, 19, 20, 21, 22, 23, 24, 25, 26, 27, 28, 29, 30, 31, 32, 33, 34, 35, 36, 37, 38, 39};
-__constant__ short SBM_RL_JYCOL[40] = {0, 0, 1, 2, 3, 4, 5, 6, 7, 8, 9, 10, 11, 12, 13, 14, 15, 16, 17, 18, 19, 1, 2, 3, 4, 5, 6, 7, 8, 9, 10, 11, 12, 13, 14, 15, 16, 17, 18, 19};
-
-__constant__ short SBM_RG0_JYPOS[40] = {0, 3, 5, 7, 9, 11, 13, 15, 17, 19, 21, 23, 25, 27, 29, 31, 33, 35, 37, 39, 1, 2, 4, 6, 8, 10, 12, 14, 16, 18, 20, 22, 24, 26, 28, 30, 32, 34, 36, 38};
+__constant__ short SBM_RL_JYCOL[40] = {0, 1, 2, 3, 4, 5, 6, 7, 8, 9, 10, 11, 12, 13, 14, 15, 16, 17, 18, 19, 19, 0, 1, 2, 3, 4, 5, 6, 7, 8, 9, 10, 11, 12, 13, 14, 15, 16, 17, 18};
+
+__constant__ short SBM_RG0_JYPOS[40] = {0, 2, 4, 6, 8, 10, 12, 14, 16, 18, 20, 22, 24, 26, 28, 30, 32, 34, 36, 38, 1, 3, 5, 7, 9, 11, 13, 15, 17, 19, 21, 23, 25, 27, 29, 31, 33, 35, 37, 39};
 __constant__ short SBM_RG0_HSRC[3] = {19, 6, 13};
 
-__constant__ short SBM_RG1_JYPOS[40] = {0, 3, 5, 7, 9, 11, 13, 15, 17, 19, 21, 23, 25, 27, 29, 31, 33, 35, 37, 39, 1, 2, 4, 6, 8, 10, 12, 14, 16, 18, 20, 22, 24, 26, 28, 30, 32, 34, 36, 38};
+__constant__ short SBM_RG1_JYPOS[40] = {0, 2, 4, 6, 8, 10, 12, 14, 16, 18, 20, 22, 24, 26, 28, 30, 32, 34, 36, 38, 1, 3, 5, 7, 9, 11, 13, 15, 17, 19, 21, 23, 25, 27, 29, 31, 33, 35, 37, 39};
 __constant__ short SBM_RG1_HSRC[7] = {19, 2, 5, 8, 11, 14, 17};
 
-__constant__ short SBM_RG2_JYPOS[40] = {0, 3, 5, 7, 9, 11, 13, 15, 17, 19, 21, 23, 25, 27, 29, 31, 33, 35, 37, 39, 1, 2, 4, 6, 8, 10, 12, 14, 16, 18, 20, 22, 24, 26, 28, 30, 32, 34, 36, 38};
+__constant__ short SBM_RG2_JYPOS[40] = {0, 2, 4, 6, 8, 10, 12, 14, 16, 18, 20, 22, 24, 26, 28, 30, 32, 34, 36, 38, 1, 3, 5, 7, 9, 11, 13, 15, 17, 19, 21, 23, 25, 27, 29, 31, 33, 35, 37, 39};
 __constant__ short SBM_RG2_HSRC[3] = {19, 6, 13};
 
 __constant__ short SBM_IM_RSTART[1] = {0};
@@ -271,39 +271,41 @@
                                                         double (&jy)[RL_MAXJY], double (&jp)[RL_MAXJP]) {
     (void)t; (void)ys; (void)ps;
     const bool is0 = (cls == 0);
-    const double h0 = SBM_RCP(SBM_SEL(is0, ys[0], ys[1]) + 1.0);
+    const double h0 = SBM_RCP(ys[0] + 1.0);
     const double c0_x0 = h0;
     const double c1_x0 = h0;
-    f = SBM_SEL(is0, ps[0]*c0_x0 - ps[1]*ys[1], -ps[0]*ys[0] + ps[1]*ys[1]*c1_x0);
-    jy[0] = SBM_SEL(is0, -ps[1], ps[1]*(c1_x0*c1_x0));
-    jy[1] = SBM_SEL(is0, -ps[0]*(c0_x0*c0_x0), -ps[0]);
-    jp[0] = SBM_SEL(is0, c0_x0, ys[1]*c1_x0);
-    jp[1] = SBM_SEL(is0, -ys[1], -ys[0]);
+    const double c1_x1 = ys[0]*c1_x0;
+    const double h1 = ps[0]*SBM_SEL(is0, c0_x0, c1_x1) - ps[1]*ys[1];
+    f = h1;
+    jy[0] = -ps[1];
+    jy[1] = SBM_SEL(is0, -ps[0]*(c0_x0*c0_x0), ps[0]*(c1_x0*c1_x0));
+    jp[0] = SBM_SEL(is0, c0_x0, c1_x1);
+    jp[1] = -ys[1];
   }
 
   static constexpr int RL_NSTATIC = 20;
   __device__ __forceinline__ static void rl_static(const double (&jy)[RL_MAXJY], double (&sj)[20]) {
     (void)jy;
     sj[0] = SBM_LANE_BCAST(jy[0], 0);
-    sj[1] = SBM_LANE_BCAST(jy[1], 1);
-    sj[2] = SBM_LANE_BCAST(jy[1], 2);
-    sj[3] = SBM_LANE_BCAST(jy[1], 3);
-    sj[4] = SBM_LANE_BCAST(jy[1], 4);
-    sj[5] = SBM_LANE_BCAST(jy[1], 5);
-    sj[6] = SBM_LANE_BCAST(jy[1], 6);
-    sj[7] = SBM_LANE_BCAST(jy[1], 7);
-    sj[8] = SBM_LANE_BCAST(jy[1], 8);
-    sj[9] = SBM_LANE_BCAST(jy[1], 9);
-    sj[10] = SBM_LANE_BCAST(jy[1], 10);
-    sj[11] = SBM_LANE_BCAST(jy[1], 11);
-    sj[12] = SBM_LANE_BCAST(jy[1], 12);
-    sj[13] = SBM_LANE_BCAST(jy[1], 13);
-    sj[14] = SBM_LANE_BCAST(jy[1], 14);
-    sj[15] = SBM_LANE_BCAST(jy[1], 15);
-    sj[16] = SBM_LANE_BCAST(jy[1], 16);
-    sj[17] = SBM_LANE_BCAST(jy[1], 17);
-    sj[18] = SBM_LANE_BCAST(jy[1], 18);
-    sj[19] = SBM_LANE_BCAST(jy[1], 19);
+    sj[1] = SBM_LANE_BCAST(jy[0], 1);
+    sj[2] = SBM_LANE_BCAST(jy[0], 2);
+    sj[3] = SBM_LANE_BCAST(jy[0], 3);
+    sj[4] = SBM_LANE_BCAST(jy[0], 4);
+    sj[5] = SBM_LANE_BCAST(jy[0], 5);
+    sj[6] = SBM_LANE_BCAST(jy[0], 6);
+    sj[7] = SBM_LANE_BCAST(jy[0], 7);
+    sj[8] = SBM_LANE_BCAST(jy[0], 8);
+    sj[9] = SBM_LANE_BCAST(jy[0], 9);
+    sj[10] = SBM_LANE_BCAST(jy[0], 10);
+    sj[11] = SBM_LANE_BCAST(jy[0], 11);
+    sj[12] = SBM_LANE_BCAST(jy[0], 12);
+    sj[13] = SBM_LANE_BCAST(jy[0], 13);
+    sj[14] = SBM_LANE_BCAST(jy[0], 14);
+    sj[15] = SBM_LANE_BCAST(jy[0], 15);
+    sj[16] = SBM_LANE_BCAST(jy[0], 16);
+    sj[17] = SBM_LANE_BCAST(jy[0], 17);
+    sj[18] = SBM_LANE_BCAST(jy[0], 18);
+    sj[19] = SBM_LANE_BCAST(jy[0], 19);
   }
 
   template <int NZ>
@@ -312,25 +314,25 @@
                                                        double (&dz)[NZ]) {
     (void)jy; (void)sj;
     dz[0] = fma(SBM_LANE_BCAST(jy[1], 0), z[19], fma(sj[0], z[0], acol[0]));
-    dz[1] = fma(sj[1], z[1], fma(SBM_LANE_BCAST(jy[0], 1), z[0], acol[1]));
-    dz[2] = fma(sj[2], z[2], fma(SBM_LANE_BCAST(jy[0], 2), z[1], acol[2]));
-    dz[3] = fma(sj[3], z[3], fma(SBM_LANE_BCAST(jy[0], 3), z[2], acol[3]));
-    dz[4] = fma(sj[4], z[4], fma(SBM_LANE_BCAST(jy[0], 4), z[3], acol[4]));
-    dz[5] = fma(sj[5], z[5], fma(SBM_LANE_BCAST(jy[0], 5), z[4], acol[5]));
-    dz[6] = fma(sj[6], z[6], fma(SBM_LANE_BCAST(jy[0], 6), z[5], acol[6]));
-    dz[7] = fma(sj[7], z[7], fma(SBM_LANE_BCAST(jy[0], 7), z[6], acol[7]));
-    dz[8] = fma(sj[8], z[8], fma(SBM_LANE_BCAST(jy[0], 8), z[7], acol[8]));
-    dz[9] = fma(sj[9], z[9], fma(SBM_LANE_BCAST(jy[0], 9), z[8], acol[9]));
-    dz[10] = fma(sj[10], z[10], fma(SBM_LANE_BCAST(jy[0], 10), z[9], acol[10]));
-    dz[11] = fma(sj[11], z[11], fma(SBM_LANE_BCAST(jy[0], 11), z[10], acol[11]));
-    dz[12] = fma(sj[12], z[12], fma(SBM_LANE_BCAST(jy[0], 12), z[11], acol[12]));
-    dz[13] = fma(sj[13], z[13], fma(SBM_LANE_BCAST(jy[0], 13), z[12], acol[13]));
-    dz[14] = fma(sj[14], z[14], fma(SBM_LANE_BCAST(jy[0], 14), z[13], acol[14]));
-    dz[15] = fma(sj[15], z[15], fma(SBM_LANE_BCAST(jy[0], 15), z[14], acol[15]));
-    dz[16] = fma(sj[16], z[16], fma(SBM_LANE_BCAST(jy[0], 16), z[15], acol[16]));
-    dz[17] = fma(sj[17], z[17], fma(SBM_LANE_BCAST(jy[0], 17), z[16], acol[17]));
-    dz[18] = fma(sj[18], z[18], fma(SBM_LANE_BCAST(jy[0], 18), z[17], acol[18]));
-    dz[19] = fma(sj[19], z[19], fma(SBM_LANE_BCAST(jy[0], 19), z[18], acol[19]));
+    dz[1] = fma(sj[1], z[1], fma(SBM_LANE_BCAST(jy[1], 1), z[0], acol[1]));
+    dz[2] = fma(sj[2], z[2], fma(SBM_LANE_BCAST(jy[1], 2), z[1], acol[2]));
+    dz[3] = fma(sj[3], z[3], fma(SBM_LANE_BCAST(jy[1], 3), z[2], acol[3]));
+    dz[4] = fma(sj[4], z[4], fma(SBM_LANE_BCAST(jy[1], 4), z[3], acol[4]));
+    dz[5] = fma(sj[5], z[5], fma(SBM_LANE_BCAST(jy[1], 5), z[4], acol[5]));
+    dz[6] = fma(sj[6], z[6], fma(SBM_LANE_BCAST(jy[1], 6), z[5], acol[6]));
+    dz[7] = fma(sj[7], z[7], fma(SBM_LANE_BCAST(jy[1], 7), z[6], acol[7]));
+    dz[8] = fma(sj[8], z[8], fma(SBM_LANE_BCAST(jy[1], 8), z[7], acol[8]));
+    dz[9] = fma(sj[9], z[9], fma(SBM_LANE_BCAST(jy[1], 9), z[8], acol[9]));
+    dz[10] = fma(sj[10], z[10], fma(SBM_LANE_BCAST(jy[1], 10), z[9], acol[10]));
+    dz[11] = fma(sj[11], z[11], fma(SBM_LANE_BCAST(jy[1], 11), z[10], acol[11]));
+    dz[12] = fma(sj[12], z[12], fma(SBM_LANE_BCAST(jy[1], 12), z[11], acol[12]));
+    dz[13] = fma(sj[13], z[13], fma(SBM_LANE_BCAST(jy[1], 13), z[12], acol[13]));
+    dz[14] = fma(sj[14], z[14], fma(SBM_LANE_BCAST(jy[1], 14), z[13], acol[14]));
+    dz[15] = fma(sj[15], z[15], fma(SBM_LANE_BCAST(jy[1], 15), z[14], acol[15]));
+    dz[16] = fma(sj[16], z[16], fma(SBM_LANE_BCAST(jy[1], 16), z[15], acol[16]));
+    dz[17] = fma(sj[17], z[17], fma(SBM_LANE_BCAST(jy[1], 17), z[16], acol[17]));
+    dz[18] = fma(sj[18], z[18], fma(SBM_LANE_BCAST(jy[1], 18), z[17], acol[18]));
+    dz[19] = fma(sj[19], z[19], fma(SBM_LANE_BCAST(jy[1], 19), z[18], acol[19]));
   }
 
   template <int NZ>
@@ -338,25 +340,25 @@
                                                    const double (&z)[NZ], double (&dz)[NZ]) {
     (void)jyl;
     dz[0] = fma(jyl[1], z[19], fma(jyl[0], z[0], acol[0]));
-    dz[1] = fma(jyl[3], z[1], fma(jyl[2], z[0], acol[1]));
-    dz[2] = fma(jyl[5], z[2], fma(jyl[4], z[1], acol[2]));
-    dz[3] = fma(jyl[7], z[3], fma(jyl[6], z[2], acol[3]));
-    dz[4] = fma(jyl[9], z[4], fma(jyl[8], z[3], acol[4]));
-    dz[5] = fma(jyl[11], z[5], fma(jyl[10], z[4], acol[5]));
-    dz[6] = fma(jyl[13], z[6], fma(jyl[12], z[5], acol[6]));
-    dz[7] = fma(jyl[15], z[7], fma(jyl[14], z[6], acol[7]));
-    dz[8] = fma(jyl[17], z[8], fma(jyl[16], z[7], acol[8]));
-    dz[9] = fma(jyl[19], z[9], fma(jyl[18], z[8], acol[9]));
-    dz[10] = fma(jyl[21], z[10], fma(jyl[20], z[9], acol[10]));
-    dz[11] = fma(jyl[23], z[11], fma(jyl[22], z[10], acol[11]));
-    dz[12] = fma(jyl[25], z[12], fma(jyl[24], z[11], acol[12]));
-    dz[13] = fma(jyl[27], z[13], fma(jyl[26], z[12], acol[13]));
-    dz[14] = fma(jyl[29], z[14], fma(jyl[28], z[13], acol[14]));
-    dz[15] = fma(jyl[31], z[15], fma(jyl[30], z[14], acol[15]));
-    dz[16] = fma(jyl[33], z[16], fma(jyl[32], z[15], acol[16]));
-    dz[17] = fma(jyl[35], z[17], fma(jyl[34], z[16], acol[17]));
-    dz[18] = fma(jyl[37], z[18], fma(jyl[36], z[17], acol[18]));
-    dz[19] = fma(jyl[39], z[19], fma(jyl[38], z[18], acol[19]));
+    dz[1] = fma(jyl[2], z[1], fma(jyl[3], z[0], acol[1]));
+    dz[2] = fma(jyl[4], z[2], fma(jyl[5], z[1], acol[2]));
+    dz[3] = fma(jyl[6], z[3], fma(jyl[7], z[2], acol[3]));
+    dz[4] = fma(jyl[8], z[4], fma(jyl[9], z[3], acol[4]));
+    dz[5] = fma(jyl[10], z[5], fma(jyl[11], z[4], acol[5]));
+    dz[6] = fma(jyl[12], z[6], fma(jyl[13], z[5], acol[6]));
+    dz[7] = fma(jyl[14], z[7], fma(jyl[15], z[6], acol[7]));
+    dz[8] = fma(jyl[16], z[8], fma(jyl[17], z[7], acol[8]));
+    dz[9] = fma(jyl[18], z[9], fma(jyl[19], z[8], acol[9]));
+    dz[10] = fma(jyl[20], z[10], fma(jyl[21], z[9], acol[10]));
+    dz[11] = fma(jyl[22], z[11], fma(jyl[23], z[10], acol[11]));
+    dz[12] = fma(jyl[24], z[12], fma(jyl[25], z[11], acol[12]));
+    dz[13] = fma(jyl[26], z[13], fma(jyl[27], z[12], acol[13]));
+    dz[14] = fma(jyl[28], z[14], fma(jyl[29], z[13], acol[14]));
+    dz[15] = fma(jyl[30], z[15], fma(jyl[31], z[14], acol[15]));
+    dz[16] = fma(jyl[32], z[16], fma(jyl[33], z[15], acol[16]));
+    dz[17] = fma(jyl[34], z[17], fma(jyl[35], z[16], acol[17]));
+    dz[18] = fma(jyl[36], z[18], fma(jyl[37], z[17], acol[18]));
+    dz[19] = fma(jyl[38], z[19], fma(jyl[39], z[18], acol[19]));
   }
 
   struct RG0 {
diff --git a/sysbio_modeling_amd/csrc/models/michaelis_menten.hpp b/sysbio_modeling_amd/csrc/models/michaelis_menten.hpp
--- a/sysbio_modeling_amd/csrc/models/michaelis_menten.hpp
+++ b/sysbio_modeling_amd/csrc/models/michaelis_menten.hpp
@@ -1,8 +1,8 @@
 #pragma once
 
 __constant__ short SBM_RL_CLASS[2] = {0, 1};
-__constant__ short SBM_RL_YS[4] = {0, 1, 0, 0};
-__constant__ short SBM_RL_PS[8] = {2, 4, 3, 0, 0, 1, 1, 0};
+__constant__ short SBM_RL_YS[4] = {0, 0, 0, 1};
+__constant__ short SBM_RL_PS[8] = {2, 4, 3, 0, 0, 0, 1, 1};
 __constant__ short SBM_RL_JYOUT[4] = {0, 1, 3, 2};
 __constant__ short SBM_RL_APOS[8] = {0, 64, 1, 65, 2, 68, 3, 128};
 __constant__ short SBM_RL_JPCOL[8] = {0, 0, 1, 1, 2, 4, 3, -1};
@@ -96,18 +96,19 @@
                                                         double (&jy)[RL_MAXJY], double (&jp)[RL_MAXJP]) {
     (void)t; (void)ys; (void)ps;
     const bool is0 = (cls == 0);
-    const double h0 = SBM_RCP(SBM_SEL(is0, ps[3], ps[2]) + SBM_SEL(is0, ys[0], ys[1]));
+    const double h0 = SBM_RCP(ps[3] + ys[0]);
     const double c0_x0 = h0;
     const double c0_x1 = ys[0]*c0_x0;
     const double c0_x2 = ps[2]*(c0_x0*c0_x0);
     const double c1_x0 = h0;
     const double c1_x1 = ps[1]*(c1_x0*c1_x0);
-    f = SBM_SEL(is0, ps[0] - ps[1]*ys[0] - ps[2]*c0_x1, -ps[0]*ys[0] + ps[1]*ys[1]*c1_x0);
-    jy[0] = SBM_SEL(is0, -ps[1] - ps[3]*c0_x2, ps[2]*c1_x1);
+    const double c1_x2 = ys[0]*c1_x0;
+    f = SBM_SEL(is0, ps[0] - ps[1]*ys[0] - ps[2]*c0_x1, -ps[0]*ys[1] + ps[1]*c1_x2);
+    jy[0] = SBM_SEL(is0, -ps[1] - ps[3]*c0_x2, ps[3]*c1_x1);
     jy[1] = SBM_SEL(is0, 0.0, -ps[0]);
-    jp[0] = SBM_SEL(is0, -c0_x1, ys[1]*c1_x0);
-    jp[1] = SBM_SEL(is0, ys[0]*c0_x2, -ys[1]*c1_x1);
-    jp[2] = SBM_SEL(is0, 1.0, -ys[0]);
+    jp[0] = SBM_SEL(is0, -c0_x1, c1_x2);
+    jp[1] = SBM_SEL(is0, ys[0]*c0_x2, -ys[0]*c1_x1);
+    jp[2] = SBM_SEL(is0, 1.0, -ys[1]);
     jp[3] = SBM_SEL(is0, -ys[0], 0.0);
   }
 
diff --git a/sysbio_modeling_amd/csrc/models/stiff50.hpp b/sysbio_modeling_amd/csrc/models/stiff50.hpp
--- a/sysbio_modeling_amd/csrc/models/stiff50.hpp
+++ b/sysbio_modeling_amd/csrc/models/stiff50.hpp
@@ -966,18 +966,21 @@
                                                         double (&jy)[RL_MAXJY], double (&jp)[RL_MAXJP]) {
     (void)t; (void)ys; (void)ps;
     const bool is0 = (cls == 0);
-    const double c0_x0 = 2.0*ys[0];
-    const double h0 = SBM_RCP((2.0*SBM_SEL(is0, ys[0], ys[1])) + 1.0);
+    const double h1 = 2.0*ys[1];
+    const double c0_x0 = h1;
+    const double h0 = SBM_RCP((h1) + 1.0);
     const double c0_x1 = h0;
-    const double c0_x2 = ps[1]*c0_x0*c0_x1 + ys[0] + (-1.0);
+    const double c0_x2 = ps[1]*c0_x0*c0_x1 + ys[1] + (-1.0);
     const double c1_x0 = ys[1] + (-1.0);
-    const double c1_x1 = 2.0*ys[1];
+    const double c1_x1 = h1;
     const double c1_x2 = h0;
     const double c1_x3 = ps[1]*c1_x1*c1_x2 + ys[0]*c1_x0;
     const double c1_x4 = 4.0*ys[0];
+    const double h2 = 2.0*ps[1];
+    const double h3 = (ys[1]*ys[1]);
     f = SBM_SEL(is0, -ps[0]*c0_x2, -ps[0]*c1_x3);
-    jy[0] = SBM_SEL(is0, -ps[0]*(c0_x1*c0_x1)*(2.0*ps[1] + 4.0*(ys[0]*ys[0]) + 4.0*ys[0] + 1.0), -ps[0]*c1_x0);
-    jy[1] = SBM_SEL(is0, 0.0, -ps[0]*(c1_x2*c1_x2)*(2.0*ps[1] + ys[0] + (ys[1]*ys[1])*c1_x4 + ys[1]*c1_x4));
+    jy[0] = SBM_SEL(is0, -ps[0]*(c0_x1*c0_x1)*(h2 + 4.0*h3 + 4.0*ys[1] + 1.0), -ps[0]*c1_x0);
+    jy[1] = SBM_SEL(is0, 0.0, -ps[0]*(c1_x2*c1_x2)*(h2 + ys[0] + h3*c1_x4 + ys[1]*c1_x4));
     jp[0] = SBM_SEL(is0, -c0_x2, -c1_x3);
   }
 
diff --git a/sysbio_modeling_amd/csrc/sbm_integrators.hpp b/sysbio_modeling_amd/csrc/sbm_integrators.hpp
--- a/sysbio_modeling_amd/csrc/sbm_integrators.hpp
+++ b/sysbio_modeling_amd/csrc/sbm_integrators.hpp
@@ -26,6 +26,15 @@
 #define SBM_PICK(scol, c, v, otherwise) sbm_pick(scol, c, v, otherwise)
 __device__ __forceinline__ double sbm_sel(bool c, double a, double b) { return c ? a : b; }
 #define SBM_SEL(c, a, b) sbm_sel(c, a, b)
+__device__ __forceinline__ double sbm_max_abs(double a, double b) {
+#if defined(__HIP_DEVICE_COMPILE__)
+  double m;
+  asm("v_max_f64 %0, |%1|, |%2|" : "=v"(m) : "v"(a), "v"(b));
+  return m;
+#else
+  return fmax(fabs(a), fabs(b));
+#endif
+}
 __device__ __forceinline__ double sbm_pick_col(int col, int c, double v, double otherwise) {
   const int chunk = __builtin_amdgcn_readfirstlane(col) >> 6;
   const unsigned long long mask = (c >> 6) == chunk ? (1ull << (c & 63)) : 0ull;
@@ -388,7 +397,7 @@
       float xsum = 0.f;
       auto err_ratio = [&](int c, int i) {
         const double e = fma(E7, k1[c][i], k4[c][i]);
-        const double sc = fma(rtol, fmax(fabs(z[c][i]), fabs(zt[c][i])), atol);
+        const double sc = fma(rtol, sbm_max_abs(z[c][i], zt[c][i]), atol);
         return (float)e * __builtin_amdgcn_rcpf((float)sc);
       };
 #pragma unroll
diff --git a/sysbio_modeling_amd/symbolic/emit.py b/sysbio_modeling_amd/symbolic/emit.py
--- a/sysbio_modeling_amd/symbolic/emit.py
+++ b/sysbio_modeling_amd/symbolic/emit.py
@@ -101,8 +101,9 @@
 
 class Derived:
 
-    def __init__(self, spec: ModelSpec):
+    def __init__(self, spec: ModelSpec, class_align: bool = True):
         self.spec = spec
+        self.class_align = class_align
         params = OrderedDict((p, 'fixed' if p in spec.fixed else Symbol(p)) for p in spec.params)
         jy, jp = sympy_tools.derive_sparse_jacobians(spec.equations, params)
         self.jy = jy
@@ -128,6 +129,22 @@
         for e, (r, c, _) in enumerate(jp):
             self.jp_rows[r].append((e, c))
         self._order_slots_by_structure()
+        self._align_class_slots()
+
+    def _align_class_slots(self):
+        from . import emit_rowlane
+        self.align = None
+        self.jy_base = [list(r) for r in self.jy_rows]
+        self.jp_base = [list(r) for r in self.jp_rows]
+        if self.class_align:
+            self.align = emit_rowlane.choose_alignment(
+                self.spec, self, lambda smap: _ExprPrinter(smap, rcp="SBM_RCP(%s)", lang='hip'))
+        if self.align is not None:
+            classes, row_info = emit_rowlane.find_classes(self.spec, self)
+            for i, r in enumerate(row_info):
+                c = classes[r['cls']]
+                self.jy_rows[i] = [ec for _, ec in sorted(zip(c['jy_slot'], self.jy_base[i]))]
+                self.jp_rows[i] = [ec for _, ec in sorted(zip(c['jp_slot'], self.jp_base[i]))]
 
     def _order_slots_by_structure(self):
         from . import emit_rowlane
@@ -257,7 +274,7 @@
         L.append(pad + "jp_%d = %s" % (e_idx, pr.doprint(e)))
     for i in range(n):
         for j in range(k):
-            terms = ["jy_%d*y[%d]" % (e_idx, n + c * k + j) for e_idx, c in d.jy_rows[i]]
+            terms = ["jy_%d*y[%d]" % (e_idx, n + c * k + j) for e_idx, c in d.jy_base[i]]
             terms += ["jp_%d" % e_idx for e_idx, c in d.jp_rows[i] if c == j]
             L.append(pad + "yout[%d] = (%s)" % (n + i * k + j, " + ".join(terms) if terms else "0.0"))
     L.append("")
@@ -373,8 +390,12 @@
     return "\n".join(L)
 
 
-def emit_hip(spec: ModelSpec, derived: Derived = None, class_hoist: bool = True) -> str:
-    d = derived or Derived(spec)
+def emit_hip(spec: ModelSpec, derived: Derived = None, class_hoist: bool = True, class_align: bool = None) -> str:
+    if derived is None:
+        derived = Derived(spec, class_align=True if class_align is None else class_align)
+    elif class_align is not None and derived.class_align != class_align:
+        raise ValueError("emit_hip: derived was made with class_align=%s" % derived.class_align)
+    d = derived
     n, k = spec.n_vars, spec.n_sens
     pr = _ExprPrinter(_symbol_map(spec), rcp="SBM_RCP(%s)", lang='hip')
     nnz_y, nnz_p = max(len(d.jy), 1), max(len(d.jp), 1)
@@ -426,10 +447,10 @@
           "                                                   int scol, const double (&z)[NV], double (&dz)[NV]) {"]
     for i in range(n):
         sel = "0.0"
-        for e_idx, c in reversed(d.jp_rows[i]):
+        for e_idx, c in reversed(d.jp_base[i]):
             sel = "SBM_PICK(scol, %d, jp[%d], %s)" % (c, e_idx, sel)
         expr = sel
-        for e_idx, c in d.jy_rows[i]:
+        for e_idx, c in d.jy_base[i]:
             expr = "fma(jy[%d], z[%d], %s)" % (e_idx, c, expr)
         L.append("    dz[%d] = %s;" % (i, expr))
     L += ["  }", ""]
@@ -449,7 +470,7 @@
                 out.append(s)
 
     for i in range(n):
-        exprs = [d.f_red[i]] + [d.jy_red[e] for e, _ in d.jy_rows[i]] + [d.jp_red[e] for e, _ in d.jp_rows[i]]
+        exprs = [d.f_red[i]] + [d.jy_red[e] for e, _ in d.jy_base[i]] + [d.jp_red[e] for e, _ in d.jp_base[i]]
         todo = []
         for e in exprs:
             need(e, todo)
@@ -457,10 +478,10 @@
             L.append("    const double %s = %s;" % (s, pr.doprint(temp_expr[s])))
             emitted.add(s)
         sel = "0.0"
-        for e_idx, c in reversed(d.jp_rows[i]):
+        for e_idx, c in reversed(d.jp_base[i]):
             sel = "SBM_PICK(scol, %d, %s, %s)" % (c, pr.doprint(d.jp_red[e_idx]), sel)
         expr = sel
-        for e_idx, c in d.jy_rows[i]:
+        for e_idx, c in d.jy_base[i]:
             expr = "fma(%s, z[%d], %s)" % (pr.doprint(d.jy_red[e_idx]), c, expr)
         L.append("    dz[%d] = SBM_SEL(state_lane, %s, %s);" % (i, pr.doprint(d.f_red[i]), expr))
     L += ["  }", ""]
diff --git a/sysbio_modeling_amd/symbolic/emit_rowlane.py b/sysbio_modeling_amd/symbolic/emit_rowlane.py
--- a/sysbio_modeling_amd/symbolic/emit_rowlane.py
+++ b/sysbio_modeling_amd/symbolic/emit_rowlane.py
@@ -23,49 +23,80 @@
     return canon, ys, ps
 
 
-def find_classes(spec, d):
+def find_classes(spec, d, align='derived'):
     var_index = {v: i for i, v in enumerate(spec.variables)}
     par_index = {p: i for i, p in enumerate(spec.params)}
     classes = OrderedDict()
     row_info = []
+    jy_rows, jp_rows = getattr(d, 'jy_base', d.jy_rows), getattr(d, 'jp_base', d.jp_rows)
     for i in range(spec.n_vars):
-        bundle = [d.f_c[i]] + [d.jy_c[e] for e, _ in d.jy_rows[i]] + [d.jp_c[e] for e, _ in d.jp_rows[i]]
+        bundle = [d.f_c[i]] + [d.jy_c[e] for e, _ in jy_rows[i]] + [d.jp_c[e] for e, _ in jp_rows[i]]
         canon, ys, ps = _canonical(bundle, var_index, par_index)
-        key = (sympy.srepr(canon), len(d.jy_rows[i]), len(d.jp_rows[i]))
+        key = (sympy.srepr(canon), len(jy_rows[i]), len(jp_rows[i]))
         if key not in classes:
-            classes[key] = dict(canon=canon, rows=[], n_jy=len(d.jy_rows[i]), n_jp=len(d.jp_rows[i]),
+            classes[key] = dict(canon=canon, rows=[], n_jy=len(jy_rows[i]), n_jp=len(jp_rows[i]),
                                 n_ys=len(ys), n_ps=len(ps))
         classes[key]['rows'].append(i)
         row_info.append(dict(cls=list(classes.keys()).index(key), ys=ys, ps=ps))
-    return list(classes.values()), row_info
+    classes = list(classes.values())
+    if align == 'derived':
+        align = getattr(d, 'align', None)
+    _place(classes, align)
+    if align is not None:
+        for r in row_info:
+            c = classes[r['cls']]
+            for kind in ('ys', 'ps'):
+                at = [None] * (max(c[kind + '_slot'] + [-1]) + 1)
+                for k, s in enumerate(c[kind + '_slot']):
+                    at[s] = r[kind][k]
+                r[kind] = at
+    return classes, row_info
+
+
+def _place(classes, align):
+    for ci, c in enumerate(classes):
+        a = align[ci] if align is not None else dict(ys=range(c['n_ys']), ps=range(c['n_ps']), jy=range(c['n_jy']),
+                                                     jp=range(c['n_jp']))
+        for kind in ('ys', 'ps', 'jy', 'jp'):
+            c[kind + '_slot'] = list(a[kind])
+            assert len(c[kind + '_slot']) == c['n_' + kind] == len(set(c[kind + '_slot']))
+        if align is not None:
+            rename = {Symbol('YS_%d' % k): Symbol('YS_%d' % s) for k, s in enumerate(c['ys_slot'])}
+            rename.update({Symbol('PS_%d' % k): Symbol('PS_%d' % s) for k, s in enumerate(c['ps_slot'])})
+            c['canon'] = tuple(e.xreplace(rename) for e in c['canon'])
+
+
+def _n_slots(classes, kind):
+    return max([s + 1 for c in classes for s in c[kind + '_slot']] + [1])
 
 
 def emit_rowlane_tables(spec, d, printer_factory):
     classes, row_info = find_classes(spec, d)
     n = spec.n_vars
-    max_ys = max([c['n_ys'] for c in classes] + [1])
-    max_ps = max([c['n_ps'] for c in classes] + [1])
-    max_jy = max([c['n_jy'] for c in classes] + [1])
-    max_jp = max([c['n_jp'] for c in classes] + [1])
+    max_ys, max_ps, max_jy, max_jp = (_n_slots(classes, kind) for kind in ('ys', 'ps', 'jy', 'jp'))
     tag = "SBM_RL"
 
     def table(name, rows_of_slots):
         flat = ", ".join(str(v) for slot in rows_of_slots for v in slot)
         return "__constant__ short %s_%s[%d] = {%s};" % (tag, name, len(rows_of_slots) * n, flat)
 
-    ys_t = [[(row_info[i]['ys'][s] if s < len(row_info[i]['ys']) else 0) for i in range(n)] for s in range(max_ys)]
-    ps_t = [[(row_info[i]['ps'][s] if s < len(row_info[i]['ps']) else 0) for i in range(n)] for s in range(max_ps)]
+    def operand(i, kind, s):
+        at = row_info[i][kind]
+        return at[s] if s < len(at) and at[s] is not None else 0
+
+    ys_t = [[operand(i, 'ys', s) for i in range(n)] for s in range(max_ys)]
+    ps_t = [[operand(i, 'ps', s) for i in range(n)] for s in range(max_ps)]
     nj = max(len(d.jy), 1)
     jy_t = [[(d.jy_rows[i][s][0] if s < len(d.jy_rows[i]) else nj) for i in range(n)] for s in range(max_jy)]
-    jp_t = [[(i * 64 + d.jp_rows[i][s][1] if s < len(d.jp_rows[i]) else n * 64) for i in range(n)]
-            for s in range(max_jp)]
+    jp_t = [[(i * 64 + d.jp_rows[i][s][1] if s < len(d.jp_rows[i]) else n * 64) for i in range(n)] for s in range(max_jp)]
     jpc_t = [[(d.jp_rows[i][s][1] if s < len(d.jp_rows[i]) else -1) for i in range(n)] for s in range(max_jp)]
     jyc_t = [[(d.jy_rows[i][s][1] if s < len(d.jy_rows[i]) else -1) for i in range(n)] for s in range(max_jy)]
     L = ["// row-lane tables: [slot][row]",
          "__constant__ short %s_CLASS[%d] = {%s};" % (tag, n, ", ".join(str(r['cls']) for r in row_info)),
          table("YS", ys_t), table("PS", ps_t), table("JYOUT", jy_t), table("APOS", jp_t), table("JPCOL", jpc_t),
          table("JYCOL", jyc_t), ""]
-    meta = dict(classes=classes, max_ys=max_ys, max_ps=max_ps, max_jy=max_jy, max_jp=max_jp)
+    meta = dict(classes=classes, max_ys=max_ys, max_ps=max_ps, max_jy=max_jy, max_jp=max_jp,
+                share_products=getattr(d, 'align', None) is not None)
     return L, meta
 
 
@@ -94,6 +125,8 @@
     if kind is None:
         return 0
     n = int(node.exp) - 1 if node.is_Pow and kind == 'mul' else max(len(node.args) - 1, 1)
+    if node.is_Mul and node.args[0] == -1:
+        n -= 1
     return _OP_COST[kind] * n + sum(_tree_cost(a) for a in node.args)
 
 
@@ -122,7 +155,7 @@
     def printed(ci, node):
         pr.shared = {k: v for k, v in shared[ci].items() if k != node}
         for (sym, _), e in zip(per_class[ci][0], exprs[ci]):
-            if _op_kind(e) == 'mul':
+            if _op_kind(e) == 'mul' and _op_kind(node) not in ('add', 'mul'):
                 pr.shared[sym] = "(%s)" % pr._print(e)
         text = pr._print(node)
         return _LEAF.sub('@', text), _LEAF.findall(text)
@@ -144,7 +177,7 @@
                     if node in shared[ci]:
                         walk.skip()
                         continue
-                    if node in seen or _op_kind(node) in (None, 'add', 'mul'):
+                    if node in seen or _op_kind(node) is None or _tree_cost(node) == 0:
                         continue
                     seen.add(node)
                     shape, leaves = printed(ci, node)
@@ -199,6 +232,197 @@
     return "".join(out)
 
 
+def _share_products(repl, red, prefix):
+    repl, red = list(repl), list(red)
+    n_temp = len(repl)
+    for e in list(red):
+        if not (e.is_Mul and len(e.args) >= 2 and not e.args[0].is_Number):
+            continue
+        factors = set(e.args)
+
+        def holds(m):
+            return m.is_Mul and factors < set(m.args)
+        if not any(x.has(e) or any(holds(m) for m in sympy.preorder_traversal(x)) for x in red if x != e):
+            continue
+        sym = Symbol('%s%d' % (prefix, n_temp))
+        n_temp += 1
+        repl.append((sym, e))
+        red = [sym if x == e else x.replace(holds, lambda m: sympy.Mul(sym, *[a for a in m.args if a not in factors]))
+               for x in red]
+    return repl, red
+
+
+_CALL = re.compile(r'(?<![A-Za-z0-9_])([A-Za-z_][A-Za-z0-9_]*)\(')
+
+
+def _text_cost(lines):
+    cost = 0
+    for ln in lines:
+        if '=' not in ln or ln.lstrip().startswith('//'):
+            continue
+        rhs = ln.split('=', 1)[1].split(';')[0]
+        if rhs.lstrip().startswith('(cls =='):
+            continue
+        for name in _CALL.findall(rhs):
+            cost += {'SBM_RCP': _OP_COST['rcp'], 'SBM_SEL': _SEL_COST, 'sqrt': _OP_COST['sqrt'], 'exp': _OP_COST['exp'],
+                     'log': _OP_COST['log'], 'pow': _OP_COST['pow']}.get(name, _OP_COST['call'])
+        cost += rhs.count('*') * _OP_COST['mul'] + (rhs.count(' + ') + rhs.count(' - ')) * _OP_COST['add']
+    return cost
+
+
+_MAX_CANDIDATES = 600
+_MAX_GREEDY = 300
+
+
+def choose_alignment(spec, d, make_printer):
+    import math
+    from itertools import islice, permutations, product, repeat
+    base, _ = find_classes(spec, d, align=None)
+    if len(base) < 2:
+        return None
+    kinds = ('ys', 'ps', 'jy', 'jp')
+    width = {k: max(c['n_' + k] for c in base) for k in kinds}
+    n_slots = {k: max(width[k], 1) for k in kinds}
+    ref = max(range(len(base)), key=lambda ci: (sum(base[ci]['n_' + k] for k in kinds), -ci))
+    others = [ci for ci in range(len(base)) if ci != ref]
+    identity = [{k: tuple(range(c['n_' + k])) for k in kinds} for c in base]
+    memo = {}
+
+    def cost(align, only=None):
+        classes = [dict(c) for c in base]
+        _place(classes, align)
+        if only is not None:
+            classes = [classes[ci] for ci in sorted(only)]
+        return _text_cost(_dispatch_body(classes, n_slots, make_printer, hoist=True, share_products=True, memo=memo))
+
+    def placements(ci, k):
+        n_own = base[ci]['n_' + k]
+        return permutations(range(width[k] if k in ('ys', 'ps') else n_own), n_own)
+
+    def n_placements(ci, k):
+        n_own = base[ci]['n_' + k]
+        return math.perm(width[k] if k in ('ys', 'ps') else n_own, n_own)
+
+    def combos(ci):
+        return (dict(zip(kinds, combo)) for combo in product(*[placements(ci, k) for k in kinds]))
+
+    def n_combos(ci):
+        return math.prod(n_placements(ci, k) for k in kinds)
+
+    _place(base, None)
+    plain = _text_cost(_dispatch_body(base, n_slots, make_printer, hoist=True, share_products=False))
+    n_all = 1
+    for ci in others:
+        n_all = min(n_all * n_combos(ci), _MAX_CANDIDATES + 1)
+    if n_all <= _MAX_CANDIDATES:
+        best, best_cost = identity, cost(identity)
+        for choice in product(*[combos(ci) for ci in others]):
+            cand = list(identity)
+            for ci, a in zip(others, choice):
+                cand[ci] = a
+            c = cost(cand) if cand != identity else best_cost
+            if c < best_cost:
+                best, best_cost = cand, c
+        return best if best_cost < plain else None
+    best = list(identity)
+    for ci in others:
+        pair_cost = cost(best, only=(ref, ci))
+        if n_combos(ci) <= _MAX_GREEDY // 4:
+            rounds = [combos(ci)]
+        else:
+            rounds = [zip(repeat(k), placements(ci, k)) for k in kinds]
+        share = max(_MAX_GREEDY // (len(others) * len(rounds)), 1)
+        for trials in rounds:
+            for a in islice(trials, share):
+                if isinstance(a, tuple):
+                    a = dict(best[ci], **{a[0]: a[1]})
+                if a == best[ci]:
+                    continue
+                c = cost(best[:ci] + [a] + best[ci + 1:], only=(ref, ci))
+                if c < pair_cost:
+                    best[ci], pair_cost = a, c
+    return best if cost(best) < plain else None
+
+
+def _dispatch_body(classes, n_slots, make_printer, hoist=True, share_products=False, memo=None):
+    smap = {'t': 't'}
+    for s in range(n_slots['ys']):
+        smap['YS_%d' % s] = 'ys[%d]' % s
+    for s in range(n_slots['ps']):
+        smap['PS_%d' % s] = 'ps[%d]' % s
+    pr = make_printer(smap)
+    L = []
+    last = len(classes) - 1
+    for ci in range(last):
+        L.append("    const bool is%d = (cls == %d);" % (ci, ci))
+    is_last_at = len(L)
+    def class_cse(ci, canon):
+        key = (ci, canon, share_products)
+        if memo is not None and key in memo:
+            return memo[key]
+        repl, red = cse(list(canon), symbols=sympy.numbered_symbols('c%d_x' % ci), optimizations='basic')
+        if share_products:
+            repl, red = _share_products(repl, red, 'c%d_x' % ci)
+        if memo is not None:
+            memo[key] = (repl, red)
+        return repl, red
+    per_class = [class_cse(ci, c['canon']) for ci, c in enumerate(classes)]
+    shared, hoisted = _plan_hoist(per_class, pr) if hoist and len(classes) > 1 else ([{} for _ in classes], [])
+    stmts = OrderedDict()
+    for ci, (repl, _) in enumerate(per_class):
+        pr.shared = shared[ci]
+        for sym, e in repl:
+            stmts[str(sym)] = "    const double %s = %s;" % (sym, pr.doprint(e))
+    for h in hoisted:
+        stmts[h['name']] = "    const double %s = %s;   // classes %s" % (
+            h['name'], _sel_template(h), ", ".join(str(ci) for ci in h['classes']))
+    emitted = set()
+
+    def emit_stmt(name):
+        if name in emitted:
+            return
+        emitted.add(name)
+        for dep in _NAME.findall(stmts[name].split('=', 1)[1]):
+            if dep in stmts:
+                emit_stmt(dep)
+        L.append(stmts[name])
+
+    bodies = []
+    for ci, c in enumerate(classes):
+        L.append("    // class %d: rows %s" % (ci, ", ".join(str(r) for r in c['rows'])))
+        pr.shared = shared[ci]
+        for sym, _ in per_class[ci][0]:
+            emit_stmt(str(sym))
+        bodies.append([pr.doprint(e) for e in per_class[ci][1]])
+    pr.shared = {}
+    for h in hoisted:
+        emit_stmt(h['name'])
+    if any("(is%d," % last in ln for ln in L[is_last_at:]):
+        L.insert(is_last_at, "    const bool is%d = (cls == %d);" % (last, last))
+
+    def chain(kind, k):
+        def of(ci):
+            c = classes[ci]
+            if kind == 'f':
+                return bodies[ci][0]
+            if kind == 'jy':
+                return bodies[ci][1 + c['jy_slot'].index(k)] if k in c['jy_slot'] else "0.0"
+            return bodies[ci][1 + c['n_jy'] + c['jp_slot'].index(k)] if k in c['jp_slot'] else "0.0"
+        expr = of(last)
+        if all(of(ci) == expr for ci in range(last)):
+            return expr
+        for ci in range(last - 1, -1, -1):
+            expr = "SBM_SEL(is%d, %s, %s)" % (ci, of(ci), expr)
+        return expr
+
+    L.append("    f = %s;" % chain('f', 0))
+    for k in range(n_slots['jy']):
+        L.append("    jy[%d] = %s;" % (k, chain('jy', k)))
+    for k in range(n_slots['jp']):
+        L.append("    jp[%d] = %s;" % (k, chain('jp', k)))
+    return L
+
+
 def emit_rowlane_members(spec, d, meta, make_printer, hoist=True):
     n = spec.n_vars
     classes = meta['classes']
@@ -221,69 +445,8 @@
          "                                                        const double (&ps)[RL_MAXPS], double& f,",
          "                                                        double (&jy)[RL_MAXJY], double (&jp)[RL_MAXJP]) {",
          "    (void)t; (void)ys; (void)ps;"]
-    smap = {'t': 't'}
-    for s in range(meta['max_ys']):
-        smap['YS_%d' % s] = 'ys[%d]' % s
-    for s in range(meta['max_ps']):
-        smap['PS_%d' % s] = 'ps[%d]' % s
-    pr = make_printer(smap)
-    last = len(classes) - 1
-    for ci in range(last):
-        L.append("    const bool is%d = (cls == %d);" % (ci, ci))
-    is_last_at = len(L)
-    per_class = [cse(list(c['canon']), symbols=sympy.numbered_symbols('c%d_x' % ci), optimizations='basic')
-                 for ci, c in enumerate(classes)]
-    shared, hoisted = _plan_hoist(per_class, pr) if hoist and len(classes) > 1 else ([{} for _ in classes], [])
-    stmts = OrderedDict()
-    for ci, (repl, _) in enumerate(per_class):
-        pr.shared = shared[ci]
-        for sym, e in repl:
-            stmts[str(sym)] = "    const double %s = %s;" % (sym, pr.doprint(e))
-    for h in hoisted:
-        stmts[h['name']] = "    const double %s = %s;   // classes %s" % (
-            h['name'], _sel_template(h), ", ".join(str(ci) for ci in h['classes']))
-    emitted = set()
-
-    def emit_stmt(name):
-        if name in emitted:
-            return
-        emitted.add(name)
-        for dep in _NAME.findall(stmts[name].split('=', 1)[1]):
-            if dep in stmts:
-                emit_stmt(dep)
-        L.append(stmts[name])
-
-    bodies = []
-    for ci, c in enumerate(classes):
-        L.append("    // class %d: rows %s" % (ci, ", ".join(str(r) for r in c['rows'])))
-        pr.shared = shared[ci]
-        for sym, _ in per_class[ci][0]:
-            emit_stmt(str(sym))
-        bodies.append([pr.doprint(e) for e in per_class[ci][1]])
-    pr.shared = {}
-    for h in hoisted:
-        emit_stmt(h['name'])
-    if any("(is%d," % last in ln for ln in L[is_last_at:]):
-        L.insert(is_last_at, "    const bool is%d = (cls == %d);" % (last, last))
-
-    def chain(kind, k):
-        def of(ci):
-            c = classes[ci]
-            if kind == 'f':
-                return bodies[ci][0]
-            if kind == 'jy':
-                return bodies[ci][1 + k] if k < c['n_jy'] else "0.0"
-            return bodies[ci][1 + c['n_jy'] + k] if k < c['n_jp'] else "0.0"
-        expr = of(last)
-        for ci in range(last - 1, -1, -1):
-            expr = "SBM_SEL(is%d, %s, %s)" % (ci, of(ci), expr)
-        return expr
-
-    L.append("    f = %s;" % chain('f', 0))
-    for k in range(meta['max_jy']):
-        L.append("    jy[%d] = %s;" % (k, chain('jy', k)))
-    for k in range(meta['max_jp']):
-        L.append("    jp[%d] = %s;" % (k, chain('jp', k)))
+    L += _dispatch_body(classes, dict(ys=meta['max_ys'], ps=meta['max_ps'], jy=meta['max_jy'], jp=meta['max_jp']),
+                        make_printer, hoist=hoist, share_products=meta.get('share_products', False))
     where = {}
     for i in range(n):
         for k, (e_idx, c) in enumerate(d.jy_rows[i]):
@@ -316,7 +479,7 @@
           "    (void)jy; (void)sj;"]
     for i in range(n):
         expr = "acol[%d]" % i
-        for e_idx, c in d.jy_rows[i]:
+        for e_idx, c in d.jy_base[i]:
             if e_idx in static_idx:
                 expr = "fma(sj[%d], z[%d], %s)" % (static_idx[e_idx], c, expr)
             else:
@@ -332,8 +495,8 @@
           "    (void)jyl;"]
     for i in range(n):
         expr = "acol[%d]" % i
-        for k, (e_idx, c) in enumerate(d.jy_rows[i]):
-            expr = "fma(jyl[%d], z[%d], %s)" % (i * meta['max_jy'] + k, c, expr)
+        for e_idx, c in d.jy_base[i]:
+            expr = "fma(jyl[%d], z[%d], %s)" % (i * meta['max_jy'] + where[e_idx][1], c, expr)
         L.append("    dz[%d] = %s;" % (i, expr))
     L += ["  }"]
     return L
```

After: 449.1 million ODE-steps/s (median of 6 runs). 4.3% higher.
